# ocean1100/stereo_match

Measured on AMD Instinct MI355X. Metric: stereo pairs/sec + Mpix·disp/sec, KITTI 1242×375 D=128 SGM, 1/2/4/8 GPU, higher is better.
Workload: dtype u8

## Files before the change

### include/stereo_match_amd.h

```cpp
#ifndef STEREO_MATCH_AMD_H
#define STEREO_MATCH_AMD_H

#include <stddef.h>
#include <stdint.h>

#ifdef __cplusplus
extern "C" {
#endif

#define SM_ABI_VERSION 3

#define SM_OK 0
#define SM_E_ARG (-1)
#define SM_E_HIP (-2)
#define SM_E_UNSUPPORTED (-4)

#define SM_COST_SGBM 0
#define SM_COST_CENSUS 1
#define SM_COST_VOLUME 2

#define SM_MODE_SGBM 5
#define SM_MODE_HH 8

typedef struct sm_params {
// ... 158 lines not shown
    int min_disparity;
    int num_disparities;
    int block_size;
    int pre_filter_type;
    int pre_filter_size;
    int pre_filter_cap;
    int texture_threshold;
    int uniqueness_ratio;
    int speckle_window_size;
    int speckle_range;
    int disp12_max_diff;
} sm_bm_params;

int sm_bm_default_params(int num_disparities, int block_size, sm_bm_params* out);
int sm_bm_right_matcher_params(const sm_bm_params* left, sm_bm_params* right_out);
int sm_bm_compute(sm_ctx* ctx, const uint8_t* left, const uint8_t* right, int H, int W, int stride,
                  const sm_bm_params* p, int16_t* disp_out);
int sm_bm_compute_batch_device(sm_ctx* ctx, const uint8_t* d_left, const uint8_t* d_right, int npairs,
                               size_t pair_stride_bytes, int H, int W, int stride, const sm_bm_params* p,
                               int16_t* d_disp_out);

int sm_compute_batch(sm_ctx** ctxs, int ngpu, const uint8_t* const* left, const uint8_t* const* right, int npairs,
                     int H, int W, const sm_params* p, int16_t* out);

int sm_right_matcher_params(const sm_params* left, sm_params* right_out);

int sm_synchronize(sm_ctx* ctx);

int sm_get_counters(sm_ctx* ctx, long long* sweep_fallbacks);

#define SM_COUNTER_SWEEP_FALLBACKS 0
#define SM_COUNTER_EW_REPAIRS 1
#define SM_COUNTER_VOLUME_CLAMPED 2
#define SM_COUNTER_VOLUME_NAN 3
#define SM_COUNTER_LINE_GROUPS 4
#define SM_COUNTER_EW_OPEN 5
#define SM_COUNTER_BAND_REPAIRS 6
#define SM_COUNTER_BAND_OPEN 7
#define SM_COUNTER_BAND_GROUPS 8
#define SM_COUNTER_LINE_STRIPS 9
int sm_get_counter(sm_ctx* ctx, int which, long long* value);

int sm_set_cu_mask(sm_ctx* ctx, const uint32_t* mask, int nwords);

#define SM_STAGE_COST 0
#define SM_STAGE_PATHS 1
#define SM_STAGE_WTA 2
#define SM_STAGE_MEDIAN 3
#define SM_STAGE_TOTAL 4
#define SM_STAGE_WLS 5
#define SM_STAGE_SPECKLE 6
#define SM_STAGE_HORIZONTAL 7
#define SM_STAGE_SWEEP 8
#define SM_STAGE_SWEEP_WTA 9
#define SM_STAGE_H2D 10
#define SM_STAGE_D2H 11
#define SM_STAGE_FALLBACK 12
#define SM_STAGE_CALL 13
#define SM_NUM_STAGES 14
#define SM_TIMING_ONLY 0x40000000
int sm_set_timing(sm_ctx* ctx, int enable);
int sm_get_timing(sm_ctx* ctx, int stage, double* total_ms, long long* launches, long long* pairs);
int sm_reset_timing(sm_ctx* ctx);

long long sm_debug_fetch(sm_ctx* ctx, int what, void* host, size_t bytes);

int sm_set_debug_flags(sm_ctx* ctx, int flags);

#define SM_TUNE_EW_LANES 1
#define SM_TUNE_SWEEP_NCW 2
#define SM_TUNE_EW_WAVES 3
#define SM_TUNE_EW_PRIO 4
#define SM_TUNE_EW_WARMUP 5
#define SM_TUNE_SWEEP_LINES 6
#define SM_TUNE_EW_GUESS 7
#define SM_TUNE_BANDS 8
#define SM_TUNE_BAND_WARMUP 9
#define SM_TUNE_BAND_GUESS 10
#define SM_TUNE_COST_WGS 11
#define SM_TUNE_LR_STAGGER 12
#define SM_TUNE_SWEEP_XCD 13
#define SM_TUNE_PLY_STAGE 14
#define SM_TUNE_EW_START 15
int sm_set_tuning(sm_ctx* ctx, int key, int value);

const char* sm_last_error(sm_ctx* ctx);

const char* sm_version(void);
int sm_abi_version(void);

#ifdef __cplusplus
}
#endif

#endif
```

### stereo_match_amd/_lib.py

```python
from __future__ import annotations

import ctypes
import os
import re
import threading

import numpy as np

_HERE = os.path.dirname(os.path.abspath(__file__))
LIB_PATH = os.environ.get("STEREO_MATCH_AMD_LIB") or os.path.join(_HERE, "libstereo_match_amd.so")
HEADER_PATH = os.path.join(os.path.dirname(_HERE), "include", "stereo_match_amd.h")

SM_OK, SM_E_ARG, SM_E_HIP, SM_E_UNSUPPORTED = 0, -1, -2, -4
SM_COST_SGBM, SM_COST_CENSUS, SM_COST_VOLUME = 0, 1, 2
SM_MODE_SGBM, SM_MODE_HH = 5, 8
TIMING_ONLY = 0x40000000
STAGES = ("cost", "paths", "wta", "median", "total", "wls", "speckle", "horizontal", "sweep", "sweep_wta", "h2d",
          "d2h", "fallback", "call")


class SmParams(ctypes.Structure):
    _fields_ = [(n, ctypes.c_int) for n in (
        "min_disparity", "num_disparities", "block_size", "P1", "P2",
        "disp12_max_diff", "uniqueness_ratio", "pre_filter_cap",
# ... 632 lines not shown
        if src.size and (src.strides[1] != cn or (src.ndim == 3 and src.strides[2] != 1) or src.strides[0] < W * cn):
            src = np.ascontiguousarray(src)
        dH, dW = (H + 1) // 2, (W + 1) // 2
        out = np.empty((dH, dW) if src.ndim == 2 else (dH, dW, cn), np.uint8)
        self._check(self._lib.sm_pyr_down_u8(self.ctx, src.ctypes.data if src.size else None, H, W,
                                             src.strides[0] if src.size else W * cn, cn,
                                             out.ctypes.data if out.size else None))
        return out

    def pyr_down_batch_device(self, d_src: int, nimg: int, src_img_stride: int, H: int, W: int, src_stride: int,
                              channels: int, d_dst: int, dst_img_stride: int, dst_stride: int):
        self._check(self._lib.sm_pyr_down_u8_batch_device(
            self.ctx, ctypes.c_void_p(d_src), nimg, src_img_stride, H, W, src_stride, channels, ctypes.c_void_p(d_dst),
            dst_img_stride, dst_stride))

    def bm_compute(self, left: np.ndarray, right: np.ndarray, params: "SmBmParams") -> np.ndarray:
        left = np.ascontiguousarray(left)
        right = np.ascontiguousarray(right)
        H, W = left.shape
        out = np.empty((H, W), np.int16)
        self._check(self._lib.sm_bm_compute(self.ctx, left.ctypes.data, right.ctypes.data, H, W, W,
                                            ctypes.byref(params), out.ctypes.data))
        return out

    def bm_compute_batch_device(self, d_left: int, d_right: int, npairs: int, pair_stride: int, H: int, W: int,
                                stride: int, params: "SmBmParams", d_out: int):
        self._check(self._lib.sm_bm_compute_batch_device(
            self.ctx, ctypes.c_void_p(d_left), ctypes.c_void_p(d_right), npairs, pair_stride, H, W, stride,
            ctypes.byref(params), ctypes.c_void_p(d_out)))

    def synchronize(self):
        self._check(self._lib.sm_synchronize(self.ctx))

    COUNTERS = ("sweep_fallbacks", "ew_repairs", "volume_clamped", "volume_nan", "line_groups",
                "ew_open", "band_repairs", "band_open", "band_groups", "line_strips")

    def counters(self) -> dict:
        out = {}
        n = ctypes.c_longlong()
        for i, name in enumerate(self.COUNTERS):
            self._check(self._lib.sm_get_counter(self.ctx, i, ctypes.byref(n)))
            out[name] = n.value
        return out

    def set_cu_mask(self, cus):
        if cus is None:
            self._check(self._lib.sm_set_cu_mask(self.ctx, None, 0))
            return
        nwords = (max(cus) // 32 + 1) if cus else 1
        words = (ctypes.c_uint32 * nwords)()
        for c in cus:
            words[c // 32] |= 1 << (c % 32)
        self._check(self._lib.sm_set_cu_mask(self.ctx, words, nwords))

    def set_timing(self, on, stages=None):
        v = int(bool(on))
        if on and stages is not None:
            v = TIMING_ONLY
            for name in stages:
                v |= 1 << STAGES.index(name)
        self._check(self._lib.sm_set_timing(self.ctx, v))

    def reset_timing(self):
        self._check(self._lib.sm_reset_timing(self.ctx))

    def timing(self) -> dict:
        out = {}
        for i, name in enumerate(STAGES):
            ms = ctypes.c_double()
            n = ctypes.c_longlong()
            np_ = ctypes.c_longlong()
            self._check(self._lib.sm_get_timing(self.ctx, i, ctypes.byref(ms), ctypes.byref(n), ctypes.byref(np_)))
            out[name] = (ms.value, n.value, np_.value)
        return out

    def set_debug_flags(self, flags: int):
        self._check(self._lib.sm_set_debug_flags(self.ctx, int(flags)))

    TUNE_EW_LANES, TUNE_SWEEP_NCW, TUNE_EW_WAVES, TUNE_EW_PRIO, TUNE_EW_WARMUP, TUNE_SWEEP_LINES = 1, 2, 3, 4, 5, 6
    TUNE_EW_GUESS = 7
    TUNE_BANDS, TUNE_BAND_WARMUP, TUNE_BAND_GUESS, TUNE_COST_WGS, TUNE_LR_STAGGER, TUNE_SWEEP_XCD = 8, 9, 10, 11, 12, 13
    TUNE_PLY_STAGE = 14
    TUNE_EW_START = 15

    def set_tuning(self, key: int, value: int):
        self._check(self._lib.sm_set_tuning(self.ctx, int(key), int(value)))

    def debug_fetch(self, what: int) -> bytes:
        n = self._lib.sm_debug_fetch(self.ctx, what, None, 0)
        if n < 0:
            _raise(int(n), self.ctx)
        buf = (ctypes.c_char * max(int(n), 1))()
        r = self._lib.sm_debug_fetch(self.ctx, what, buf, int(n))
        if r < 0:
            _raise(int(r), self.ctx)
        return bytes(buf)[:int(n)]


def right_matcher_params(p: SmParams) -> SmParams:
    lib = load()
    out = SmParams()
    rc = lib.sm_right_matcher_params(ctypes.byref(p), ctypes.byref(out))
    if rc != SM_OK:
        _raise(rc, None)
    return out


def compute_batch(engines, lefts, rights, params: SmParams) -> np.ndarray:
    lib = load()
    n = len(lefts)
    if n != len(rights):
        raise ValueError("lefts and rights differ in length")
    if n == 0:
        return np.empty((0, 0, 0), np.int16)
    L = [np.ascontiguousarray(a, np.uint8) for a in lefts]
    R = [np.ascontiguousarray(b, np.uint8) for b in rights]
    H, W = L[0].shape
    if any(a.shape != (H, W) for a in L + R):
        raise ValueError("all images must have the same shape")
    out = np.empty((n, H, W), np.int16)
    ctxs = (ctypes.c_void_p * len(engines))(*[e.ctx for e in engines])
    lp = (ctypes.c_void_p * n)(*[a.ctypes.data for a in L])
    rp = (ctypes.c_void_p * n)(*[b.ctypes.data for b in R])
    rc = lib.sm_compute_batch(ctxs, len(engines), lp, rp, n, H, W, ctypes.byref(params), out.ctypes.data)
    if rc != SM_OK:
        _raise(rc, None)
    return out


_engines: dict = {}


def engine(device: int = 0) -> Engine:
    key = (threading.get_ident(), device)
    e = _engines.get(key)
    if e is None:
        e = _engines[key] = Engine(device)
    return e
```

### stereo_match_amd/csrc/sm_api.hip

```cpp
#include <hip/hip_runtime.h>

#include <algorithm>
#include <cmath>
#include <cstdarg>
#include <cstdio>
#include <cstring>
#include <string>
#include <thread>
#include <type_traits>
#include <vector>

#include "../../include/stereo_match_amd.h"
#include "sm_cost.hpp"
#include "sm_paths.hpp"
#include "sm_post.hpp"
#include "sm_wls.hpp"
#include "sm_speckle.hpp"
#include "sm_reproject.hpp"
#include "sm_rectify.hpp"
#include "sm_nlm.hpp"
#include "sm_filter.hpp"
#include "sm_cloud.hpp"
#include "sm_bm.hpp"
#include "sm_wide.hpp"
// ... 30 lines not shown
    hipEvent_t a, b;
};

struct BufSet {
    DevBuf census[2], cost, L, raw;
    DevBuf part, key2, pre;
    DevBuf st;
    DevBuf vst;
    hipEvent_t paths_done = nullptr, wta_done = nullptr;
    bool pending = false;
};

#ifndef EW_PATCH_ATOM
#define EW_PATCH_ATOM 1
#endif

constexpr int DBG_VL16 = 8, DBG_STORE_W = 16, DBG_ROW = 32, DBG_OVERLAP = 64, DBG_H64 = 512, DBG_NO_C8 = 1024;
constexpr int DBG_OLD_EW = 256, DBG_SWEEP_V2 = 128, DBG_SWEEP2_NW = 1 << 27;
constexpr int DBG_FGS_NO_SWEEP = 1 << 28, DBG_FGS_NO_MEM = 1 << 29;
constexpr int DBG_NO_MALL_GROUPS = 1 << 30;
constexpr int DBG_NARROW_SWEEPS = 1 << 19, DBG_WIDE_SWEEPS = 1 << 21;
constexpr int DBG_LEGACY = 4096, DBG_SWEEP1 = 8192, DBG_SWEEP8 = 16384, DBG_HYBRID = 32768;
constexpr int DBG_COST_TILE = 1 << 22;
constexpr int DBG_CONCURRENT_LR = 1 << 20;
constexpr int DBG_FORCE_FALLBACK = 1 << 23;
constexpr int ERR_GROUP0 = 0, ERR_STICKY = 32, ERR_FALLBACKS = 48;
constexpr int ERR_VOL_CLAMPED = 52, ERR_VOL_NAN = 54, ERR_EW_REPAIRS = 56, ERR_EW_OPEN = 58;
constexpr int ERR_BAND_REPAIRS = 60, ERR_BAND_OPEN = 62;
constexpr int DBG_NO_FALLBACK = (int)0x80000000u;
constexpr int kAblationFlags = 1 | 2 | 4 | DBG_STORE_W | DBG_ROW | DBG_SWEEP_V2 | DBG_SWEEP2_NW | DBG_HYBRID |
                               (7 << 24) | DBG_FGS_NO_SWEEP | DBG_FGS_NO_MEM | DBG_NO_FALLBACK;

}

struct sm_ctx {
    int device = 0;
    hipStream_t own_stream = nullptr;
    hipStream_t stream = nullptr;
    hipStream_t side = nullptr;
    DevBuf img[2], planes, out, dbg, volbuf, sp_parent, sp_count, rp_in, rp_out, rp_min, bm_pre[2], bm_cost;
    DevBuf rm_src, rm_mapx, rm_mapy, rm_dst, rm_gray;
    DevBuf nlm_tab;
    std::vector<int32_t> nlm_tab_host;
    uint32_t nlm_key_h = 0;
    int nlm_key_t = 0, nlm_key_s = 0, nlm_ntab = 0, nlm_shift = 0;
    DevBuf cl_tot, cl_off, ply_tot, ply_off, cl_verts, cl_colors, cl_out;
    DevBuf flt_a;
    DevBuf wls_num, wls_den, wls_inter, wls_w, wls_disp[2], wls_out;
    DevBuf wls_R, wls_IT;
    hipStream_t wls_stream = nullptr;
    hipStream_t lr_stream = nullptr;
    hipEvent_t ev_stagger = nullptr;
    hipEvent_t sweep_done_ev = nullptr;
    bool sweep_done_hit = false;
    int tune_lr_stagger = 0;
    hipEvent_t ev_wls_fork = nullptr, ev_wls_ready = nullptr;
    DevBuf hop, sweep_err;
    DevBuf volwin;

    void* pin = nullptr;
    size_t pin_n = 0;
    sm_ctx* twin = nullptr;
    hipEvent_t ev_lr_fork = nullptr, ev_lr_join = nullptr;
    std::vector<uint32_t> cu_mask;
    uint32_t hop_epoch = 0;
    hipEvent_t ev_fork = nullptr, ev_join = nullptr;
    hipEvent_t ev_fb_fork = nullptr, ev_fb_join = nullptr;
    hipEvent_t ev_ew_done = nullptr;
    const uint32_t* fb_guard = nullptr;
    hipStream_t wta_override = nullptr;
    const uint32_t* wta_skip = nullptr;
    int16_t* wta_dst = nullptr;
    BufSet set[2];
    int next_set = 0;
    int lastH = 0, lastW = 0, last_width1 = 0, lastD = 0, last_ndirs = 0, last_cost = 0, last_minD = 0;
    int last_minX1 = 0, last_index = 0, last_set = 0;
    size_t last_L_pair = 0;
    uint32_t timing = 0;
    int dbg_flags = 0;
    int tune_ew_lanes = 0, tune_sweep_ncw = 0, tune_ew_waves = 0, tune_ew_prio = 0;
    int tune_ew_warmup = 0, tune_sweep_lines = 0;
    int tune_ew_guess = 0;
    int tune_ew_start = 0;
    int tune_bands = 0, tune_band_warmup = 0, tune_band_guess = 0;
    int tune_cost_wgs = 0;
    int tune_ply_stage = 0;
    int tune_sweep_xcd = 0;
    long long line_groups = 0;
    long long band_groups = 0;
    long long line_strips = 0;
    std::vector<TimedEvent> pending;
    std::vector<hipEvent_t> free_events;
    double stage_ms[SM_NUM_STAGES] = {0};
    long long stage_launches[SM_NUM_STAGES] = {0};
    long long stage_pairs[SM_NUM_STAGES] = {0};
    std::string err;
};

namespace {

int fail(sm_ctx* ctx, int code, const char* fmt, ...)
{
    char buf[512];
    va_list ap;
    va_start(ap, fmt);
    vsnprintf(buf, sizeof buf, fmt, ap);
    va_end(ap);
    if (ctx) ctx->err = buf;
    g_thread_error = buf;
    return code;
}

#define HIP_TRY(ctx, expr)                                                                           \
    do {                                                                                              \
        hipError_t e_ = (expr);                                                                       \
        if (e_ != hipSuccess)                                                                         \
            return fail((ctx), SM_E_HIP, "%s failed: %s (%s:%d)", #expr, hipGetErrorString(e_),   \
                        __FILE__, __LINE__);                                                          \
    } while (0)

int ensure(sm_ctx* ctx, DevBuf& b, size_t bytes)
{
    if (b.n >= bytes && b.p) return SM_OK;
    if (b.p) {
        HIP_TRY(ctx, hipDeviceSynchronize());
        (void)hipFree(b.p);
        b.p = nullptr;
        b.n = 0;
    }
    size_t want = std::max<size_t>(bytes, 256);
    HIP_TRY(ctx, hipMalloc(&b.p, want));
    b.n = want;
    return SM_OK;
}

int normalize(sm_ctx* ctx, const sm_params* p, int H, int W, Norm& n, int cn = 1)
{
    if (!p) return fail(ctx, SM_E_ARG, "params is NULL");
    if (H <= 0 || W <= 0) return fail(ctx, SM_E_ARG, "empty image (%dx%d)", W, H);
    if (W > 32767) return fail(ctx, SM_E_UNSUPPORTED, "width %d > 32767", W);
    n.minD = p->min_disparity;
    n.D = n.Dv = p->num_disparities;
    if (p->cost_kind == SM_COST_VOLUME) {
        if (n.Dv <= 0) return fail(ctx, SM_E_ARG, "cost volume needs at least one disparity plane (got %d)", n.Dv);
        n.D = (n.Dv + 15) & ~15;
    } else if (n.D <= 0 || n.D % 16 != 0) {
        return fail(ctx, SM_E_ARG, "numDisparities must be a positive multiple of 16 (got %d)", n.D);
    }
    if (n.D > 256) return fail(ctx, SM_E_UNSUPPORTED, "numDisparities %d > 256 not built", n.Dv);
    n.maxD = n.minD + n.Dv;
    n.bs = p->block_size > 0 ? p->block_size : 5;
    n.ftzero = std::max(p->pre_filter_cap, 15) | 1;
    n.uniq = p->uniqueness_ratio >= 0 ? p->uniqueness_ratio : 10;
    n.disp12 = p->disp12_max_diff > 0 ? p->disp12_max_diff : 1;
    n.P1 = p->P1 > 0 ? p->P1 : 2;
    n.P2 = std::max(p->P2 > 0 ? p->P2 : 5, n.P1 + 1);
    n.speckle_ws = p->speckle_window_size;
    n.speckle_range = p->speckle_range;
    n.cost = p->cost_kind;
    n.mode = p->mode;
    if (n.cost != SM_COST_SGBM && n.cost != SM_COST_CENSUS && n.cost != SM_COST_VOLUME)
        return fail(ctx, SM_E_ARG, "cost_kind %d unknown", n.cost);
    if (n.mode != SM_MODE_SGBM && n.mode != SM_MODE_HH)
        return fail(ctx, SM_E_UNSUPPORTED, "mode %d not supported (5 = MODE_SGBM, 8 = MODE_HH)", n.mode);
    if (cn != 1 && cn != 3) return fail(ctx, SM_E_ARG, "images must have 1 or 3 channels (got %d)", cn);
    if (cn != 1 && n.cost != SM_COST_SGBM) return fail(ctx, SM_E_UNSUPPORTED, "colour input needs the SGBM cost");
// ... 340 lines not shown
    HIP_TRY(ctx, hipGetLastError());
    return SM_OK;
}

template <int DPLV, bool CENSUS>
int launch_paths_dpl(sm_ctx* ctx, const Norm& n, const Geo& g, BufSet& bs, int dirset)
{
    if constexpr ((16 * DPLV) % 64 == 0) {
        if (ctx->dbg_flags & DBG_H64) {
            if (DPLV == 8 && !(ctx->dbg_flags & DBG_VL16))
                return launch_paths_t<DPLV, CENSUS, 8>(ctx, n, g, bs, dirset);
            return launch_paths_t<DPLV, CENSUS, 16>(ctx, n, g, bs, dirset);
        }
    }
    if constexpr (DPLV == 8) {
        if (!(ctx->dbg_flags & DBG_VL16)) return launch_paths_t<DPLV, CENSUS, 8, true>(ctx, n, g, bs, dirset);
    }
    return launch_paths_t<DPLV, CENSUS, 16, true>(ctx, n, g, bs, dirset);
}

enum { DISPATCH_PATHS = 0, DISPATCH_WTA = 1, DISPATCH_HORIZONTAL = 2, DISPATCH_HYBRID = 3 };

int dispatch(sm_ctx* ctx, const Norm& n, const Geo& g, BufSet& bs, int what)
{
    const bool census = n.cost == SM_COST_CENSUS;
    const int h = what == DISPATCH_HORIZONTAL ? DIRS_EW : what == DISPATCH_HYBRID ? DIRS_EW_UP : DIRS_ALL;
    switch (n.dpl) {
#define CASE(k)                                                                                               \
    case k:                                                                                                   \
        if (what == DISPATCH_WTA)                                                                             \
            return census ? launch_wta_t<k, true>(ctx, n, g, bs) : launch_wta_t<k, false>(ctx, n, g, bs);     \
        return census ? launch_paths_dpl<k, true>(ctx, n, g, bs, h) : launch_paths_dpl<k, false>(ctx, n, g, bs, h);
        CASE(1) CASE(2) CASE(3) CASE(4) CASE(5) CASE(6) CASE(7) CASE(8)
        CASE(9) CASE(10) CASE(11) CASE(12) CASE(13) CASE(14) CASE(15) CASE(16)
#undef CASE
    default: return fail(ctx, SM_E_UNSUPPORTED, "numDisparities %d not built", n.D);
    }
}

int ensure_event(sm_ctx* ctx, hipEvent_t& e);
bool use_sweep(const sm_ctx* ctx, const Norm& n, int H);

int hybrid_slots(const Norm& n) { return n.ndirs == 8 ? 5 : 2; }

bool use_hybrid(const sm_ctx* ctx, const Norm& n, int H)
{
    if (!SM_ABLATIONS || (n.ndirs != 8 && n.ndirs != 5) || !(ctx->dbg_flags & DBG_HYBRID) ||
        (ctx->dbg_flags & (DBG_LEGACY | DBG_SWEEP8)))
        return false;
    sm_ctx tmp = *ctx;
    tmp.dbg_flags = (ctx->dbg_flags & ~DBG_HYBRID) | DBG_SWEEP8;
    return use_sweep(&tmp, n, H);
}

bool use_sweep(const sm_ctx* ctx, const Norm& n, int H)
{
    if (ctx->dbg_flags & (DBG_LEGACY | DBG_ROW)) return false;
    if (n.cost == SM_COST_CENSUS && !use_cost8(ctx, n)) return false;
    const int cmax = n.cost == SM_COST_CENSUS ? 64 : n.cost == SM_COST_VOLUME ? smk::VOL_CMAX : 0;
    if (cmax + n.P2 > 16383) return false;
    if (H > 65535 || n.width1 <= 0) return false;
    const size_t W = (size_t)(n.maxX1 - std::min(n.minD, 0));
    if (W * 6 + 16 > kRowLds) return false;
    return (uint64_t)H * n.width1 * n.D * 2 <= smk::kMaxRecords;
}

struct SweepJob {
    const uint8_t* cost;
    size_t cost_pair;
    const uint8_t* ew;
    size_t ew_pair, ew_slot;
    uint16_t* part;
    size_t part_pair;
    uint32_t* key2;
    uint32_t* pre;
    uint32_t* err;
    int G;
    uint8_t* st = nullptr;
    size_t st_pair = 0;
    int ewarm = 0;
    int ewguess = 0;
    int ewstart = 0;
    int part_il = 0;
    int nband = 1, band_h = 0, vwarm = 0, vguess = 0;
    uint8_t* vst = nullptr;
    size_t vst_pair = 0;
};

int stream_cus(hipStream_t st, int ncu)
{
    uint32_t mask[32] = {0};
    const uint32_t words = (uint32_t)std::min(32, (ncu + 31) / 32);
    if (hipExtStreamGetCUMask(st, words, mask) != hipSuccess) return ncu;
    int c = 0;
    for (uint32_t i = 0; i < words; i++) c += __builtin_popcount(mask[i]);
    return c > 0 ? std::min(c, ncu) : ncu;
}

int ensure_sweep_err(sm_ctx* ctx)
{
    if (ctx->sweep_err.p) return SM_OK;
    int rc = ensure(ctx, ctx->sweep_err, SWEEP_STATS ? (size_t(8) << 20) : 256);
    if (rc != SM_OK) return rc;
    HIP_TRY(ctx, hipMemsetAsync(ctx->sweep_err.p, 0, SWEEP_STATS ? (size_t(8) << 20) : 256, ctx->stream));
    return SM_OK;
}

int sweep_variant(const sm_ctx* ctx)
{
    if (SM_ABLATIONS && (ctx->dbg_flags & DBG_SWEEP_V2)) return 6;
    if (SM_ABLATIONS && (ctx->dbg_flags & DBG_SWEEP2_NW)) return 3;
    return (ctx->dbg_flags & DBG_NARROW_SWEEPS) ? 1 : 0;
}

struct SweepFit {
    smk::SweepInfo si{};
    int nwg = 0, cap = 0, ncu = 0;
};
bool sweep_fit_variant(sm_ctx* ctx, const Norm& n, int mode, int variant, SweepFit& f)
{
    if (smk::sweep_info(n.D, (int)elem_bytes(n), mode, variant, ctx->device, &f.si) != hipSuccess) return false;
    int ncu = 0;
    if (hipDeviceGetAttribute(&ncu, hipDeviceAttributeMultiprocessorCount, ctx->device) != hipSuccess) return false;
    f.ncu = stream_cus(ctx->stream, std::max(ncu, 1));
    const int per_cu = f.si.blocks_per_cu >= 3 ? f.si.blocks_per_cu - 1 : std::max(f.si.blocks_per_cu, 1);
    f.cap = per_cu * f.ncu;
    f.nwg = (n.width1 + f.si.cw - 1) / f.si.cw;
    return f.nwg <= f.cap;
}

int sweep_min_pairs(sm_ctx* ctx, const Norm& n)
{
    if (n.cost != SM_COST_CENSUS) return 3;
    SweepFit f;
    if (!sweep_fit_variant(ctx, n, 2, 0, f) || f.nwg <= 0) return 7;
    return std::max(2, std::min(7, (200 + f.nwg - 1) / f.nwg));
}

double sweep_model(const SweepFit& f, int G)
{
    const int per_launch = std::max(1, std::min(G, f.cap / std::max(f.nwg, 1)));
    const int launches = (G + per_launch - 1) / per_launch;
    const int per_cu = (per_launch * f.nwg + f.ncu - 1) / std::max(f.ncu, 1);
    return (double)launches * per_cu * (f.si.threads / 64 - 1) * std::max(f.si.dpl, 1);
}

bool sweep_capacity(sm_ctx* ctx, const Norm& n, int mode, int G, SweepFit& f)
{
    if (ctx->tune_sweep_ncw && sweep_variant(ctx) <= 1) {
        for (int v : {0, 1, 2}) {
            SweepFit t;
            if (sweep_fit_variant(ctx, n, mode, v, t) && t.si.ncw == ctx->tune_sweep_ncw) {
                f = t;
                return true;
            }
        }
        return false;
    }
    const int variant = sweep_variant(ctx);
    if (!sweep_fit_variant(ctx, n, mode, variant, f)) {
        if (!(variant == 0 && f.si.impl == 1 && sweep_fit_variant(ctx, n, mode, 1, f))) return false;
    } else if (variant == 0 && f.si.impl == 1 && G > 0 && !(ctx->dbg_flags & DBG_WIDE_SWEEPS)) {
        SweepFit nf;
        if (sweep_fit_variant(ctx, n, mode, 1, nf) && sweep_model(nf, G) < sweep_model(f, G)) f = nf;
    }
    if (variant == 0 && G > 0 && !(ctx->dbg_flags & DBG_WIDE_SWEEPS)) {
        SweepFit lf;
        if (sweep_fit_variant(ctx, n, mode, 2, lf) && sweep_model(lf, G) < sweep_model(f, G)) f = lf;
    }
    return true;
}

bool sweeps_fit(sm_ctx* ctx, const Norm& n, bool hybrid, bool lines = false)
{
    const int m8[2] = {0, 2}, m5[1] = {1}, mh[1] = {0}, l8[2] = {3, 4}, l5[1] = {3};
    const int* modes = hybrid ? mh : lines ? (n.ndirs == 8 ? l8 : l5) : n.ndirs == 8 ? m8 : m5;
    const int count = !hybrid && n.ndirs == 8 ? 2 : 1;
    for (int k = 0; k < count; k++) {
        SweepFit f;
        if (!sweep_capacity(ctx, n, modes[k], 0, f)) return false;
        if (lines && modes[k] == 3 && f.nwg > smk::patch_max_strips(n.D)) return false;
        if (lines && modes[k] == 3 && f.si.ncw < 11) return false;
    }
    return true;
}

int sweep_pass(sm_ctx* ctx, const Norm& n, const Geo& g, const SweepJob& j, int mode)
{
    SweepFit f;
    const bool banded = j.nband > 1;
    if (banded ? !(sweep_fit_variant(ctx, n, mode, 0, f) && f.si.impl == 1) : !sweep_capacity(ctx, n, mode, j.G, f)) {
        if (f.nwg > f.cap)
            return fail(ctx, SM_E_UNSUPPORTED, "sweep: %d strips exceed %d resident workgroups", f.nwg, f.cap);
        return fail(ctx, SM_E_UNSUPPORTED, "sweep: numDisparities %d not built", n.D);
    }
    const smk::SweepInfo& si = f.si;
    const int nwg = f.nwg, cap = f.cap;
    const int nb = banded ? j.nband : 1;
    const int nblk = banded ? (j.band_h + j.vwarm + si.hb - 1) / si.hb : (g.H + si.hb - 1) / si.hb;
    const int per_launch = (ctx->dbg_flags & DBG_SWEEP1) ? 1 : std::max(1, std::min(j.G, cap / (nwg * nb)));
    const size_t hop_pair = (size_t)nwg * nb * 2 * nblk * si.ngr;
    const size_t hop_bytes = hop_pair * 8 * per_launch;
    if (hop_pair * 8 > smk::kMaxRecords) return fail(ctx, SM_E_UNSUPPORTED, "sweep: boundary buffer too large");
    int rc;
    if (ctx->hop.n < hop_bytes || !ctx->hop.p) {
        if ((rc = ensure(ctx, ctx->hop, hop_bytes)) != SM_OK) return rc;
        HIP_TRY(ctx, hipMemsetAsync(ctx->hop.p, 0, ctx->hop.n, ctx->stream));
        ctx->hop_epoch = 0;
    }
    if ((rc = ensure_sweep_err(ctx)) != SM_OK) return rc;
    for (int p0 = 0; p0 < j.G; p0 += per_launch) {
        const int np = std::min(per_launch, j.G - p0);
        if (++ctx->hop_epoch > 0xFFFFu) {
            HIP_TRY(ctx, hipMemsetAsync(ctx->hop.p, 0, ctx->hop.n, ctx->stream));
            ctx->hop_epoch = 1;
        }
        smk::SweepArgs a{};
        a.cost = j.cost + (size_t)p0 * j.cost_pair;
        a.cost_pair = j.cost_pair;
        a.ew = j.ew ? j.ew + (size_t)p0 * j.ew_pair : nullptr;
        a.ew_pair = j.ew_pair;
        a.ew_slot = j.ew_slot;
        a.part = j.part ? (uint16_t*)((uint8_t*)j.part + (size_t)p0 * j.part_pair) : nullptr;
        a.part_pair = j.part_pair;
        a.hop = (unsigned long long*)ctx->hop.p;
        a.hop_pair = hop_pair;
        a.st = j.st ? j.st + (size_t)p0 * j.st_pair : nullptr;
        a.st_pair = j.st_pair;
        a.ewarm = j.ewarm;
        a.ewguess = j.ewguess;
        a.ewstart = j.ewstart;
        a.part_il = j.part_il;
        a.nband = nb;
        a.band_h = j.band_h;
        a.vwarm = j.vwarm;
        a.vguess = j.vguess;
        a.hop_nblk = nblk;
        a.vst = j.vst ? j.vst + (size_t)p0 * j.vst_pair : nullptr;
        a.vst_pair = j.vst_pair;
        if (ctx->tune_sweep_xcd > 0) {
            a.xcd_total = np * nwg * nb;
            a.xcd_per = (a.xcd_total + 7) / 8;
        }
        a.rec = j.key2 ? j.key2 + (size_t)p0 * g.H * g.W : nullptr;
        a.nb = j.pre ? j.pre + (size_t)p0 * g.H * g.W : nullptr;
        a.err = j.err;
        a.H = g.H;
        a.W = g.W;
        a.W1 = n.width1;
        a.D = n.D;
        a.Dv = n.Dv;
        a.minD = n.minD;
        a.minX1 = n.minX1;
        a.P1 = n.P1;
        a.P2 = n.P2;
        a.uniq = n.uniq;
        a.inv_ku = n.uniq < 100 ? 1.0f / (float)(100 - n.uniq) : 0.f;
        a.nwg = nwg;
        a.epoch = ctx->hop_epoch;
#if SWEEP_STATS
        a.stats = (unsigned long long*)((char*)ctx->sweep_err.p + 1024);
#endif
        a.dbg = (ctx->dbg_flags >> 24) & 7;
        HIP_TRY(ctx, smk::sweep_launch(n.D, (int)elem_bytes(n), mode, si.impl, a, np, ctx->stream));
    }
    return SM_OK;
}

struct StreamSwap {
    sm_ctx* c;
    hipStream_t old;
    StreamSwap(sm_ctx* c_, hipStream_t s) : c(c_), old(c_->stream) { c->stream = s; }
    ~StreamSwap() { c->stream = old; }
};

int ew_lanes(const sm_ctx* ctx, const Norm& n)
{
    if (ctx->tune_ew_lanes) return ctx->tune_ew_lanes;
    if (ctx->dbg_flags & DBG_OLD_EW) return -1;
    if (n.D % 64 == 0) return 32;
    if (n.D % 32 == 0) return 16;
    return elem_bytes(n) == 1 ? 0 : -1;
}

int launch_ew(sm_ctx* ctx, const Norm& n, const Geo& g, BufSet& bs)
{
    const size_t et = elem_bytes(n);
    const int vl = ew_lanes(ctx, n);
    if (vl < 0) return dispatch(ctx, n, g, bs, DISPATCH_HORIZONTAL);
    smk::EwArgs a{};
    a.cost = (const uint8_t*)bs.cost.p;
    a.cost_pair = g.vol * et;
    a.out = (uint8_t*)bs.L.p;
    a.out_pair = g.L_pair;
    a.out_slot = g.slot_bytes;
    a.H = g.H;
    a.W1 = n.width1;
    a.P1 = n.P1;
    a.P2 = n.P2;
    a.wpb = ctx->tune_ew_waves;
    a.prio = ctx->tune_ew_prio;
    StageTimer t(ctx, ctx->stream, SM_STAGE_HORIZONTAL, g.G);
    const hipError_t e = smk::ew_launch(n.D, (int)et, vl, a, g.G, ctx->stream);
    if (e == hipErrorInvalidValue) return fail(ctx, SM_E_UNSUPPORTED, "E/W lines: numDisparities %d not built", n.D);
    HIP_TRY(ctx, e);
    return SM_OK;
}

int run_sweep(sm_ctx* ctx, const Norm& n, const Geo& g, BufSet& bs, hipStream_t wta_stream, uint32_t* err)
{
    const int G = g.G;
    int rc;
    const size_t et = elem_bytes(n);
    SweepJob j{};
    j.cost = (const uint8_t*)bs.cost.p;
// ... 50 lines not shown
        if (ctx->dbg_flags & DBG_FORCE_FALLBACK) HIP_TRY(ctx, hipMemsetAsync(gflag, 1, 1, ws));
        HIP_TRY(ctx, smk::lr_rows_launch((const uint32_t*)bs.key2.p, (const uint32_t*)bs.pre.p, (int16_t*)bs.raw.p,
                                         ctx->wta_dst, g.G, g.H, g.W, n.Dv, n.minD, n.minX1, n.maxX1, n.disp12,
                                         gflag, ws));
        StreamSwap sw(ctx, ws);
        ctx->wta_override = ws;
        ctx->fb_guard = gflag;
        rc = dispatch(ctx, n, g, bs, DISPATCH_PATHS);
        if (rc == SM_OK) rc = dispatch(ctx, n, g, bs, DISPATCH_WTA);
        ctx->fb_guard = nullptr;
        ctx->wta_override = nullptr;
        return rc;
    }
    hipStream_t fs = ctx->side;
    if (fb) {
        if (ctx->dbg_flags & DBG_FORCE_FALLBACK) HIP_TRY(ctx, hipMemsetAsync(gflag, 1, 1, ws));
        if ((rc = ensure_event(ctx, ctx->ev_fb_fork)) != SM_OK) return rc;
        if ((rc = ensure_event(ctx, ctx->ev_fb_join)) != SM_OK) return rc;
        HIP_TRY(ctx, hipEventRecord(ctx->ev_fb_fork, ws));
        HIP_TRY(ctx, hipStreamWaitEvent(fs, ctx->ev_fb_fork, 0));
        StreamSwap sw(ctx, fs);
        ctx->wta_override = fs;
        ctx->fb_guard = gflag;
        rc = dispatch(ctx, n, g, bs, DISPATCH_PATHS);
        if (rc == SM_OK) rc = dispatch(ctx, n, g, bs, DISPATCH_WTA);
        ctx->fb_guard = nullptr;
        ctx->wta_override = nullptr;
        if (rc != SM_OK) return rc;
        HIP_TRY(ctx, hipEventRecord(ctx->ev_fb_join, fs));
    }
    HIP_TRY(ctx, smk::lr_rows_launch((const uint32_t*)bs.key2.p, (const uint32_t*)bs.pre.p, (int16_t*)bs.raw.p,
                                     ctx->wta_dst, g.G, g.H, g.W, n.Dv, n.minD, n.minX1, n.maxX1, n.disp12,
                                     fb ? gflag : nullptr, ws));
    if (fb) HIP_TRY(ctx, hipStreamWaitEvent(ws, ctx->ev_fb_join, 0));
    return SM_OK;
}

bool use_lines(sm_ctx* ctx, const Norm& n)
{
    if (ctx->tune_sweep_lines < 0 || ctx->tune_ew_lanes || (ctx->dbg_flags & DBG_OLD_EW)) return false;
    return sweeps_fit(ctx, n, false, true);
}

int ew_start(const sm_ctx* ctx, const Norm& n)
{
    if (ctx->tune_ew_start < 0) return 0;
    if (ctx->tune_ew_start > 0) return ctx->tune_ew_start == 1 ? smk::EWS_MAXN : ctx->tune_ew_start;
    return elem_bytes(n) == 1 ? smk::EWS_MAXN : 0;
}

int ew_warmup(const sm_ctx* ctx, const Norm& n, int ewstart)
{
    if (ctx->tune_ew_warmup > 0) return ctx->tune_ew_warmup;
    if (ewstart > 0 && elem_bytes(n) == 1) return 9;
    return 16;
}

long long path_max(const Norm& n)
{
    if (n.cost == SM_COST_CENSUS) return 62 + n.P2;
    if (n.cost == SM_COST_VOLUME) return smk::VOL_CMAX + n.P2;
    const long long side = 2 * (n.bs / 2) + 1;
    return side * side * (2 * n.ftzero + (255 >> 2)) + n.P2;
}

int line_bands(const sm_ctx* ctx, const Norm& n, int H, int G)
{
    if (n.ndirs != 5 || ctx->tune_bands == 1 || 5 * path_max(n) > 65535) return 1;
    SweepFit f;
    if (!sweep_fit_variant(const_cast<sm_ctx*>(ctx), n, 3, 0, f) || f.si.impl != 1 || f.nwg <= 0) return 1;
    int nb = ctx->tune_bands >= 2 ? ctx->tune_bands : std::min(f.cap / std::max(1, G * f.nwg), H / 24);
    nb = std::min(nb, H);
    if (nb < 2) return 1;
    const int bh = (H + nb - 1) / nb;
    return (H + bh - 1) / bh;
}

int band_warmup(const sm_ctx* ctx, const Norm& n)
{
    if (ctx->tune_band_warmup > 0) return ctx->tune_band_warmup;
    return elem_bytes(n) == 1 ? 16 : 24;
}

int run_lines(sm_ctx* ctx, const Norm& n, const Geo& g, BufSet& bs, hipStream_t ws, uint32_t* gflag)
{
    const int G = g.G;
    const size_t et = elem_bytes(n);
    int rc;
    SweepJob j{};
    j.cost = (const uint8_t*)bs.cost.p;
    j.cost_pair = g.vol * et;
    j.G = G;
    j.err = gflag;
    if ((rc = ensure(ctx, bs.part, (size_t)G * g.vol * 2)) != SM_OK) return rc;
    j.part = (uint16_t*)bs.part.p;
    j.part_pair = g.vol * 2;
    SweepFit f;
    j.nband = line_bands(ctx, n, g.H, G);
    if (j.nband > 1 ? !sweep_fit_variant(ctx, n, 3, 0, f) : !sweep_capacity(ctx, n, 3, G, f))
        return fail(ctx, SM_E_UNSUPPORTED, "sweep lines: no instance fits");
    j.st_pair = ((size_t)g.H * f.nwg * 4 * n.D * et + 255) & ~size_t(255);
    if ((rc = ensure(ctx, bs.st, j.st_pair * G)) != SM_OK) return rc;
    j.st = (uint8_t*)bs.st.p;
    j.ewstart = ew_start(ctx, n);
    j.ewarm = ew_warmup(ctx, n, j.ewstart);
    j.ewguess = ctx->tune_ew_guess;
    j.part_il = SWEEP_IL && n.ndirs == 8 && et == 1 && n.D != 256 && f.si.dpl % 2 == 0 &&
                f.si.dpl == (n.D % 32 == 0 ? n.D / 16 : n.D / 8) ? 1 : 0;
    if (j.nband > 1 && ctx->tune_ew_warmup <= 0 && et == 2) j.ewarm = 54;
    if (j.nband > 1) {
        j.band_h = (g.H + j.nband - 1) / j.nband;
        j.vwarm = band_warmup(ctx, n);
        j.vguess = ctx->tune_band_guess;
        j.vst_pair = ((size_t)j.nband * 6 * n.width1 * n.D * et + 255) & ~size_t(255);
        if ((rc = ensure(ctx, bs.vst, j.vst_pair * G)) != SM_OK) return rc;
        j.vst = (uint8_t*)bs.vst.p;
        ctx->band_groups++;
    }
    ctx->line_groups++;
    ctx->line_strips += (long long)f.nwg * G;
    const bool fb_side = n.ndirs == 5 && ws == ctx->stream && !(ctx->dbg_flags & DBG_NO_FALLBACK);
    {
        StageTimer t(ctx, ctx->stream, SM_STAGE_PATHS, G);
        {
            StageTimer ts(ctx, ctx->stream, SM_STAGE_SWEEP, G);
            if ((rc = sweep_pass(ctx, n, g, j, 3)) != SM_OK) return rc;
        }
        if (ctx->sweep_done_ev) {
            HIP_TRY(ctx, hipEventRecord(ctx->sweep_done_ev, ctx->stream));
            ctx->sweep_done_hit = true;
        }
        smk::EwPatchArgs pa{};
        pa.cost = j.cost;
        pa.cost_pair = j.cost_pair;
        pa.part = j.part;
        pa.part_pair = j.part_pair * 1;
        pa.st = j.st;
        pa.st_pair = j.st_pair;
        pa.H = g.H;
        pa.W1 = n.width1;
        pa.nwg = f.nwg;
        pa.cw = f.si.cw;
        pa.P1 = n.P1;
        pa.P2 = n.P2;
        pa.guard = gflag;
        pa.fixes = reinterpret_cast<unsigned long long*>((uint32_t*)ctx->sweep_err.p + ERR_EW_REPAIRS);
        pa.atom = EW_PATCH_ATOM && et == 2 && 5 * path_max(n) < 65536 ? 1 : 0;
        pa.part_il = j.part_il;
        auto ew_patch = [&](hipStream_t st) -> int {
            const hipError_t e = smk::ew_patch_launch(n.D, (int)et, pa, G, st);
            if (e == hipErrorInvalidValue) return fail(ctx, SM_E_UNSUPPORTED, "E/W patch: numDisparities %d not built", n.D);
            HIP_TRY(ctx, e);
            return SM_OK;
        };
        const bool ew_side = fb_side && pa.atom && j.nband > 1;
        if (fb_side) {
            if (ctx->dbg_flags & DBG_FORCE_FALLBACK) HIP_TRY(ctx, hipMemsetAsync(gflag, 1, 1, ctx->stream));
            if ((rc = ensure_event(ctx, ctx->ev_fb_fork)) != SM_OK) return rc;
            if ((rc = ensure_event(ctx, ctx->ev_fb_join)) != SM_OK) return rc;
            HIP_TRY(ctx, hipEventRecord(ctx->ev_fb_fork, ctx->stream));
            HIP_TRY(ctx, hipStreamWaitEvent(ctx->side, ctx->ev_fb_fork, 0));
            if (ew_side) {
                if ((rc = ensure_event(ctx, ctx->ev_ew_done)) != SM_OK) return rc;
                {
                    StageTimer th(ctx, ctx->side, SM_STAGE_HORIZONTAL, G);
                    if ((rc = ew_patch(ctx->side)) != SM_OK) return rc;
                }
                HIP_TRY(ctx, hipEventRecord(ctx->ev_ew_done, ctx->side));
            }
            StreamSwap sw(ctx, ctx->side);
            ctx->wta_override = ctx->side;
            ctx->fb_guard = gflag;
            rc = dispatch(ctx, n, g, bs, DISPATCH_PATHS);
            if (rc == SM_OK) rc = dispatch(ctx, n, g, bs, DISPATCH_WTA);
            ctx->fb_guard = nullptr;
            ctx->wta_override = nullptr;
            if (rc != SM_OK) return rc;
            HIP_TRY(ctx, hipEventRecord(ctx->ev_fb_join, ctx->side));
        }
        if (!ew_side) {
            StageTimer th(ctx, ctx->stream, SM_STAGE_HORIZONTAL, G);
            if ((rc = ew_patch(ctx->stream)) != SM_OK) return rc;
        }
        if (j.nband > 1) {
            smk::BandPatchArgs ba{};
            ba.cost = j.cost;
            ba.cost_pair = j.cost_pair;
            ba.part = j.part;
            ba.part_pair = j.part_pair;
            ba.vst = j.vst;
            ba.vst_pair = j.vst_pair;

            ba.H = g.H;
            ba.W1 = n.width1;
            ba.nband = j.nband;
            ba.band_h = j.band_h;
            ba.P1 = n.P1;
            ba.P2 = n.P2;
            ba.guard = gflag;
            ba.fixes = reinterpret_cast<unsigned long long*>((uint32_t*)ctx->sweep_err.p + ERR_BAND_REPAIRS);
            const hipError_t eb = smk::band_patch_launch(n.D, (int)et, ba, G, ctx->stream);
            if (eb == hipErrorInvalidValue) return fail(ctx, SM_E_UNSUPPORTED, "band patch: numDisparities %d not built", n.D);
            HIP_TRY(ctx, eb);
            if (ew_side) HIP_TRY(ctx, hipStreamWaitEvent(ctx->stream, ctx->ev_ew_done, 0));
        }
    }
    if (ws != ctx->stream) {
        HIP_TRY(ctx, hipEventRecord(bs.paths_done, ctx->stream));
        HIP_TRY(ctx, hipStreamWaitEvent(ws, bs.paths_done, 0));
    }
    if (n.ndirs == 8) {
        if ((rc = ensure(ctx, bs.key2, (size_t)G * g.H * g.W * 4)) != SM_OK) return rc;
        if ((rc = ensure(ctx, bs.pre, (size_t)G * g.H * g.W * 4)) != SM_OK) return rc;
        j.key2 = (uint32_t*)bs.key2.p;
        j.pre = (uint32_t*)bs.pre.p;
        {
            StreamSwap sw(ctx, ws);
            StageTimer t(ctx, ctx->stream, SM_STAGE_WTA, G);
            StageTimer ts(ctx, ctx->stream, SM_STAGE_SWEEP_WTA, G);
            if ((rc = sweep_pass(ctx, n, g, j, 4)) != SM_OK) return rc;
        }
        return sweep_finish(ctx, n, g, bs, ws, gflag);
    }
    StreamSwap sw(ctx, ws);
    ctx->wta_override = ws;
    {
        StageTimer ts(ctx, ws, SM_STAGE_SWEEP_WTA, G);
        ctx->wta_skip = fb_side ? gflag : nullptr;
        rc = dispatch(ctx, n, g, bs, DISPATCH_WTA);
        ctx->wta_skip = nullptr;
    }
    if (fb_side) {
        if (rc == SM_OK) HIP_TRY(ctx, hipStreamWaitEvent(ws, ctx->ev_fb_join, 0));
    } else if (rc == SM_OK && !(ctx->dbg_flags & DBG_NO_FALLBACK)) {
        if (ctx->dbg_flags & DBG_FORCE_FALLBACK) HIP_TRY(ctx, hipMemsetAsync(gflag, 1, 1, ws));
        ctx->fb_guard = gflag;
        rc = dispatch(ctx, n, g, bs, DISPATCH_PATHS);
        if (rc == SM_OK) rc = dispatch(ctx, n, g, bs, DISPATCH_WTA);
        ctx->fb_guard = nullptr;
    }
    ctx->wta_override = nullptr;
    return rc;
}

int run_hybrid(sm_ctx* ctx, const Norm& n, const Geo& g, BufSet& bs)
{
    const int G = g.G;
    int rc;
    SweepJob j{};
    j.cost = (const uint8_t*)bs.cost.p;
    j.cost_pair = g.vol * elem_bytes(n);
    j.G = G;
    if ((rc = ensure_sweep_err(ctx)) != SM_OK) return rc;
    j.err = (uint32_t*)ctx->sweep_err.p + ERR_STICKY;
    if ((rc = ensure(ctx, bs.part, (size_t)G * g.vol * 2)) != SM_OK) return rc;
    j.part = (uint16_t*)bs.part.p;
    j.part_pair = g.vol * 2;
    if ((rc = ensure_event(ctx, ctx->ev_fork)) != SM_OK) return rc;
    if ((rc = ensure_event(ctx, ctx->ev_join)) != SM_OK) return rc;
    StageTimer t(ctx, ctx->stream, SM_STAGE_PATHS, G);
    HIP_TRY(ctx, hipEventRecord(ctx->ev_fork, ctx->stream));
    HIP_TRY(ctx, hipStreamWaitEvent(ctx->side, ctx->ev_fork, 0));
    const hipStream_t main = ctx->stream;
    ctx->stream = ctx->side;
    {
        StageTimer ts(ctx, ctx->stream, SM_STAGE_SWEEP, G);
        rc = sweep_pass(ctx, n, g, j, 0);
    }
    ctx->stream = main;
    if (rc != SM_OK) return rc;
    HIP_TRY(ctx, hipEventRecord(ctx->ev_join, ctx->side));
    if ((rc = dispatch(ctx, n, g, bs, n.ndirs == 8 ? DISPATCH_HYBRID : DISPATCH_HORIZONTAL)) != SM_OK) return rc;
    HIP_TRY(ctx, hipStreamWaitEvent(ctx->stream, ctx->ev_join, 0));
    return SM_OK;
}

int check_sweep_errors(sm_ctx* ctx)
{
    if (ctx->twin) {
        int rc = check_sweep_errors(ctx->twin);
        if (rc != SM_OK) return fail(ctx, rc, "%s", ctx->twin->err.c_str());
    }
    if (!ctx->sweep_err.p) return SM_OK;
    uint32_t e = 0;
    uint32_t* w = (uint32_t*)ctx->sweep_err.p + ERR_STICKY;
    HIP_TRY(ctx, hipMemcpy(&e, w, 4, hipMemcpyDeviceToHost));
    if (e) {
        HIP_TRY(ctx, hipMemset(w, 0, 4));
        return fail(ctx, SM_E_HIP, "sweep: strip-boundary hand-off timed out (workgroups not co-resident?)");
    }
    return SM_OK;
}

int cost_nt(const Geo& g, size_t elem_bytes)
{
    return (size_t)g.G * g.vol * elem_bytes > ((size_t)224 << 20) ? 1 : 0;
}

#ifndef SGBM_COST2_WGS
#define SGBM_COST2_WGS 2048
#endif
template <int S, int CPT>
int launch_cost2_s(sm_ctx* ctx, const Norm& n, const Geo& g, const smk::SgbmCostArgs& sc)
// ... 2497 lines not shown
        hipError_t e = hipStreamCreateWithFlags(&b, hipStreamNonBlocking);
        if (e != hipSuccess) {
            (void)hipStreamDestroy(a);
            return fail(ctx, SM_E_HIP, "hipStreamCreateWithFlags: %s", hipGetErrorString(e));
        }
    }
    (void)hipStreamDestroy(ctx->own_stream);
    (void)hipStreamDestroy(ctx->side);
    if (ctx->wls_stream) {
        (void)hipStreamDestroy(ctx->wls_stream);
        ctx->wls_stream = nullptr;
    }
    if (ctx->lr_stream) {
        (void)hipStreamDestroy(ctx->lr_stream);
        ctx->lr_stream = nullptr;
    }
    ctx->own_stream = a;
    ctx->side = b;
    ctx->stream = a;
    ctx->cu_mask.assign(mask, mask + nwords);
    if (ctx->twin) {
        int rc = sm_set_cu_mask(ctx->twin, mask, nwords);
        if (rc != SM_OK) return fail(ctx, rc, "%s", ctx->twin->err.c_str());
    }
    return SM_OK;
}

int sm_set_timing(sm_ctx* ctx, int enable)
{
    if (!ctx) return fail(nullptr, SM_E_ARG, "ctx is NULL");
    if (ctx->twin) sm_set_timing(ctx->twin, enable);
    ctx->timing = enable == 0 ? 0u
                : (enable & SM_TIMING_ONLY) ? (uint32_t)enable & ((1u << SM_NUM_STAGES) - 1)
                                            : (1u << SM_NUM_STAGES) - 1;
    return SM_OK;
}

int sm_set_debug_flags(sm_ctx* ctx, int flags)
{
    if (!ctx) return fail(nullptr, SM_E_ARG, "ctx is NULL");
    if (!SM_ABLATIONS && (flags & kAblationFlags))
        return fail(ctx, SM_E_UNSUPPORTED, "debug flags 0x%x need the ablation build (make -C stereo_match_amd/csrc "
                    "ablation; STEREO_MATCH_AMD_LIB=.../libstereo_match_amd_ablate.so)",
                    (unsigned)(flags & kAblationFlags));
    if (ctx->twin) sm_set_debug_flags(ctx->twin, flags);
    ctx->dbg_flags = flags;
    return SM_OK;
}

int sm_set_tuning(sm_ctx* ctx, int key, int value)
{
    if (!ctx) return fail(nullptr, SM_E_ARG, "ctx is NULL");
    switch (key) {
    case SM_TUNE_EW_LANES:
        if (value != 0 && value != -1 && value != 8 && value != 16 && value != 32 && value != 64)
            return fail(ctx, SM_E_ARG, "E/W lanes %d: 0, -1, 8, 16, 32 or 64", value);
        ctx->tune_ew_lanes = value;
        break;
    case SM_TUNE_EW_WAVES:
        if (value < 0 || value > 4) return fail(ctx, SM_E_ARG, "E/W waves per workgroup %d: 0..4", value);
        ctx->tune_ew_waves = value;
        break;
    case SM_TUNE_EW_PRIO:
        if (value < 0 || value > 3) return fail(ctx, SM_E_ARG, "E/W issue priority %d: 0..3", value);
        ctx->tune_ew_prio = value;
        break;
    case SM_TUNE_SWEEP_NCW:
        if (value < 0) return fail(ctx, SM_E_ARG, "sweep compute waves %d < 0", value);
        ctx->tune_sweep_ncw = value;
        break;
    case SM_TUNE_EW_WARMUP:
        if (value < 0 || value > 4096) return fail(ctx, SM_E_ARG, "E/W segment warmup %d: 0..4096", value);
        ctx->tune_ew_warmup = value;
        break;
    case SM_TUNE_EW_GUESS:
        if (value < 0 || value > 1) return fail(ctx, SM_E_ARG, "E/W guess %d: 0 or 1", value);
        ctx->tune_ew_guess = value;
        break;
    case SM_TUNE_EW_START:
        if (value < -1 || value > smk::EWS_MAXN)
            return fail(ctx, SM_E_ARG, "E/W start state %d: -1, 0, 1 or 2..%d cost columns", value, smk::EWS_MAXN);
        ctx->tune_ew_start = value;
        break;
    case SM_TUNE_SWEEP_LINES:
        if (value < -1 || value > 1) return fail(ctx, SM_E_ARG, "sweep lines %d: -1, 0 or 1", value);
        ctx->tune_sweep_lines = value;
        break;
    case SM_TUNE_BANDS:
        if (value < 0 || value > 65535) return fail(ctx, SM_E_ARG, "row bands %d: 0..65535", value);
        ctx->tune_bands = value;
        break;
    case SM_TUNE_BAND_WARMUP:
        if (value < 0 || value > 4096) return fail(ctx, SM_E_ARG, "band warmup %d: 0..4096", value);
        ctx->tune_band_warmup = value;
        break;
    case SM_TUNE_BAND_GUESS:
        if (value < 0 || value > 1) return fail(ctx, SM_E_ARG, "band guess %d: 0 or 1", value);
        ctx->tune_band_guess = value;
        break;
    case SM_TUNE_COST_WGS:
        if (value < 0 || value > 65536) return fail(ctx, SM_E_ARG, "cost workgroups %d: 0..65536", value);
        ctx->tune_cost_wgs = value;
        break;
    case SM_TUNE_SWEEP_XCD:
        if (value < -1 || value > 1) return fail(ctx, SM_E_ARG, "sweep XCD placement %d: -1, 0 or 1", value);
        ctx->tune_sweep_xcd = value;
        break;
    case SM_TUNE_LR_STAGGER:
        if (value < -1 || value > 1) return fail(ctx, SM_E_ARG, "matcher stagger %d: -1, 0 or 1", value);
        ctx->tune_lr_stagger = value;
        break;
    case SM_TUNE_PLY_STAGE:
        if (value < -1 || value > 1) return fail(ctx, SM_E_ARG, "PLY staging %d: -1, 0 or 1", value);
        ctx->tune_ply_stage = value;
        break;
    default: return fail(ctx, SM_E_ARG, "unknown tuning key %d", key);
    }
    if (ctx->twin) sm_set_tuning(ctx->twin, key, value);
    return SM_OK;
}

int sm_reset_timing(sm_ctx* ctx)
{
    if (!ctx) return fail(nullptr, SM_E_ARG, "ctx is NULL");
    if (ctx->twin) sm_reset_timing(ctx->twin);
    harvest_timing(ctx);
    for (int i = 0; i < SM_NUM_STAGES; i++) {
        ctx->stage_ms[i] = 0;
        ctx->stage_launches[i] = 0;
        ctx->stage_pairs[i] = 0;
    }
    return SM_OK;
}

int sm_get_timing(sm_ctx* ctx, int stage, double* total_ms, long long* launches, long long* pairs)
{
    if (!ctx) return fail(nullptr, SM_E_ARG, "ctx is NULL");
    if (stage < 0 || stage >= SM_NUM_STAGES) return fail(ctx, SM_E_ARG, "stage %d out of range", stage);
    harvest_timing(ctx);
    double ms = ctx->stage_ms[stage];
    long long nl = ctx->stage_launches[stage], np = ctx->stage_pairs[stage];
    if (ctx->twin) {
        double tms = 0;
        long long tl = 0, tp = 0;
        sm_get_timing(ctx->twin, stage, &tms, &tl, &tp);
        ms += tms;
        nl += tl;
        np += tp;
    }
    if (total_ms) *total_ms = ms;
    if (launches) *launches = nl;
    if (pairs) *pairs = np;
    return SM_OK;
}

long long sm_debug_fetch(sm_ctx* ctx, int what, void* host, size_t bytes)
{
    if (!ctx) return fail(nullptr, SM_E_ARG, "ctx is NULL");
    const size_t et = ctx->last_cost == SM_COST_CENSUS ? 1 : 2;
    const size_t vol = (size_t)ctx->lastH * ctx->last_width1 * ctx->lastD;
    const size_t slot_bytes = (vol * et + 255) & ~size_t(255);
    const size_t img = (size_t)ctx->lastH * ctx->lastW;
    const int li = ctx->last_index;
    BufSet& bs = ctx->set[ctx->last_set];
    size_t need;
    switch (what) {
// ... 82 lines not shown
```

### stereo_match_amd/csrc/sm_ew.hpp

```cpp
#pragma once
#include "sm_pk.hpp"
#include "sm_sweep_host.hpp"

namespace smk {

#ifndef SWEEP_STREAM_AUX
#define SWEEP_STREAM_AUX 2
#endif
#ifndef EW_H16
#define EW_H16 1
#endif
#ifndef EW_STEPN
#define EW_STEPN 1
#endif

template <int VL, int NP, typename CT, typename LT, int PF>
__global__ void __launch_bounds__(256) k_ew(EwArgs a)
{
    constexpr int LPW = 64 / VL, DPL = 2 * NP, D = VL * DPL;
    constexpr int CB = DPL * (int)sizeof(CT);
    switch (a.prio) {
    case 1: __builtin_amdgcn_s_setprio(1); break;
    case 2: __builtin_amdgcn_s_setprio(2); break;
    case 3: __builtin_amdgcn_s_setprio(3); break;
    default: break;
    }
    const int lane = threadIdx.x & 63, wave = threadIdx.x >> 6;
    const int g = lane % VL, kl = lane / VL;
    const int dir = (int)blockIdx.x >= a.nrb ? 1 : 0;
    const int H = a.H, W1 = a.W1;
    const int y0 = (((int)blockIdx.x - dir * a.nrb) * a.wpb + wave) * LPW;
    if (y0 >= H) return;
    const bool line_ok = y0 + kl < H;
    const int y = min(y0 + kl, H - 1);
    const size_t pair = blockIdx.y;
    const uint64_t cells = (uint64_t)H * W1 * D;
    const rsrc_t rc = make_rsrc(a.cost + pair * a.cost_pair, cells * sizeof(CT));
    const rsrc_t ro = make_rsrc(a.out + pair * a.out_pair + (size_t)dir * a.out_slot, cells * sizeof(LT));
    const uint32_t estep = dir ? (uint32_t)(-D) : (uint32_t)D;
    uint32_t e = ((uint32_t)y * (uint32_t)W1 + (uint32_t)(dir ? W1 - 1 : 0)) * (uint32_t)D + (uint32_t)(g * DPL);
    const uint32_t P1p = (uint32_t)a.P1 * 0x10001u, P2p = (uint32_t)a.P2 * 0x10001u;
    constexpr bool H16 = sizeof(CT) == 1 && EW_H16;
    constexpr uint32_t EDGE = H16 ? 0x7BFF7BFFu : (kBig | (kBig << 16));
    const uint32_t eL = g == 0 ? EDGE : 0u, eR = g == VL - 1 ? EDGE : 0u;

    RawBytes<CB> ring[PF];
#pragma unroll
    for (int k = 0; k < PF; k++) {
        ring[k].load(rc, k < W1 ? (e + (uint32_t)k * estep) * (uint32_t)sizeof(CT) : kOOB);
        asm volatile("" ::: "memory");
    }
    uint32_t Lp[NP];
#pragma unroll
    for (int k = 0; k < NP; k++) Lp[k] = 0;
    uint32_t minLp = 0;
    for (int s0 = 0; s0 < W1; s0 += PF) {
#pragma unroll
        for (int k = 0; k < PF; k++) {
            const int s = s0 + k;
#pragma unroll
            for (int j = 0; j < RawBytes<CB>::WORDS; j++) asm volatile("" : "+v"(ring[k].w[j]) : "v"(minLp));
            uint32_t C[NP];
            unpack_ct_pk<CT, DPL>(ring[k], C);
#pragma unroll
            for (int i = 0; i < NP; i++) asm volatile("" : "+v"(C[i])::"memory");
            ring[k].load(rc, s + PF < W1 ? (e + (uint32_t)PF * estep) * (uint32_t)sizeof(CT) : kOOB);
            uint32_t Ln[NP], mn;
            if constexpr (EW_STEPN) {
                uint32_t Lp1[1][NP], m1[1] = {minLp}, C1[1][NP], Ln1[1][NP], mn1[1];
#pragma unroll
                for (int i = 0; i < NP; i++) {
                    Lp1[0][i] = Lp[i];
                    C1[0][i] = C[i];
                }
                sweep_step2n<VL, NP, H16, 1>(Lp1, m1, C1, P1p, P2p, eL, eR, Ln1, mn1);
#pragma unroll
                for (int i = 0; i < NP; i++) Ln[i] = Ln1[0][i];
                mn = mn1[0];
            } else {
                mn = sweep_step2<VL, NP, H16>(Lp, minLp, C, P1p, P2p, eL, eR, Ln);
            }
            store_pk<LT, NP, SWEEP_STREAM_AUX>(ro, (line_ok && s < W1) ? e * (uint32_t)sizeof(LT) : kOOB, Ln);
            e += estep;
#pragma unroll
            for (int i = 0; i < NP; i++) Lp[i] = Ln[i];
            minLp = mn;
        }
    }
}

#ifndef EW_PATCH_NO_CARRY
#define EW_PATCH_NO_CARRY 0
#endif
#ifndef EW_PATCH_B64
#define EW_PATCH_B64 1
#endif
#ifndef EW_PATCH_RC
#define EW_PATCH_RC 0
#endif
template <int VL, int NP, typename CT, bool ATOM = false>
__global__ void __launch_bounds__(256) k_ew_patch(EwPatchArgs a)
{
    constexpr int LPW = 64 / VL, DPL = 2 * NP, D = VL * DPL;
    constexpr int CB = DPL * (int)sizeof(CT);
    constexpr bool H16 = sizeof(CT) == 1 && EW_H16;
    constexpr bool SAT = sizeof(CT) == 2;
    constexpr uint32_t EDGE = H16 ? 0x7BFF7BFFu : (kBig | (kBig << 16));
    constexpr int KU = 8;
    constexpr int CHUNK = LPW * KU;
    constexpr int RC = EW_PATCH_RC ? EW_PATCH_RC : sizeof(CT) == 1 ? 8 : 16;
    if (a.guard && __hip_atomic_load(a.guard, __ATOMIC_RELAXED, __HIP_MEMORY_SCOPE_AGENT) != 0u) return;
    const int lane = threadIdx.x & 63, wave = threadIdx.x >> 6;
    const int g = lane % VL, kl = lane / VL;
    const int yw = (int)blockIdx.x * 4 + wave;
    const int y = ATOM ? yw >> 1 : yw;
    const int dir0 = ATOM ? (yw & 1) : 0, dir1 = ATOM ? dir0 + 1 : 2;
    const size_t pair = blockIdx.y;
    const int H = a.H, W1 = a.W1, nwg = a.nwg, CW = a.cw;
    if (y >= H) return;
    const uint64_t cells = (uint64_t)H * W1 * D;
    const rsrc_t rc = make_rsrc(a.cost + pair * a.cost_pair, cells * sizeof(CT));
    const rsrc_t rp = make_rsrc((const uint8_t*)a.part + pair * a.part_pair, cells * 2);
    uint32_t* const pw = reinterpret_cast<uint32_t*>((uint8_t*)a.part + pair * a.part_pair);
    auto atom_add = [&](uint32_t word, uint32_t first, uint32_t second) {
        const int lo = (int)(second & 0xFFFFu) - (int)(first & 0xFFFFu);
        const int hi = (int)(second >> 16) - (int)(first >> 16);
        const uint32_t add = (uint32_t)(hi * 65536 + lo);
        if (add) __hip_atomic_fetch_add(pw + word, add, __ATOMIC_RELAXED, __HIP_MEMORY_SCOPE_AGENT);
    };
    const rsrc_t rs = make_rsrc(a.st + pair * a.st_pair, a.st_pair);
    const uint32_t P1p = (uint32_t)a.P1 * 0x10001u, P2p = (uint32_t)a.P2 * 0x10001u;
    const uint32_t eL = g == 0 ? EDGE : 0u, eR = g == VL - 1 ? EDGE : 0u;
    const bool pil = !ATOM && a.part_il != 0;
    auto soff = [&](int k, int dir, int which) -> uint32_t {
        return (((((uint32_t)y * (uint32_t)nwg + (uint32_t)k) * 2u + (uint32_t)dir) * 2u + (uint32_t)which) *
                    (uint32_t)D + (uint32_t)(g * DPL)) * (uint32_t)sizeof(CT);
    };
    auto cell = [&](int c) -> uint32_t { return ((uint32_t)y * (uint32_t)W1 + (uint32_t)c) * (uint32_t)D + (uint32_t)(g * DPL); };
    auto line_all = [&](bool ok) -> bool { return group_min<VL>(ok ? 1u : 0u) != 0u; };
    auto same_state = [&](const uint32_t (&x)[NP], const uint32_t (&z)[NP]) -> bool {
        bool ok = true;
#pragma unroll
        for (int i = 0; i < NP; i++) ok &= x[i] == z[i];
        return line_all(ok);
    };
    auto state_min = [&](const uint32_t (&x)[NP]) -> uint32_t {
        uint32_t m = x[0];
#pragma unroll
        for (int i = 1; i < NP; i++) m = pk_min(m, x[i]);
        m = ::min(m & 0xFFFFu, m >> 16);
        return group_min<VL>(m) * 0x10001u;
    };
    auto load_state = [&](uint32_t off, uint32_t (&v)[NP]) {
        RawBytes<CB> b;
        b.load(rs, off);
        unpack_ct_pk<CT, DPL>(b, v);
    };
    auto walk = [&](int k, int dir, uint32_t aoff, uint32_t toff, uint32_t (&T)[NP], bool check) -> int {
        const int x0 = k * CW, ncol = ::min(CW, W1 - x0);
        RawBytes<CB> cc[RC];
        RawBytes<DPL * 2> pb[RC];
        auto issue1 = [&](int u, int o) {
            const int c = dir ? x0 + CW - 1 - o : x0 + o;
            cc[u].load(rc, o < ncol ? cell(c) * (uint32_t)sizeof(CT) : kOOB);
            if constexpr (!ATOM) pb[u].load(rp, o < ncol ? cell(c) * 2u : kOOB);
        };
        auto issue = [&](int o0) {
#pragma unroll
            for (int u = 0; u < RC; u++) issue1(u, o0 + u);
        };
        issue(0);
        uint32_t A[NP];
        load_state(aoff, A);
        if (toff != kOOB) load_state(toff, T);
        if (check && same_state(A, T)) return 2;
        uint32_t Lq[2][NP], mq[2];
#pragma unroll
        for (int q = 0; q < NP; q++) {
            Lq[0][q] = A[q];
            Lq[1][q] = T[q];
        }
        mq[0] = state_min(Lq[0]);
        mq[1] = state_min(Lq[1]);
        bool met = false;
        for (int o0 = 0; o0 < ncol && !met; o0 += RC) {
            if (o0 > 0) issue(o0);
#pragma unroll
            for (int u = 0; u < RC; u++) {
                const int o = o0 + u;
                if (o >= ncol || met) continue;
                const int c = dir ? x0 + CW - 1 - o : x0 + o;
                uint32_t C2[2][NP], Ln[2][NP], mn[2], pv_[NP];
                unpack_ct_pk<CT, DPL>(cc[u], C2[0]);
#pragma unroll
                for (int q = 0; q < NP; q++) pv_[q] = ATOM ? 0u : pb[u].w[q];
                if (pil) {
                    uint32_t t[NP];
                    pk_to_plain<NP, true>(pv_, t);
#pragma unroll
                    for (int q = 0; q < NP; q++) pv_[q] = t[q];
                }
#pragma unroll
                for (int q = 0; q < NP; q++) C2[1][q] = C2[0][q];
                sweep_step2n<VL, NP, H16, 2>(Lq, mq, C2, P1p, P2p, eL, eR, Ln, mn);
                if (same_state(Ln[0], Ln[1])) {
                    met = true;
                    continue;
                }
                if constexpr (ATOM) {
#pragma unroll
                    for (int q = 0; q < NP; q++) atom_add(cell(c) / 2u + (uint32_t)q, Ln[0][q], Ln[1][q]);
                }
                uint32_t P[NP];
#pragma unroll
                for (int q = 0; q < NP && !ATOM; q++) {
                    if constexpr (SAT) {
                        const uint32_t pv = pv_[q];
                        const uint32_t x = pk_adds(pk_sub(pv, Ln[0][q]), Ln[1][q]);
                        const uint32_t sat = pk_sub(pk_min(pk_add(pv, 0x00010001u), 0x00010001u), 0x00010001u);
                        P[q] = pkw(__builtin_elementwise_max(pkv(x), pkv(sat)));
                    } else {
                        P[q] = pk_add(pk_sub(pv_[q], Ln[0][q]), Ln[1][q]);
                    }
                }
                if (pil) {
                    uint32_t t[NP];
                    pk_from_plain<NP, true>(P, t);
#pragma unroll
                    for (int q = 0; q < NP; q++) P[q] = t[q];
                }
                if constexpr (!ATOM) bstore_n<uint32_t, NP>(rp, cell(c) * 2u, P);
#pragma unroll
                for (int q = 0; q < NP; q++) {
                    Lq[0][q] = Ln[0][q];
                    Lq[1][q] = Ln[1][q];
                }
                mq[0] = mn[0];
                mq[1] = mn[1];
            }
        }
        if (!met) {
#pragma unroll
            for (int q = 0; q < NP; q++) T[q] = pk_sub(Lq[1][q], mq[1]);
        }
        return met ? 1 : 0;
    };
    constexpr int DPLW = D % 128 == 0 ? D / 64 : 2, NPW = DPLW / 2;
    constexpr int CBW = DPLW * (int)sizeof(CT);
    auto soff64 = [&](int k, int dir, int which) -> uint32_t {
        return (((((uint32_t)y * (uint32_t)nwg + (uint32_t)k) * 2u + (uint32_t)dir) * 2u + (uint32_t)which) *
                    (uint32_t)D + (uint32_t)(lane * DPLW)) * (uint32_t)sizeof(CT);
    };
    auto cell64 = [&](int c) -> uint32_t {
        return ((uint32_t)y * (uint32_t)W1 + (uint32_t)c) * (uint32_t)D + (uint32_t)(lane * DPLW);
    };
    auto load_state64 = [&](uint32_t off, uint32_t (&v)[NPW]) {
        RawBytes<CBW> b;
        b.load(rs, off);
        unpack_ct_pk<CT, DPLW>(b, v);
    };
    auto same_state64 = [&](const uint32_t (&x)[NPW], const uint32_t (&z)[NPW]) -> bool {
        bool ok = true;
#pragma unroll
        for (int i = 0; i < NPW; i++) ok &= x[i] == z[i];
        return __all(ok);
    };
    auto state_min64 = [&](const uint32_t (&x)[NPW]) -> uint32_t {
        uint32_t m = x[0];
#pragma unroll
        for (int i = 1; i < NPW; i++) m = pk_min(m, x[i]);
        m = ::min(m & 0xFFFFu, m >> 16);
        return Line<64>::min(m) * 0x10001u;
    };
    auto walk64 = [&](int k, int dir, uint32_t aoff, uint32_t toff, uint32_t (&T)[NPW], bool check) -> int {
        const int x0 = k * CW, ncol = ::min(CW, W1 - x0);
        RawBytes<CBW> cc[RC];
        RawBytes<DPLW * 2> pb[RC];
        auto issue1 = [&](int u, int o) {
            const int c = dir ? x0 + CW - 1 - o : x0 + o;
            cc[u].load(rc, o < ncol ? cell64(c) * (uint32_t)sizeof(CT) : kOOB);
            if constexpr (!ATOM) pb[u].load(rp, o < ncol ? cell64(c) * 2u : kOOB);
        };
        auto issue = [&](int o0) {
#pragma unroll
            for (int u = 0; u < RC; u++) issue1(u, o0 + u);
        };
        issue(0);
        uint32_t A[NPW];
        load_state64(aoff, A);
        if (toff != kOOB) load_state64(toff, T);
        if (check && same_state64(A, T)) return 2;
        uint32_t Lq[2][NPW], mq[2];
#pragma unroll
        for (int q = 0; q < NPW; q++) {
            Lq[0][q] = A[q];
            Lq[1][q] = T[q];
        }
        mq[0] = state_min64(Lq[0]);
        mq[1] = state_min64(Lq[1]);
        bool met = false;
        for (int o0 = 0; o0 < ncol && !met; o0 += RC) {
            if (o0 > 0) issue(o0);
#pragma unroll
            for (int u = 0; u < RC; u++) {
                const int o = o0 + u;
                if (o >= ncol || met) continue;
                const int c = dir ? x0 + CW - 1 - o : x0 + o;
                uint32_t C2[2][NPW], Ln[2][NPW], mn[2], pv_[NPW];
                unpack_ct_pk<CT, DPLW>(cc[u], C2[0]);
#pragma unroll
                for (int q = 0; q < NPW; q++) pv_[q] = ATOM ? 0u : pb[u].w[q];
#pragma unroll
                for (int q = 0; q < NPW; q++) C2[1][q] = C2[0][q];
                sweep_step2n<64, NPW, H16, 2>(Lq, mq, C2, P1p, P2p, 0u, 0u, Ln, mn);
                if (same_state64(Ln[0], Ln[1])) {
                    met = true;
                    continue;
                }
                if constexpr (ATOM) {
#pragma unroll
                    for (int q = 0; q < NPW; q++) atom_add(cell64(c) / 2u + (uint32_t)q, Ln[0][q], Ln[1][q]);
                }
                uint32_t P[NPW];
#pragma unroll
                for (int q = 0; q < NPW && !ATOM; q++) {
                    if constexpr (SAT) {
                        const uint32_t pv = pv_[q];
                        const uint32_t x = pk_adds(pk_sub(pv, Ln[0][q]), Ln[1][q]);
                        const uint32_t sat = pk_sub(pk_min(pk_add(pv, 0x00010001u), 0x00010001u), 0x00010001u);
                        P[q] = pkw(__builtin_elementwise_max(pkv(x), pkv(sat)));
                    } else {
                        P[q] = pk_add(pk_sub(pv_[q], Ln[0][q]), Ln[1][q]);
                    }
                }
                if constexpr (!ATOM) bstore_n<uint32_t, NPW>(rp, cell64(c) * 2u, P);
#pragma unroll
                for (int q = 0; q < NPW; q++) {
                    Lq[0][q] = Ln[0][q];
                    Lq[1][q] = Ln[1][q];
                }
                mq[0] = mn[0];
                mq[1] = mn[1];
            }
        }
        if (!met) {
#pragma unroll
            for (int q = 0; q < NPW; q++) T[q] = pk_sub(Lq[1][q], mq[1]);
        }
        return met ? 1 : 0;
    };
    auto lines_or = [&](uint64_t v) -> uint64_t {
        uint64_t m = 0;
#pragma unroll
        for (int l = 0; l < LPW; l++) {
            const uint32_t lo = __builtin_amdgcn_readlane((uint32_t)v, l * VL);
            const uint32_t hi = __builtin_amdgcn_readlane((uint32_t)(v >> 32), l * VL);
            m |= ((uint64_t)hi << 32) | lo;
        }
        return m;
    };
    auto order_partial = [&]() {
        __builtin_amdgcn_fence(__ATOMIC_RELEASE, "workgroup");
        __builtin_amdgcn_fence(__ATOMIC_ACQUIRE, "workgroup");
    };
    __shared__ uint64_t openm[4][kPatchMaxChunks];
    uint32_t nfix = 0, nopen = 0;
    for (int dir = dir0; dir < dir1; dir++) {
        auto strip_of = [&](int i) { return dir ? nwg - 1 - i : i; };
        int first_open = nwg;
        for (int i0 = 1, ch = 0; i0 < nwg; i0 += CHUNK, ch++) {
            RawBytes<CB> sb[KU], eb[KU];
#pragma unroll
            for (int u = 0; u < KU; u++) {
                const int i = i0 + kl + LPW * u;
                sb[u].load(rs, i < nwg ? soff(strip_of(i), dir, 0) : kOOB);
                eb[u].load(rs, i < nwg ? soff(strip_of(i - 1), dir, 1) : kOOB);
            }
            uint64_t bad = 0;
#pragma unroll
            for (int u = 0; u < KU; u++) {
                bool ok = true;
#pragma unroll
                for (int q = 0; q < RawBytes<CB>::WORDS; q++) ok &= sb[u].w[q] == eb[u].w[q];
                ok = line_all(ok);
                if (!ok && i0 + kl + LPW * u < nwg) bad |= 1ull << (kl + LPW * u);
            }
            const uint64_t m = lines_or(bad);
            uint64_t open = 0;
            uint64_t rest = m;
            while (rest) {
                int mine = -1;
#pragma unroll
                for (int l = 0; l < LPW; l++) {
                    if (rest && l == kl) mine = __builtin_ctzll(rest);
                    if (rest) rest &= rest - 1;
                }
                if (mine >= 0) {
                    const int i = i0 + mine, k = strip_of(i);
                    uint32_t T[NP];
                    nfix++;
                    if (walk(k, dir, soff(k, dir, 0), soff(strip_of(i - 1), dir, 1), T, false) == 0) {
                        store_pk<CT, NP>(rs, soff(k, dir, 0), T);
                        open |= 1ull << mine;
                    }
                }
            }
            open = lines_or(open);
            nopen += (uint32_t)__builtin_popcountll(open);
            if (lane == 0) openm[wave][ch] = open;
            if (open && first_open == nwg) first_open = i0 + __builtin_ctzll(open);
        }
        if (first_open < nwg && !EW_PATCH_NO_CARRY && D % 128 == 0 && EW_PATCH_B64 && !pil) {
            order_partial();
            bool carry = false;
            uint32_t T[NPW];
#pragma unroll
            for (int q = 0; q < NPW; q++) T[q] = 0;
            for (int i = first_open; i < nwg; i++) {
                const int k = strip_of(i);
                if (carry) {
                    const int r = walk64(k, dir, soff64(strip_of(i - 1), dir, 1), kOOB, T, true);
                    nfix += r != 2 && kl == 0;
                    if (r != 0) carry = false;
                }
                const bool open_i = ((openm[wave][(i - 1) / CHUNK] >> ((i - 1) % CHUNK)) & 1ull) != 0;
                if (!carry && open_i) {
                    load_state64(soff64(k, dir, 0), T);
                    carry = true;
                }
            }
        } else if (first_open < nwg && !EW_PATCH_NO_CARRY) {
            order_partial();
            if (kl == 0) {
                bool carry = false;
                uint32_t T[NP];
#pragma unroll
                for (int q = 0; q < NP; q++) T[q] = 0;
                for (int i = first_open; i < nwg; i++) {
                    const int k = strip_of(i);
                    if (carry) {
                        const int r = walk(k, dir, soff(strip_of(i - 1), dir, 1), kOOB, T, true);
                        nfix += r != 2;
                        if (r != 0) carry = false;
                    }
                    const bool open_i = ((openm[wave][(i - 1) / CHUNK] >> ((i - 1) % CHUNK)) & 1ull) != 0;
                    if (!carry && open_i) {
                        load_state(soff(k, dir, 0), T);
                        carry = true;
                    }
                }
            }
        }
        if (!ATOM && dir == 0) order_partial();
    }
    if (a.fixes) {
        nfix = group_sum_u32_wave(g == 0 ? nfix : 0u);
        if (lane == 0 && nfix) atomicAdd(a.fixes, (unsigned long long)nfix);
        if (lane == 0 && nopen) atomicAdd(a.fixes + 1, (unsigned long long)nopen);
    }
}

template <int VL, int NP, typename CT>
__global__ void __launch_bounds__(256) k_band_patch(BandPatchArgs a)
{
    constexpr int LPW = 64 / VL, DPL = 2 * NP, D = VL * DPL, CB = DPL * (int)sizeof(CT);
    constexpr bool H16 = sizeof(CT) == 1 && EW_H16;
    constexpr uint32_t EDGE = H16 ? 0x7BFF7BFFu : (kBig | (kBig << 16));
    constexpr int RC = 8;
    if (a.guard && __hip_atomic_load(a.guard, __ATOMIC_RELAXED, __HIP_MEMORY_SCOPE_AGENT) != 0u) return;
    const int lane = threadIdx.x & 63, wave = threadIdx.x >> 6;
    const int g = lane % VL, kl = lane / VL;
    const int bi = (int)blockIdx.y + 1;
    const size_t pair = blockIdx.z;
    const int H = a.H, W1 = a.W1;
    const int y0 = bi * a.band_h;
    const int id = ((int)blockIdx.x * 4 + wave) * LPW + kl;
    const bool on = id < 3 * W1 && y0 < H;
    const int dir = on ? id / W1 : 0, x = on ? id % W1 : 0;
    const int dx = dir == 0 ? 0 : dir == 1 ? 1 : -1;
    const int nr = !on ? 0 : dx == 0 ? H - y0 : dx > 0 ? min(H - y0, W1 - 1 - x) : min(H - y0, x);
    const uint64_t cells = (uint64_t)H * W1 * D;
    const rsrc_t rc = make_rsrc(a.cost + pair * a.cost_pair, cells * sizeof(CT));
    const rsrc_t rv = make_rsrc(a.vst + pair * a.vst_pair, a.vst_pair);
    uint32_t* part = reinterpret_cast<uint32_t*>(reinterpret_cast<uint8_t*>(a.part) + pair * a.part_pair);
    const uint32_t P1p = (uint32_t)a.P1 * 0x10001u, P2p = (uint32_t)a.P2 * 0x10001u;
    const uint32_t eL = g == 0 ? EDGE : 0u, eR = g == VL - 1 ? EDGE : 0u;
    auto voff = [&](int band, int which, int col) -> uint32_t {
        return (((((uint32_t)band * 2u + (uint32_t)which) * 3u + (uint32_t)dir) * (uint32_t)W1 + (uint32_t)col) *
                    (uint32_t)D + (uint32_t)(g * DPL)) * (uint32_t)sizeof(CT);
    };
    auto cost_off = [&](int r) -> uint32_t {
        return r < nr ? (((uint32_t)(y0 + r) * (uint32_t)W1 + (uint32_t)(x + dx * (r + 1))) * (uint32_t)D +
                         (uint32_t)(g * DPL)) * (uint32_t)sizeof(CT)
                      : kOOB;
    };
    auto line_all = [&](bool ok) -> bool { return group_min<VL>(ok ? 1u : 0u) != 0u; };
    auto state_min = [&](const uint32_t (&v)[NP]) -> uint32_t {
        uint32_t m = v[0];
#pragma unroll
        for (int i = 1; i < NP; i++) m = pk_min(m, v[i]);
        m = ::min(m & 0xFFFFu, m >> 16);
        return group_min<VL>(m) * 0x10001u;
    };
    RawBytes<CB> sb, tb, cc[RC];
    sb.load(rv, on ? voff(bi, 0, x) : kOOB);
    tb.load(rv, on ? voff(bi - 1, 1, x) : kOOB);
#pragma unroll
    for (int u = 0; u < RC; u++) cc[u].load(rc, cost_off(u));
    uint32_t Lq[2][NP], mq[2];
    unpack_ct_pk<CT, DPL>(sb, Lq[0]);
    unpack_ct_pk<CT, DPL>(tb, Lq[1]);
    bool same = true;
#pragma unroll
    for (int i = 0; i < NP; i++) same &= Lq[0][i] == Lq[1][i];
    same = line_all(same);
    uint32_t nfix = 0, nlong = 0;
    if (on && !same && nr > 0) {
        nfix++;
        mq[0] = state_min(Lq[0]);
        mq[1] = state_min(Lq[1]);
        const int rb = min(H, y0 + a.band_h) - y0;
        bool met = false;
        int r0 = 0;
        for (; r0 < nr && !met; r0 += RC) {
            if (r0 > 0) {
#pragma unroll
                for (int u = 0; u < RC; u++) cc[u].load(rc, cost_off(r0 + u));
            }
#pragma unroll
            for (int u = 0; u < RC; u++) {
                const int r = r0 + u;
                if (r >= nr || met) continue;
                uint32_t C2[2][NP], Ln[2][NP], mn[2];
                unpack_ct_pk<CT, DPL>(cc[u], C2[0]);
#pragma unroll
                for (int q = 0; q < NP; q++) C2[1][q] = C2[0][q];
                sweep_step2n<VL, NP, H16, 2>(Lq, mq, C2, P1p, P2p, eL, eR, Ln, mn);
                bool eq = true;
#pragma unroll
                for (int q = 0; q < NP; q++) eq &= Ln[0][q] == Ln[1][q];
                if (line_all(eq)) {
                    met = true;
// ... 31 lines not shown
```

### stereo_match_amd/csrc/sm_sweep.hip

```cpp
#include <algorithm>

#include "sm_sweep.hpp"
#include "sm_sweep_host.hpp"
#ifndef SWEEP_WIDE
#define SWEEP_WIDE 0
#endif
#ifndef SM_ABLATIONS
#define SM_ABLATIONS 0
#endif
#if SM_ABLATIONS
#include "sm_sweep2.hpp"
#endif

namespace smk {

namespace {

template <class F>
hipError_t with_sweep(int D, int ct_bytes, F& f)
{
    return ct_bytes == 1 ? with_d<uint8_t, SWEEP_MODE>(D, f) : with_d<uint16_t, SWEEP_MODE>(D, f);
}

}

template <typename CT, int MODE, class F>
hipError_t with_d(int D, F& f)
{
    switch (D) {
#define SW8(d) \
    case d: return f.template run<8, d / 8, CT, MODE>();
#define SW16(d) \
    case d: return f.template run<16, d / 16, CT, MODE>();
        SW8(16) SW8(32) SW8(48) SW8(64) SW16(80) SW16(96) SW16(112)
#ifdef SWEEP_VL8_128
        SW8(128)
#else
        SW16(128)
#endif
        SW16(144) SW16(160) SW16(176) SW16(192) SW16(208) SW16(224) SW16(240)
#if SWEEP_WIDE == 1
    case 256:
        if constexpr (sizeof(CT) == 1) return f.template run<32, 8, CT, MODE>();
        else return f.template run<16, 16, CT, MODE>();
#else
        SW16(256)
#endif
#undef SW8
#undef SW16
    default: return hipErrorInvalidValue;
    }
}

namespace {

template <int D, typename CT>
constexpr int unit_ncw()
{
    if constexpr (SWEEP_WIDE == 2) return lat_built(D) ? kLatNcw : 0;
    return SWEEP_WIDE ? wide_ncw(D, (int)sizeof(CT)) : kNarrowNcw;
}

template <int VL, int DPL, typename CT, int MODE>
constexpr bool unit_built()
{
    constexpr int NCW = unit_ncw<VL * DPL, CT>();
    if constexpr (NCW == 0) return false;
    else if constexpr (MODE < 3) return true;
    else if constexpr (DPL % 2 != 0 || SWEEP_U32) return false;
    else if constexpr (MODE == 3) return LineGeo<VL, DPL, NCW, 3, (int)sizeof(CT)>::BUILT;
    else return true;
}

struct InfoF {
    int device;
    SweepInfo* out;
    template <int VL, int DPL, typename CT, int MODE>
    hipError_t run()
    {
        constexpr int NCW = unit_ncw<VL * DPL, CT>();
        if constexpr (!unit_built<VL, DPL, CT, MODE>()) {
            return hipErrorInvalidValue;
        } else {
            using SG = SweepGeo<VL, DPL, NCW>;
            constexpr int THREADS = sweep_threads<VL, DPL, NCW, MODE>();
            auto kern = k_sweep<VL, DPL, CT, MODE, NCW>;
            static int per_cu = -1;
            if (per_cu < 0) {
                int nb = 0;
                if (hipOccupancyMaxActiveBlocksPerMultiprocessor(&nb, kern, THREADS, 0) != hipSuccess) nb = 0;
                hipFuncAttributes fa{};
                if (SWEEP_WIDE && (hipFuncGetAttributes(&fa, (const void*)kern) != hipSuccess || fa.localSizeBytes > 0))
                    nb = 0;
                per_cu = SWEEP_WIDE ? nb : std::max(nb, 1);
            }
            if (per_cu < 1) return hipErrorInvalidValue;
            out->cw = SG::CW;
            out->hb = SG::HB;
            out->ngr = SG::SNG;
            out->threads = THREADS;
            out->blocks_per_cu = per_cu;
            out->impl = SWEEP_WIDE == 2 ? 2 : SWEEP_WIDE ? 1 : 0;
            out->dpl = DPL;
            out->ncw = NCW;
            return hipSuccess;
        }
    }
};

struct LaunchF {
    const SweepArgs* a;
    dim3 grid;
    hipStream_t stream;
    template <int VL, int DPL, typename CT, int MODE>
    hipError_t run()
    {
        constexpr int NCW = unit_ncw<VL * DPL, CT>();
        if constexpr (!unit_built<VL, DPL, CT, MODE>()) {
            return hipErrorInvalidValue;
        } else {
            hipLaunchKernelGGL((k_sweep<VL, DPL, CT, MODE, NCW>), grid, dim3(sweep_threads<VL, DPL, NCW, MODE>()), 0,
                               stream, *a);
            return hipGetLastError();
        }
    }
};

#if !SWEEP_WIDE && SM_ABLATIONS && SWEEP_MODE <= 2

constexpr int sw2_pf(int mode) { return mode == 2 ? 2 : 4; }

template <int NW, int CPW, int NP, int MODE>
hipError_t sweep2_run(bool info, int device, SweepInfo* out, const SweepArgs* a, int npairs, hipStream_t stream)
{
    using SG = Sweep2Geo<NW, CPW, NP>;
    auto kern = k_sweep2<NW, CPW, NP, uint8_t, MODE, sw2_pf(MODE)>;
    if (info) {
        static int per_cu = -1;
        if (per_cu < 0) {
            int nb = 0;
            if (hipOccupancyMaxActiveBlocksPerMultiprocessor(&nb, kern, SG::THREADS, 0) != hipSuccess) nb = 1;
            per_cu = nb;
        }
        out->cw = SG::CW;
        out->hb = SG::HB;
        out->ngr = SG::NGR;
        out->threads = SG::THREADS;
        out->blocks_per_cu = per_cu;
        out->impl = NW;
        out->dpl = 128 / 64;
        out->ncw = NW;
        return hipSuccess;
    }
    hipLaunchKernelGGL(kern, dim3(a->nwg, npairs), dim3(SG::THREADS), 0, stream, *a);
    return hipGetLastError();
}

template <int NW, int CPW>
hipError_t sweep2_d(int D, bool info, int device, SweepInfo* out, const SweepArgs* a, int npairs, hipStream_t stream)
{
    constexpr int PARTS = 64 / CPW;
    if (D != 128) return hipErrorInvalidValue;
    return sweep2_run<NW, CPW, 128 / (2 * PARTS), SWEEP_MODE>(info, device, out, a, npairs, stream);
}

hipError_t sweep2(int D, int ct_bytes, int variant, bool info, int device, SweepInfo* out, const SweepArgs* a,
                  int npairs, hipStream_t stream)
{
    if (ct_bytes != 1) return hipErrorInvalidValue;
    switch (variant) {
    case 3: return sweep2_d<3, 16>(D, info, device, out, a, npairs, stream);
    case 6: return sweep2_d<6, 8>(D, info, device, out, a, npairs, stream);
    default: return hipErrorInvalidValue;
    }
}

#endif

}

#define SW_CAT2(a, b) a##b
#define SW_CAT(a, b) SW_CAT2(a, b)

#if SWEEP_WIDE == 2
hipError_t SW_CAT(sweep_info_lat_m, SWEEP_MODE)(int D, int ct_bytes, int device, SweepInfo* out)
{
    InfoF f{device, out};
    return with_sweep(D, ct_bytes, f);
}

hipError_t SW_CAT(sweep_launch_lat_m, SWEEP_MODE)(int D, int ct_bytes, const SweepArgs& a, int npairs,
                                                  hipStream_t stream)
{
    LaunchF f{&a, a.xcd_per > 0 ? dim3(8 * a.xcd_per, 1) : dim3(a.nwg * (a.nband > 1 ? a.nband : 1), npairs), stream};
    return with_sweep(D, ct_bytes, f);
}
#elif SWEEP_WIDE
hipError_t SW_CAT(sweep_info_wide_m, SWEEP_MODE)(int D, int ct_bytes, int device, SweepInfo* out)
{
    InfoF f{device, out};
    return with_sweep(D, ct_bytes, f);
}

hipError_t SW_CAT(sweep_launch_wide_m, SWEEP_MODE)(int D, int ct_bytes, const SweepArgs& a, int npairs,
                                                   hipStream_t stream)
{
    LaunchF f{&a, a.xcd_per > 0 ? dim3(8 * a.xcd_per, 1) : dim3(a.nwg * (a.nband > 1 ? a.nband : 1), npairs), stream};
    return with_sweep(D, ct_bytes, f);
}
#else
hipError_t SW_CAT(sweep_info_m, SWEEP_MODE)(int D, int ct_bytes, int variant, int device, SweepInfo* out)
{
#if SM_ABLATIONS && SWEEP_MODE <= 2
    if (variant && sweep2(D, ct_bytes, variant, true, device, out, nullptr, 0, nullptr) == hipSuccess)
        return hipSuccess;
#else
    (void)variant;
#endif
    InfoF f{device, out};
    return with_sweep(D, ct_bytes, f);
}

hipError_t SW_CAT(sweep_launch_m, SWEEP_MODE)(int D, int ct_bytes, int variant, const SweepArgs& a, int npairs,
                                              hipStream_t stream)
{
#if SM_ABLATIONS && SWEEP_MODE <= 2
    if (variant) {
        const hipError_t e = sweep2(D, ct_bytes, variant, false, 0, nullptr, &a, npairs, stream);
        if (e != hipErrorInvalidValue) return e;
    }
#else
    (void)variant;
#endif
    LaunchF f{&a, a.xcd_per > 0 ? dim3(8 * a.xcd_per, 1) : dim3(a.nwg * (a.nband > 1 ? a.nband : 1), npairs), stream};
    return with_sweep(D, ct_bytes, f);
}
#endif

#if SWEEP_MODE == 0 && !SWEEP_WIDE
hipError_t lr_rows_launch(const uint32_t* rec, const uint32_t* nb, int16_t* out, int16_t* wta, int G, int H, int W,
                          int D, int minD, int minX1, int maxX1, int disp12, const uint32_t* guard, hipStream_t stream)
{
    hipLaunchKernelGGL(k_lr_rows, dim3(H, G), dim3(256), (size_t)W * 6 + 16, stream, rec, nb, out, wta, H, W, D, minD,
                       minX1, maxX1, disp12, guard);
    return hipGetLastError();
}
#endif

}
```

### stereo_match_amd/csrc/sm_sweep.hpp

```cpp
#pragma once
#include "sm_common.hpp"
#include "sm_sweep_host.hpp"
#include "sm_pk.hpp"

#include <type_traits>

namespace smk {

typedef __attribute__((address_space(1))) unsigned long long gu64;

constexpr uint32_t SW_SPIN_LIMIT = 1u << 19;

#if SWEEP_STATS
#define SW_T0(v) const uint64_t v = __builtin_readcyclecounter()
#define SW_ACC(acc, v) acc += __builtin_readcyclecounter() - v
#else
#define SW_T0(v) (void)0
#define SW_ACC(acc, v) (void)0
#endif

#ifndef SWEEP_STREAM_AUX
#define SWEEP_STREAM_AUX 2
#endif

#ifndef SWEEP_COST_AUX
#define SWEEP_COST_AUX 0
#endif

#ifndef SWEEP_ROW_SYNC
#define SWEEP_ROW_SYNC 1
#endif
#ifndef SWEEP_ROW_SLEEP
#define SWEEP_ROW_SLEEP 1
#endif

#ifndef SWEEP_U32
#define SWEEP_U32 0
#endif
#ifndef SWEEP_H16
#define SWEEP_H16 1
#endif
#ifndef SWEEP_DS
#define SWEEP_DS 1
#endif
#ifndef SWEEP_DS_LINES
#define SWEEP_DS_LINES 1
#endif
#ifndef SWEEP_DS_LANE0
#define SWEEP_DS_LANE0 0
#endif
#define SWEEP_DS_RN 16
static_assert(62 * SWEEP_DS_RN + 62 + 193 + 192 < 2048, "DS renormalisation interval too long for the f16 form");
#ifndef SWEEP_STEPN
#define SWEEP_STEPN 1
#endif
#ifndef SWEEP_LDS_FIRST
#define SWEEP_LDS_FIRST 1
#endif
template <typename CT, int DPL>
constexpr bool sweep_il()
{
    return SWEEP_IL && sizeof(CT) == 1 && DPL % 2 == 0 && !SWEEP_U32;
}

constexpr int kNarrowNcw = 7;
#ifndef SWEEP_LAT_NCW
#define SWEEP_LAT_NCW 5
#endif
constexpr int kLatNcw = SWEEP_LAT_NCW;
constexpr bool lat_built(int D) { return D % 32 == 0 && D >= 64 && D <= 224; }
#ifndef SWEEP_HM
#define SWEEP_HM 2
#endif
template <int VL, int DPL, int NCW_ = kNarrowNcw>
struct SweepGeo {
    static constexpr int LPW = 64 / VL;
    static constexpr int HM = (DPL % 2 == 0 && !SWEEP_U32 && NCW_ >= 2 + 2 * SWEEP_HM) ? SWEEP_HM : 1;
    static constexpr int NCW = NCW_;
    static constexpr int THREADS = (NCW + 1) * 64;
    static constexpr int HW = HM * LPW;
    static constexpr int HB = HW;
    static constexpr int NCOL = (NCW - 2) * LPW + 2 * HW;
    static constexpr int COLS = NCOL + 2;
    static constexpr int CW = (NCW - 2) * LPW;
    static constexpr int D = VL * DPL;
    static constexpr int NG = (DPL + 1) / 2;
    static constexpr int NDAT = NG * HW * VL;
    static constexpr int SNG = NDAT + HW;
    static constexpr int PF = ((DPL >= 10 && NCW_ >= 11) || VL == 32) ? 2 : 4;
    static_assert(NCW - 2 >= 2 * HM, "the snapshot's own waves of the two sides are distinct");
    static_assert(HB % PF == 0, "the input ring is indexed by the row within a block");
};

constexpr int wide_ncw(int D, int ct_bytes)
{
    if (ct_bytes == 1 && D == 256) return 15;
    if (ct_bytes == 1) return (D <= 96 || D == 128 || D == 160 || D == 192) ? 11 : 0;
    if (D == 16 || D == 32 || D == 96) return 13;
    return (D == 48 || D == 80 || D == 128 || D == 160) ? 11 : 0;
}

#ifndef SWEEP_NLW
#define SWEEP_NLW 4
#endif
#ifndef SWEEP_HALO_POLL
#define SWEEP_HALO_POLL 1
#endif
#ifndef SWEEP_LINE_PRIO
#define SWEEP_LINE_PRIO 2
#endif
#ifndef SWEEP_LPF8
#define SWEEP_LPF8 12
#endif
#ifndef SWEEP_LPF16
#define SWEEP_LPF16 12
#endif
constexpr int largest_divisor_upto(int n, int cap)
{
    for (int p = cap < n ? cap : n; p > 1; p--)
        if (n % p == 0) return p;
    return 1;
}
#ifndef SWEEP_LEAD_BLOCKS
#define SWEEP_LEAD_BLOCKS 1
#endif
#ifndef SWEEP_LINE_NOBAR
#define SWEEP_LINE_NOBAR 1
#endif
#ifndef SWEEP_NOBAR_MODES
#define SWEEP_NOBAR_MODES 21
#endif
constexpr int kMaxLds = 163840;
#ifndef SWEEP_ROWSYNC_M1
#define SWEEP_ROWSYNC_M1 0
#endif
template <int DPL, int MODE>
constexpr bool sweep_nobar()
{
    return SWEEP_ROW_SYNC && (MODE != 1 || SWEEP_ROWSYNC_M1) && DPL % 2 == 0 && !SWEEP_U32 &&
           (MODE == 3 ? SWEEP_LINE_NOBAR != 0 : ((SWEEP_NOBAR_MODES >> MODE) & 1) != 0);
}
template <int DPL, int MODE>
constexpr bool sweep_halo_poll() { return sweep_nobar<DPL, MODE>() && SWEEP_HALO_POLL; }
template <int VL, int DPL, int NCW_, int MODE, int CTB = 1>
struct LineGeo {
    using G = SweepGeo<VL, DPL, NCW_>;
    static constexpr bool ON = MODE == 3;
    static constexpr bool DSO = CTB == 1 && SWEEP_DS && SWEEP_DS_LINES && SWEEP_H16 && VL != 8;
    static constexpr bool HPOLL = sweep_halo_poll<DPL, MODE>();
    static constexpr int POLLER = HPOLL ? 0 : 1;
    static constexpr int NLW = !ON ? 0 : (SWEEP_NLW < 16 - POLLER - NCW_ ? SWEEP_NLW : 16 - POLLER - NCW_);
    static constexpr int RPW = G::LPW / 2;
    static constexpr int BASE = 8 * G::COLS * G::D + 16 * G::COLS + 4 * NCW_ + 4 * 16 + 512 + 4 * G::D;
    static constexpr int ROWB = G::CW * G::D * 2 + (DSO ? G::CW * 8 : 0);
    static constexpr int FIT = (kMaxLds - BASE) / ROWB;
    static constexpr int LEAD0 = SWEEP_LEAD_BLOCKS * G::HB;
    static constexpr int LEAD = LEAD0 + RPW <= FIT ? LEAD0 : (FIT > RPW ? (FIT - RPW) / RPW * RPW : 0);
    static constexpr int LR = SWEEP_LINE_NOBAR ? FIT : LEAD + 2 * RPW <= FIT ? LEAD + 2 * RPW : LEAD + RPW;
    static constexpr bool BUILT = ON && NLW >= 3 && DPL % 2 == 0 && !SWEEP_U32 &&
                                  (SWEEP_LINE_NOBAR ? RPW <= FIT : LEAD + RPW <= FIT) &&
                                  G::CW % 2 == 0 && G::HB % RPW == 0 && RPW >= 1;
    template <typename CT>
    static constexpr int lpf()
    {
        return largest_divisor_upto(G::CW / 2, VL == 8 ? 9 : sizeof(CT) == 1 ? SWEEP_LPF8 : SWEEP_LPF16);
    }
};
template <int VL, int DPL, int NCW_, int MODE>
constexpr int sweep_threads()
{
    using LG = LineGeo<VL, DPL, NCW_, MODE>;
    return SweepGeo<VL, DPL, NCW_>::THREADS + 64 * (LG::NLW - (LG::HPOLL ? 1 : 0));
}

template <int NP>
__device__ __forceinline__ void lds_get_pk(const uint16_t* p, uint32_t (&v)[NP])
{
    if constexpr (NP % 4 == 0) {
#pragma unroll
        for (int k = 0; k < NP / 4; k++) {
            const uint4 q = reinterpret_cast<const uint4*>(p)[k];
            v[4 * k] = q.x; v[4 * k + 1] = q.y; v[4 * k + 2] = q.z; v[4 * k + 3] = q.w;
        }
    } else if constexpr (NP % 2 == 0) {
#pragma unroll
        for (int k = 0; k < NP / 2; k++) {
            const uint2 q = reinterpret_cast<const uint2*>(p)[k];
            v[2 * k] = q.x; v[2 * k + 1] = q.y;
        }
    } else {
#pragma unroll
        for (int k = 0; k < NP; k++) v[k] = reinterpret_cast<const uint32_t*>(p)[k];
    }
}

template <int NP>
__device__ __forceinline__ void lds_put_pk(uint16_t* p, const uint32_t (&v)[NP])
{
    if constexpr (NP % 4 == 0) {
#pragma unroll
        for (int k = 0; k < NP / 4; k++)
            reinterpret_cast<uint4*>(p)[k] = make_uint4(v[4 * k], v[4 * k + 1], v[4 * k + 2], v[4 * k + 3]);
    } else if constexpr (NP % 2 == 0) {
#pragma unroll
        for (int k = 0; k < NP / 2; k++) reinterpret_cast<uint2*>(p)[k] = make_uint2(v[2 * k], v[2 * k + 1]);
    } else {
#pragma unroll
        for (int k = 0; k < NP; k++) reinterpret_cast<uint32_t*>(p)[k] = v[k];
    }
}

template <int DPL>
__device__ __forceinline__ void lds_put(uint16_t* p, const uint32_t (&v)[DPL])
{
    if constexpr (DPL % 2 == 0) {
        uint32_t w[DPL / 2];
#pragma unroll
        for (int k = 0; k < DPL / 2; k++) w[k] = __builtin_amdgcn_perm(v[2 * k + 1], v[2 * k], 0x05040100u);
        if constexpr (DPL % 8 == 0) {
#pragma unroll
            for (int k = 0; k < DPL / 8; k++)
                reinterpret_cast<uint4*>(p)[k] = make_uint4(w[4 * k], w[4 * k + 1], w[4 * k + 2], w[4 * k + 3]);
        } else if constexpr (DPL % 4 == 0) {
#pragma unroll
            for (int k = 0; k < DPL / 4; k++) reinterpret_cast<uint2*>(p)[k] = make_uint2(w[2 * k], w[2 * k + 1]);
        } else {
#pragma unroll
            for (int k = 0; k < DPL / 2; k++) reinterpret_cast<uint32_t*>(p)[k] = w[k];
        }
    } else {
#pragma unroll
        for (int i = 0; i < DPL; i++) p[i] = (uint16_t)v[i];
    }
}

template <int DPL>
__device__ __forceinline__ void lds_get(const uint16_t* p, uint32_t (&v)[DPL])
{
    if constexpr (DPL % 8 == 0) {
#pragma unroll
        for (int k = 0; k < DPL / 8; k++) {
            const uint4 q = reinterpret_cast<const uint4*>(p)[k];
            const uint32_t w[4] = {q.x, q.y, q.z, q.w};
#pragma unroll
            for (int j = 0; j < 4; j++) {
                v[8 * k + 2 * j] = w[j] & 0xFFFFu;
                v[8 * k + 2 * j + 1] = w[j] >> 16;
            }
        }
    } else if constexpr (DPL % 4 == 0) {
#pragma unroll
        for (int k = 0; k < DPL / 4; k++) {
            const uint2 q = reinterpret_cast<const uint2*>(p)[k];
            v[4 * k] = q.x & 0xFFFFu;
            v[4 * k + 1] = q.x >> 16;
            v[4 * k + 2] = q.y & 0xFFFFu;
            v[4 * k + 3] = q.y >> 16;
        }
    } else if constexpr (DPL % 2 == 0) {
#pragma unroll
        for (int k = 0; k < DPL / 2; k++) {
            const uint32_t q = reinterpret_cast<const uint32_t*>(p)[k];
            v[2 * k] = q & 0xFFFFu;
            v[2 * k + 1] = q >> 16;
        }
    } else {
#pragma unroll
        for (int i = 0; i < DPL; i++) v[i] = p[i];
    }
}

template <typename CT, int DPL>
__device__ __forceinline__ void unpack_ct(const RawBytes<DPL * (int)sizeof(CT)>& r, uint32_t (&C)[DPL])
{
#pragma unroll
    for (int i = 0; i < DPL; i++) C[i] = r.template get<CT>(i);
}

__device__ __forceinline__ void lds_barrier()
{
    __builtin_amdgcn_fence(__ATOMIC_RELEASE, "workgroup", "local");
    __builtin_amdgcn_s_barrier();
    __builtin_amdgcn_fence(__ATOMIC_ACQUIRE, "workgroup", "local");
}

#ifndef SWEEP_EARLY_XCHG
#define SWEEP_EARLY_XCHG 1
#endif

template <int N>
__device__ __forceinline__ void poll_set(const gu64* const (&src)[N], const bool (&need)[N], uint32_t tag,
                                         uint32_t (&v)[N], bool& dead, uint32_t* err)
{
    for (uint32_t spins = 0;; spins++) {
        unsigned long long x[N];
#pragma unroll
        for (int k = 0; k < N; k++) x[k] = __hip_atomic_load(src[k], __ATOMIC_RELAXED, __HIP_MEMORY_SCOPE_AGENT);
        bool ok = true;
#pragma unroll
        for (int k = 0; k < N; k++) {
            v[k] = (uint32_t)x[k];
            ok &= !need[k] || (uint32_t)(x[k] >> 32) == tag;
        }
        if (__all(ok) || dead) return;
        if (spins >= SW_SPIN_LIMIT) {
            if ((threadIdx.x & 63) == 0) atomicOr(err, 1u);
            dead = true;
            return;
        }
        __builtin_amdgcn_s_sleep(2);
    }
}

template <int N>
__device__ __forceinline__ void poll_granules(const gu64* src, bool need, uint32_t tag, uint32_t (&v)[N], bool& dead,
                                              uint32_t* err)
{
    const gu64* p[N];
    bool nd[N];
#pragma unroll
    for (int k = 0; k < N; k++) {
        p[k] = src + k;
        nd[k] = need;
    }
    poll_set<N>(p, nd, tag, v, dead, err);
}

template <int VL, int DPL, typename CT, int MODE, int NCW_ = kNarrowNcw>
__global__ void __launch_bounds__((sweep_threads<VL, DPL, NCW_, MODE>())) k_sweep(SweepArgs a)
{
    using G = SweepGeo<VL, DPL, NCW_>;
    using LG = LineGeo<VL, DPL, NCW_, MODE, (int)sizeof(CT)>;
    constexpr bool UP = MODE == 2 || MODE == 4;
    constexpr bool WTA = MODE == 1 || MODE == 2 || MODE == 4;
    constexpr bool EWIN = MODE == 1 || MODE == 2;
    constexpr bool PARTR = MODE == 2 || MODE == 4;
    constexpr bool LINES = MODE == 3;
    constexpr bool HPOLL = LG::HPOLL;
    static_assert(!LINES || LG::BUILT, "MODE 3 instance not built for this geometry");
    static_assert(MODE < 3 || (DPL % 2 == 0 && !SWEEP_U32), "MODES 3 / 4 run the packed row loops only");
    constexpr int NTH = sweep_threads<VL, DPL, NCW_, MODE>();
#ifndef SWEEP_PRIO
#define SWEEP_PRIO 2
#endif
#ifndef SWEEP_DYNPRIO
#define SWEEP_DYNPRIO 1
#endif
    constexpr int PRIO_HI = 3, PRIO_LO = MODE == 0 ? 2 : 1;
    if constexpr (MODE == 0 && SWEEP_PRIO > 0) __builtin_amdgcn_s_setprio(SWEEP_PRIO);
    constexpr bool ROWSYNC = SWEEP_ROW_SYNC && (MODE != 1 || SWEEP_ROWSYNC_M1);
    constexpr bool NOBAR = sweep_nobar<DPL, MODE>();
    static_assert(!LINES || ROWSYNC, "the line waves mirror the row-synchronised barrier pattern");
    constexpr int LPW = G::LPW, NCW = G::NCW, HB = G::HB, NCOL = G::NCOL, COLS = G::COLS, CW = G::CW, D = G::D;
    constexpr int NG = G::NG, SNG = G::SNG, PF = G::PF, HM = G::HM, HW = G::HW;
    constexpr int CB = DPL * (int)sizeof(CT);
    constexpr bool IL = sweep_il<CT, DPL>();
    constexpr int NPW = DPL / 2 > 0 ? DPL / 2 : 1;
    __shared__ __attribute__((aligned(16))) uint16_t lv[2][2][COLS][D];
    __shared__ uint32_t lmin[2][2][COLS];
    __shared__ __attribute__((aligned(16))) uint16_t srow[WTA ? NCW - 2 : 1][WTA ? LPW : 1][WTA ? D : 2];
    __shared__ uint32_t rowcnt[NCW];
    constexpr int RING_D = LINES ? D : 2;
    __shared__ __attribute__((aligned(16))) uint16_t ring_pad[(LINES ? LG::LR : 1) * (LINES ? CW : 1) * RING_D + 2 * RING_D];
    auto& ring = *reinterpret_cast<uint16_t(*)[LINES ? LG::LR : 1][LINES ? CW : 1][RING_D]>(ring_pad + RING_D);
    __shared__ __attribute__((aligned(8))) uint32_t roff[LINES && LG::DSO ? LG::LR : 1][LINES && LG::DSO ? CW : 1][2];
    __shared__ uint32_t linecnt[LINES ? LG::NLW : 1], conscnt[NCW];
    __shared__ uint32_t pollcnt;

    int bx = blockIdx.x, by = blockIdx.y;
    if (a.xcd_per > 0) {
        const int item = (int)(blockIdx.x & 7u) * a.xcd_per + (int)(blockIdx.x >> 3);
        if (item >= a.xcd_total) return;
        const int per_pair = a.nwg * (a.nband > 1 ? a.nband : 1);
        by = item / per_pair;
        bx = item - by * per_pair;
    }
    const int nband = LINES && a.nband > 1 ? a.nband : 1;
    const int band = nband > 1 ? bx / a.nwg : 0;
    const int wg = bx - band * a.nwg, pair = by;
    const int H = a.H, W1 = a.W1;
    const int y0b = nband > 1 ? band * a.band_h : 0;
    const int y1b = nband > 1 ? min(H, y0b + a.band_h) : H;
    const int ys = band > 0 ? max(0, y0b - a.vwarm) : 0;
    const int nrow = y1b - ys, wrows = y0b - ys;
    const int nblk = (nrow + HB - 1) / HB;
    const int nblk_rec = nband > 1 ? a.hop_nblk : nblk;
    const bool vguess = a.vguess && band > 0;
    auto in_domain_slot = [&](int q) { const int x = wg * CW + (q - 1) - HW; return x >= 0 && x < W1; };

    for (int i = threadIdx.x; i < 2 * 2 * COLS * D / 2; i += NTH) {
        uint32_t v = 0;
        if (vguess) {
            const int q = (i / (D / 2)) % COLS, wi = i % (D / 2);
            const int d0 = IL ? wi / NPW * DPL + pk_disp<NPW, IL>(wi % NPW, 0) : 2 * wi;
            const int d1 = IL ? wi / NPW * DPL + pk_disp<NPW, IL>(wi % NPW, 1) : 2 * wi + 1;
            if (in_domain_slot(q)) v = (uint32_t)(d0 % 5 + 3 * (q & 1)) | ((uint32_t)(d1 % 5 + 3 * (q & 1)) << 16);
        }
        reinterpret_cast<uint32_t*>(&lv[0][0][0][0])[i] = v;
    }
    for (int i = threadIdx.x; i < 2 * 2 * COLS; i += NTH) {
        const int q = i % COLS;
        (&lmin[0][0][0])[i] = vguess && in_domain_slot(q) ? (uint32_t)(3 * (q & 1)) * 0x10001u : 0u;
    }
    for (int i = threadIdx.x; i < NCW; i += NTH) rowcnt[i] = conscnt[i] = 0;
    if (threadIdx.x == 0) pollcnt = 0;

    if constexpr (LINES)
        for (int i = threadIdx.x; i < LG::NLW; i += NTH) linecnt[i] = 0;
    __syncthreads();

    const int lane = threadIdx.x & 63, wave = threadIdx.x >> 6;
    const bool has_left = wg > 0, has_right = wg + 1 < a.nwg;
    const uint32_t tag0 = a.epoch << 16;
    unsigned long long* hopp = a.hop + (size_t)pair * a.hop_pair;
    auto gbase = [&](int strip, int dir, int b) -> size_t {
        return ((size_t)((band * a.nwg + strip) * 2 + dir) * nblk_rec + b) * SNG;
    };

    if (!HPOLL && wave == NCW) {
        constexpr int NDAT = G::NDAT;
        constexpr int GPL = (2 * SNG + 63) / 64;
        int gdir[GPL], grec[GPL];
        bool gneed[GPL];
#pragma unroll
        for (int k = 0; k < GPL; k++) {
            const int r2 = k * 64 + lane;
            gdir[k] = r2 >= SNG ? 1 : 0;
            grec[k] = r2 - gdir[k] * SNG;
            gneed[k] = r2 < 2 * SNG && (gdir[k] == 0 ? has_left : has_right);
        }
        bool dead = (a.dbg & 1) != 0;
        [[maybe_unused]] uint64_t st_poll = 0, st_bar = 0;
        SW_T0(st_life);
        const bool xchg = (has_left || has_right) && !(a.dbg & 2);
        for (int b = 0; b < nblk; b++) {
            uint32_t v[GPL];
            auto poll = [&]() {
                if (b + 1 < nblk && xchg) {
                    const gu64* src[GPL];
#pragma unroll
                    for (int k = 0; k < GPL; k++)
                        src[k] = (const gu64*)(hopp + gbase(gneed[k] ? wg + (gdir[k] ? 1 : -1) : wg, gdir[k], b) + grec[k]);
                    SW_T0(tp);
                    poll_set<GPL>(src, gneed, tag0 | (uint32_t)(b + 1), v, dead, a.err);
                    SW_ACC(st_poll, tp);
#if SWEEP_STATS
                    if (a.stats && (lane == 0 || lane == 32)) {
                        const int dir = lane == 0 ? 0 : 1;
                        if (dir == 0 ? has_left : has_right)
                            a.stats[1024 + 3 * 65536 + (size_t)MODE * 65536 +
                                    ((size_t)(pair * a.nwg + wg + (dir ? 1 : -1)) * 2 + dir) * nblk + b] =
                                __builtin_amdgcn_s_memrealtime();
                    }
#endif
                }
            };
            if (NOBAR) {
                poll();
                SW_T0(tb);
                const uint32_t need = (uint32_t)((b + 1) * HB);
                for (uint32_t spins = 0; !(a.dbg & 4); spins++) {
                    const uint32_t n0 = __builtin_amdgcn_readfirstlane(
                        __hip_atomic_load(&rowcnt[0], __ATOMIC_RELAXED, __HIP_MEMORY_SCOPE_WORKGROUP));
                    const uint32_t n1 = __builtin_amdgcn_readfirstlane(
                        __hip_atomic_load(&rowcnt[NCW - 1], __ATOMIC_RELAXED, __HIP_MEMORY_SCOPE_WORKGROUP));
                    if (min(n0, n1) >= need) {
                        __builtin_amdgcn_fence(__ATOMIC_ACQUIRE, "workgroup", "local");
                        break;
                    }
                    if (spins >= SW_SPIN_LIMIT) {
                        if (lane == 0) atomicOr(a.err, 1u);
                        break;
                    }
                    __builtin_amdgcn_s_sleep(1);
                }
                SW_ACC(st_bar, tb);
            } else if (ROWSYNC) {
                if (SWEEP_EARLY_XCHG == 2) poll();
                SW_T0(tb);
                if (!(a.dbg & 4)) lds_barrier();
                SW_ACC(st_bar, tb);
            } else {
#pragma unroll 1
                for (int j = 0; j < HB; j++) {
                    if (SWEEP_EARLY_XCHG == 2 && j == HB - 1) poll();
                    if (!(a.dbg & 4)) lds_barrier();
                }
            }
// ... 173 lines not shown
                    uint32_t m = Lp[0];
#pragma unroll
                    for (int i = 1; i < NP; i++) m = pk_min(m, Lp[i]);
                    m = min(m & 0xFFFFu, m >> 16);
                    mm = group_min<VL>(m) * 0x10001u;
                }
                auto chunk = [&](int j0, auto ring_c) {
                    constexpr int RING = decltype(ring_c)::value;
#pragma unroll
                    for (int k = 0; k < LPF; k++) {
                        const int j = j0 + k;
#pragma unroll
                        for (int q = 0; q < RawBytes<CB>::WORDS; q++) asm volatile("" : "+v"(cr[k].w[q]) : "v"(mm));
                        uint32_t C[1][NP];
                        unpack_vol_pk<CT, DPL, IL>(cr[k], C[0]);
#pragma unroll
                        for (int i = 0; i < NP; i++) asm volatile("" : "+v"(C[0][i])::"memory");
                        cr[k].load(rc, coff_at(j + LPF));
                        uint32_t Lq[1][NP], mq[1] = {mm}, Ln[1][NP], mn[1];
#pragma unroll
                        for (int i = 0; i < NP; i++) Lq[0][i] = Lp[i];
                        sweep_step2n<VL, NP, H16, 1, DSL, IL>(Lq, mq, C, P1p, P2p, eL, eR, Ln, mn);
#pragma unroll
                        for (int i = 0; i < NP; i++) Lp[i] = Ln[0][i];
                        if constexpr (DSL && RING != 0) {
#if SWEEP_DS_LANE0
                            if (g == 0) rop[(j - w) * ostep] = mq[0];
#else
                            rop[(j - w) * ostep] = mq[0];
#endif
                        }
                        mm = mn[0];
                        if constexpr (RING != 0) {
                            uint16_t* p = rp + (j - w) * rstep;
                            if constexpr (RING == 2) {
                                uint32_t v[NP];
#pragma unroll
                                for (int i = 0; i < NP; i++) v[i] = pk_add(old[i], Lp[i]);
                                lds_put_pk<NP>(p, v);
                                lds_get_pk<NP>(p + rstep, old);
                            } else {
                                lds_put_pk<NP>(p, Lp);
                            }
                        }
                        if constexpr (DSL) {
                            if (k == LPF - 1) {
#pragma unroll
                                for (int i = 0; i < NP; i++) Lp[i] = pk_sub(Lp[i], mm);
                                mm = 0;
                            }
                        }
                    }
                };
                const int half = CW / 2 / LPF;
                auto min0 = [&](uint32_t (&v)[NP]) {
#pragma unroll
                    for (int i = 0; i < NP; i++) v[i] = DSL ? Lp[i] : pk_sub(Lp[i], mm);
                };
                uint32_t sv[NP];
                for (int c = 0; c < wch; c++) chunk(c * LPF, std::integral_constant<int, 0>{});
                min0(sv);
                store_vol_pk<CT, NP, IL>(rs, so, sv);
                for (int c = 0; c < half; c++) chunk(w + c * LPF, std::integral_constant<int, 1>{});
                lds_get_pk<NP>(rp + (CW / 2) * rstep, old);
                for (int c = 0; c < half; c++) chunk(w + (half + c) * LPF, std::integral_constant<int, 2>{});
                min0(sv);
                store_vol_pk<CT, NP, IL>(rs, yl ? so + (uint32_t)(D * sizeof(CT)) : kOOB, sv);
                __builtin_amdgcn_fence(__ATOMIC_RELEASE, "workgroup", "local");
                __hip_atomic_store(&linecnt[li], (uint32_t)(t + 1), __ATOMIC_RELAXED, __HIP_MEMORY_SCOPE_WORKGROUP);
            }
            barriers_to(0x7FFFFFFF);
#if SWEEP_STATS
            if (a.stats && lane == 0) {
                atomicAdd(a.stats + 41, (unsigned long long)lst_cons);
                atomicAdd(a.stats + 42, (unsigned long long)lst_bar);
                atomicAdd(a.stats + 43, (unsigned long long)(__builtin_readcyclecounter() - lst_life));
                atomicAdd(a.stats + 44, 1ull);
            }
#endif
            return;
        }
    }

    const int kl = lane / VL, g = lane % VL;
    const int c = wave == 0 ? kl : wave == NCW - 1 ? NCOL - HW + kl : HW + (wave - 1) * LPW + kl;
    const int x1 = wg * CW + c - HW;
    const bool active = x1 >= 0 && x1 < W1;
    const bool halo_l = wave == 0, halo_r = wave == NCW - 1, own = !halo_l && !halo_r;
    const int wx0 = wg * CW + wave * LPW - LPW;
    const bool wave_ragged = wx0 < 0 || wx0 + LPW > W1;
    const uint32_t P1 = (uint32_t)a.P1, P2 = (uint32_t)a.P2;
    const int wl = wave > 0 ? wave - 1 : wave, wr = wave < NCW - 1 ? wave + 1 : wave;
    bool sync_dead = (a.dbg & 4) != 0;
    auto publish_row = [&](int s) {
        __hip_atomic_store(&rowcnt[wave], (uint32_t)(s + 1), __ATOMIC_RELEASE, __HIP_MEMORY_SCOPE_WORKGROUP);
    };
    [[maybe_unused]] uint64_t st_wait = 0, st_bbar = 0;
    SW_T0(st_clife);
    auto wait_row_spin = [&](int s) {
        for (uint32_t spins = 0;; spins++) {
            const uint32_t nl = __builtin_amdgcn_readfirstlane(
                __hip_atomic_load(&rowcnt[wl], __ATOMIC_RELAXED, __HIP_MEMORY_SCOPE_WORKGROUP));
            const uint32_t nr = __builtin_amdgcn_readfirstlane(
                __hip_atomic_load(&rowcnt[wr], __ATOMIC_RELAXED, __HIP_MEMORY_SCOPE_WORKGROUP));
            if (min(nl, nr) >= (uint32_t)s) {
                __builtin_amdgcn_fence(__ATOMIC_ACQUIRE, "workgroup", "local");
                return;
            }
            if (spins >= SW_SPIN_LIMIT) {
                if (lane == 0) atomicOr(a.err, 1u);
                sync_dead = true;
                return;
            }
            if (SWEEP_ROW_SLEEP) __builtin_amdgcn_s_sleep(SWEEP_ROW_SLEEP);
        }
    };
    auto wait_row = [&](int s) {
        if (sync_dead) return;
        SW_T0(tw);
        wait_row_spin(s);
        SW_ACC(st_wait, tw);
    };
    [[maybe_unused]] uint64_t st_wl = 0;
    auto wait_lines_spin = [&](int s) {
        if constexpr (LINES) {
            const int li = (s / LG::RPW) % LG::NLW;
            const uint32_t need = (uint32_t)(s / (LG::RPW * LG::NLW) + 1);
            for (uint32_t spins = 0;; spins++) {
                const uint32_t nd = __builtin_amdgcn_readfirstlane(
                    __hip_atomic_load(&linecnt[li], __ATOMIC_RELAXED, __HIP_MEMORY_SCOPE_WORKGROUP));
                if (nd >= need) {
                    __builtin_amdgcn_fence(__ATOMIC_ACQUIRE, "workgroup", "local");
                    return;
                }
                if (spins >= SW_SPIN_LIMIT) {
                    if (lane == 0) atomicOr(a.err, 1u);
                    return;
                }
                __builtin_amdgcn_s_sleep(1);
            }
        } else {
            (void)s;
        }
    };
    auto wait_lines = [&](int s) {
        SW_T0(twl);
        wait_lines_spin(s);
        SW_ACC(st_wl, twl);
    };
    auto wait_poll = [&](int b) {
        if constexpr (NOBAR) {
            for (uint32_t spins = 0; !sync_dead; spins++) {
                const uint32_t n = __builtin_amdgcn_readfirstlane(
                    __hip_atomic_load(&pollcnt, __ATOMIC_RELAXED, __HIP_MEMORY_SCOPE_WORKGROUP));
                if (n >= (uint32_t)b) {
                    __builtin_amdgcn_fence(__ATOMIC_ACQUIRE, "workgroup", "local");
                    return;
                }
                if (spins >= SW_SPIN_LIMIT) {
                    if (lane == 0) atomicOr(a.err, 1u);
                    sync_dead = true;
                    return;
                }
                __builtin_amdgcn_s_sleep(1);
            }
        } else {
            (void)b;
        }
    };
    auto end_row = [&](int j, int s) {
        if (!ROWSYNC || j == HB - 1) {
            if (!(a.dbg & 4)) lds_barrier();
        } else {
            publish_row(s);
        }
    };

    const uint64_t cells = (uint64_t)H * W1 * D;
    const rsrc_t rc = make_rsrc(a.cost + (size_t)pair * a.cost_pair, cells * sizeof(CT));
    rsrc_t re = make_rsrc(nullptr, 0), rw = re, rp = re, rrec = re, rnb = re;
    if constexpr (EWIN) {
        re = make_rsrc(a.ew + (size_t)pair * a.ew_pair, cells * sizeof(CT));
        rw = make_rsrc(a.ew + (size_t)pair * a.ew_pair + a.ew_slot, cells * sizeof(CT));
    }
    if constexpr (WTA) {
        rrec = make_rsrc(a.rec + (size_t)pair * H * a.W, (uint64_t)H * a.W * 4);
        rnb = make_rsrc(a.nb + (size_t)pair * H * a.W, (uint64_t)H * a.W * 4);
    }
    const int ku = 100 - a.uniq;
    if constexpr (MODE != 1) rp = make_rsrc((const uint8_t*)a.part + (size_t)pair * a.part_pair, cells * 2);
    const rsrc_t rhop = make_rsrc(hopp, (uint64_t)a.hop_pair * 8);
    constexpr uint32_t NONE = 0xFFFFFFFFu;
    auto cell = [&](int y) -> uint32_t {
        return active ? ((uint32_t)y * (uint32_t)W1 + (uint32_t)x1) * (uint32_t)D + (uint32_t)(g * DPL) : NONE;
    };
    auto boff = [&](uint32_t e, int bytes) -> uint32_t { return e == NONE ? kOOB : e * (uint32_t)bytes; };

    uint32_t LV[DPL];
#pragma unroll
    for (int i = 0; i < DPL; i++) LV[i] = 0;
    uint32_t mV = 0;

    RawBytes<CB> rc_[PF], re_[PF], rw_[PF];
    RawBytes<DPL * 2> rp_[PF];
    auto issue = [&](int k, int s) {
        const uint32_t en = s < H ? cell(UP ? H - 1 - s : s) : NONE;
        const uint32_t eo = own ? en : NONE;
        rc_[k].template load<WTA ? SWEEP_COST_AUX : 0>(rc, boff(en, sizeof(CT)));
        if constexpr (EWIN) {
            re_[k].template load<SWEEP_STREAM_AUX>(re, boff(eo, sizeof(CT)));
            rw_[k].template load<SWEEP_STREAM_AUX>(rw, boff(eo, sizeof(CT)));
        }
        if constexpr (PARTR) rp_[k].template load<SWEEP_STREAM_AUX>(rp, boff(eo, 2));
    };
    if constexpr (DPL % 2 == 0 && !SWEEP_U32) {
        constexpr int NP = DPL / 2;
        const uint32_t P1p = P1 * 0x10001u, P2p = P2 * 0x10001u;
        constexpr uint32_t EDGE2 = (sizeof(CT) == 1 && SWEEP_H16) ? 0x7BFF7BFFu : (kBig | (kBig << 16));
        const uint32_t eL = g == 0 ? EDGE2 : 0u, eR = g == VL - 1 ? EDGE2 : 0u;
        constexpr bool SAT = sizeof(CT) == 2;
        constexpr bool H16 = !SAT && SWEEP_H16;
        constexpr bool DS = H16 && SWEEP_DS;
        const bool pil = IL && (MODE == 3 || MODE == 4) && a.part_il != 0;
        static_assert(!DS || SWEEP_STEPN, "deferred subtraction runs the stage-wise steps");
        auto run = [&](auto role_c) {
            constexpr int ROLE = decltype(role_c)::value;
            constexpr bool HAS_A = ROLE != 2, HAS_B = ROLE != 0, OWN = ROLE == 1;
            constexpr int NS = OWN ? 1 : HM;
            auto cell_h = [&](int h, int y) -> uint32_t {
                const int xh = x1 + h * LPW;
                return xh >= 0 && xh < W1 ? ((uint32_t)y * (uint32_t)W1 + (uint32_t)xh) * (uint32_t)D + (uint32_t)(g * DPL)
                                          : NONE;
            };
            RawBytes<CB> rcs[PF][NS];
            auto issue_r = [&](int k, int s) {
                const int yy = UP ? H - 1 - s : ys + s;
#pragma unroll
                for (int h = 0; h < NS; h++)
                    rcs[k][h].template load<WTA ? SWEEP_COST_AUX : 0>(rc, boff(s < nrow ? cell_h(h, yy) : NONE, sizeof(CT)));
                if constexpr (OWN && EWIN) {
                    const uint32_t en = s < nrow ? cell(yy) : NONE;
                    re_[k].template load<SWEEP_STREAM_AUX>(re, boff(en, sizeof(CT)));
                    rw_[k].template load<SWEEP_STREAM_AUX>(rw, boff(en, sizeof(CT)));
                }
                if constexpr (OWN && PARTR) rp_[k].template load<SWEEP_STREAM_AUX>(rp, boff(s < nrow ? cell(yy) : NONE, 2));
            };
#pragma unroll
            for (int k = 0; k < PF; k++) issue_r(k, k);
            uint32_t LVp[NP];
#pragma unroll
            for (int i = 0; i < NP; i++) LVp[i] = 0;
            uint32_t mVl = 0;
            if (vguess && OWN && active) {
                const uint32_t o = (uint32_t)(3 * ((c + 1) & 1));
#pragma unroll
                for (int i = 0; i < NP; i++) {
                    const int d0 = g * DPL + pk_disp<NP, IL>(i, 0), d1 = g * DPL + pk_disp<NP, IL>(i, 1);
                    LVp[i] = ((uint32_t)(d0 % 5) + o) | (((uint32_t)(d1 % 5) + o) << 16);
                }
                mVl = o * 0x10001u;
            }
            auto vstore = [&](int which, const uint32_t (&sV)[NP], uint32_t mV_, const uint32_t (&sA)[NP], uint32_t mA_,
                              const uint32_t (&sB)[NP], uint32_t mB_) {
                if constexpr (LINES && OWN) {
                    const rsrc_t rv = make_rsrc(a.vst + (size_t)pair * a.vst_pair, a.vst_pair);
                    auto off = [&](int dir) -> uint32_t {
                        return active ? (((((uint32_t)band * 2u + (uint32_t)which) * 3u + (uint32_t)dir) * (uint32_t)W1 +
                                          (uint32_t)x1) * (uint32_t)D + (uint32_t)(g * DPL)) * (uint32_t)sizeof(CT)
                                      : kOOB;
                    };
                    uint32_t v[NP];
#pragma unroll
                    for (int i = 0; i < NP; i++) v[i] = pk_sub(sV[i], mV_);
                    store_vol_pk<CT, NP, IL>(rv, off(0), v);
#pragma unroll
                    for (int i = 0; i < NP; i++) v[i] = pk_sub(sA[i], mA_);
                    store_vol_pk<CT, NP, IL>(rv, off(1), v);
#pragma unroll
                    for (int i = 0; i < NP; i++) v[i] = pk_sub(sB[i], mB_);
                    store_vol_pk<CT, NP, IL>(rv, off(2), v);
                }
            };
            uint32_t dpk[NP];
#pragma unroll
            for (int i = 0; i < NP; i++)
                dpk[i] = (uint32_t)(g * DPL + pk_disp<NP, IL>(i, 0) + 1) * 0x10001u +
                         ((uint32_t)(pk_disp<NP, IL>(i, 1) - pk_disp<NP, IL>(i, 0)) << 16);
            if constexpr (SWEEP_DYNPRIO && !OWN) __builtin_amdgcn_s_setprio(PRIO_HI);
            for (int b = 0; b < nblk; b++) {
#pragma unroll
                for (int j = 0; j < HB; j++) {
                    const int k = j % PF;
                    const int s = b * HB + j;
                    if constexpr (SWEEP_DYNPRIO && OWN) __builtin_amdgcn_s_setprio(PRIO_HI);
                    const bool live = s < nrow;
                    const int y = UP ? H - 1 - s : ys + s;
                    const int rb = (s + 1) & 1, wb = s & 1;
                    const uint32_t e = live ? cell(y) : NONE;
                    uint32_t C[NS][NP], Ein[NP], Win[NP], Pin[NP];
#pragma unroll
                    for (int h = 0; h < NS; h++) unpack_vol_pk<CT, DPL, IL>(rcs[k][h], C[h]);
                    if constexpr (OWN && EWIN) {
                        unpack_vol_pk<CT, DPL, IL>(re_[k], Ein);
                        unpack_vol_pk<CT, DPL, IL>(rw_[k], Win);
                    }
                    if constexpr (OWN && PARTR) {
                        if (pil) {
#pragma unroll
                            for (int i = 0; i < NP; i++) Pin[i] = rp_[k].w[i];
                        } else {
                            unpack_vol_pk<uint16_t, DPL, IL>(rp_[k], Pin);
                            if constexpr (IL) asm volatile("");
                        }
                    }
#pragma unroll
                    for (int i = 0; i < NP; i++) {
#pragma unroll
                        for (int h = 0; h < NS; h++) asm volatile("" : "+v"(C[h][i])::"memory");
                        if constexpr (OWN && EWIN) asm volatile("" : "+v"(Ein[i]), "+v"(Win[i])::"memory");
                        if constexpr (OWN && PARTR) asm volatile("" : "+v"(Pin[i])::"memory");
                    }
                    issue_r(k, s + PF);
                    if (ROWSYNC && (j > 0 || NOBAR)) wait_row(s);
                    uint32_t LA[NS][NP], LB[NS][NP], mA[NS], mB[NS];
#pragma unroll
                    for (int h = 0; h < NS; h++) {
                        const int ch = c + h * LPW;
                        if constexpr (HAS_A) {
                            lds_get_pk<NP>(&lv[rb][0][ch][g * DPL], LA[h]);
                            mA[h] = lmin[rb][0][ch];
                        }
                        if constexpr (HAS_B) {
                            lds_get_pk<NP>(&lv[rb][1][ch + 2][g * DPL], LB[h]);
                            mB[h] = lmin[rb][1][ch + 2];
                        }
                    }
                    if constexpr (SWEEP_LDS_FIRST && MODE == 1) __builtin_amdgcn_sched_barrier(0);
                    uint32_t nV[NP], nA[NS][NP], nB[NS][NP], mnV = 0, mnA[NS], mnB[NS];
                    auto step = [&](const uint32_t(&Lp)[NP], uint32_t m, const uint32_t(&Ch)[NP], uint32_t(&Ln)[NP]) {
                        return sweep_step2<VL, NP, H16, DS, IL>(Lp, m, Ch, P1p, P2p, eL, eR, Ln);
                    };
                    if constexpr (OWN) {
                        if constexpr (SWEEP_STEPN) {
                            uint32_t Lp1[1][NP], m1[1] = {mVl}, C1[1][NP], Ln1[1][NP], mn1[1];
#pragma unroll
                            for (int i = 0; i < NP; i++) {
                                Lp1[0][i] = LVp[i];
                                C1[0][i] = C[0][i];
                            }
                            sweep_step2n<VL, NP, H16, 1, DS, IL>(Lp1, m1, C1, P1p, P2p, eL, eR, Ln1, mn1);
#pragma unroll
                            for (int i = 0; i < NP; i++) nV[i] = Ln1[0][i];
                            mnV = mn1[0];
                        } else {
                            mnV = step(LVp, mVl, C[0], nV);
                        }
                    }
                    if constexpr (SWEEP_STEPN && OWN && NS == 1) {
                        uint32_t Lp2[2][NP], m2[2], C2[2][NP], Ln2[2][NP], mn2[2];
#pragma unroll
                        for (int i = 0; i < NP; i++) {
                            Lp2[0][i] = LA[0][i];
                            Lp2[1][i] = LB[0][i];
                            C2[0][i] = C2[1][i] = C[0][i];
                        }
                        m2[0] = mA[0];
                        m2[1] = mB[0];
                        sweep_step2n<VL, NP, H16, 2, DS, IL>(Lp2, m2, C2, P1p, P2p, eL, eR, Ln2, mn2);
#pragma unroll
                        for (int i = 0; i < NP; i++) {
                            nA[0][i] = Ln2[0][i];
                            nB[0][i] = Ln2[1][i];
                        }
                        mnA[0] = mn2[0];
                        mnB[0] = mn2[1];
                    } else if constexpr (SWEEP_STEPN && !OWN && NS > 1) {
                        uint32_t Lpn[NS][NP], mn_in[NS], Lnn[NS][NP], mnn[NS];
#pragma unroll
                        for (int h = 0; h < NS; h++) {
                            if constexpr (HAS_A) {
#pragma unroll
                                for (int i = 0; i < NP; i++) Lpn[h][i] = LA[h][i];
                                mn_in[h] = mA[h];
                            } else {
#pragma unroll
                                for (int i = 0; i < NP; i++) Lpn[h][i] = LB[h][i];
                                mn_in[h] = mB[h];
                            }
                        }
                        sweep_step2n<VL, NP, H16, NS, DS, IL>(Lpn, mn_in, C, P1p, P2p, eL, eR, Lnn, mnn);
#pragma unroll
                        for (int h = 0; h < NS; h++) {
#pragma unroll
                            for (int i = 0; i < NP; i++) {
                                if constexpr (HAS_A) nA[h][i] = Lnn[h][i];
                                else nB[h][i] = Lnn[h][i];
                            }
                            if constexpr (HAS_A) mnA[h] = mnn[h];
                            else mnB[h] = mnn[h];
                        }
                    } else {
#pragma unroll
                        for (int h = 0; h < NS; h++) {
                            if constexpr (HAS_A) mnA[h] = step(LA[h], mA[h], C[h], nA[h]);
// ... 189 lines not shown
                                if constexpr (EWIN) {
#pragma unroll
                                    for (int i = 0; i < NP; i++) ew[i] = pk_add(Ein[i], Win[i]);
                                    if constexpr (PARTR) {
#pragma unroll
                                        for (int i = 0; i < NP; i++) ew[i] = pk_add(ew[i], Pin[i]);
                                    }
                                } else {
#pragma unroll
                                    for (int i = 0; i < NP; i++) ew[i] = Pin[i];
                                }
#pragma unroll
                                for (int i = 0; i < NP; i++) Sp[i] = pk_add(nV[i], nA[0][i]);
#pragma unroll
                                for (int i = 0; i < NP; i++) ew[i] = pk_add(nB[0][i], ew[i]);
#pragma unroll
                                for (int i = 0; i < NP; i++) Sp[i] = pk_add(Sp[i], ew[i]);
                                if constexpr (DS) {
#pragma unroll
                                    for (int i = 0; i < NP; i++) Sp[i] = pk_sub(Sp[i], offs);
                                }
                            }
                            uint32_t key = 0xFFFFFFFFu;
#pragma unroll
                            for (int i = 0; i < NP; i++)
                                key = min(key, min((Sp[i] << 16) | wta_rank(g * DPL + pk_disp<NP, IL>(i, 0), MODE == 1),
                                                   (Sp[i] & 0xFFFF0000u) | wta_rank(g * DPL + pk_disp<NP, IL>(i, 1), MODE == 1)));
                            asm volatile("" ::: "memory");
                            lds_put_pk<NP>(&srow[(wave - 1) % (NCW - 2)][kl][g * DPL], Sp);
                            asm volatile("" ::: "memory");
                            key = group_min<VL>(key);
                            const uint32_t minS = key >> 16;
                            const int best = wta_unrank(key & 0xFFFF, MODE == 1);
                            auto srow_at = [&](int d) -> int {
                                if constexpr (!IL) return d;
                                else if constexpr ((DPL & (DPL - 1)) == 0 && NP > 1) {
                                    uint32_t hb, ro, r;
                                    asm("v_bfe_u32 %0, %1, %2, 1" : "=v"(hb) : "v"(d), "n"(__builtin_ctz(NP)));
                                    asm("v_lshl_or_b32 %0, %1, 1, %2" : "=v"(ro) : "v"(d), "v"(hb));
                                    asm("v_bfi_b32 %0, %1, %2, %3" : "=v"(r) : "n"(DPL - 1), "v"(ro), "v"(d));
                                    return (int)r;
                                } else return d / DPL * DPL + pk_slot<NP, IL>(d % DPL);
                            };
                            const int bm = srow_at(max(best - 1, 0)), bq = srow_at(min(best + 1, D - 1));
                            const uint32_t Sm = srow[(wave - 1) % (NCW - 2)][kl][bm];
                            const uint32_t Sq = srow[(wave - 1) % (NCW - 2)][kl][bq];
                            const uint32_t bm1p = (uint32_t)best * 0x10001u;
                            uint32_t tw[NP];
#pragma unroll
                            for (int i = 0; i < NP; i++) tw[i] = pk_sub(dpk[i], bm1p);
#pragma unroll
                            for (int i = 0; i < NP; i++) tw[i] = pkw(__builtin_elementwise_sub_sat(pkv(0x00030003u), pkv(tw[i])));
#pragma unroll
                            for (int i = 0; i < NP; i++) tw[i] = pk_window_push(tw[i], Sp[i]);
                            uint32_t m2p = tw[0];
#pragma unroll
                            for (int i = 1; i < NP; i++) m2p = pk_min(m2p, tw[i]);
                            const uint32_t m2 = group_min<VL>(min(m2p & 0xFFFFu, m2p >> 16));
                            const bool ok = !(__mul24((int)m2, ku) < __mul24((int)minS, 100) && (!pad || m2 <= 32767u)) &&
                                            minS < 32767u;
                            const uint32_t recw = ok ? ((minS << 16) | (uint32_t)best) : 0xFFFFFFFFu;
                            const uint32_t nbw = Sm | (Sq << 16);
                            const bool wpx = g == 0 && active && live;
                            const uint32_t px = (uint32_t)y * (uint32_t)a.W + (uint32_t)(x1 + a.minX1);
                            __builtin_amdgcn_raw_buffer_store_b32(recw, rrec, wpx ? px * 4 : kOOB, 0, 0);
                            __builtin_amdgcn_raw_buffer_store_b32(nbw, rnb, wpx ? px * 4 : kOOB, 0, 0);
                        }
                    }
                }
                if (b + 1 < nblk && !HPOLL) {
                    SW_T0(tb);
                    if constexpr (NOBAR) wait_poll(b + 1);
                    else lds_barrier();
                    SW_ACC(st_bbar, tb);
                }
            }
#if SWEEP_STATS
            if (a.stats && lane == 0) {
                atomicAdd(a.stats + 8 * MODE + 2, (unsigned long long)st_wait);
                atomicAdd(a.stats + 8 * MODE + 3, (unsigned long long)st_bbar);
                atomicAdd(a.stats + 8 * MODE + 4, (unsigned long long)(__builtin_readcyclecounter() - st_clife));
                atomicAdd(a.stats + 8 * MODE + 5, 1ull);
                if (LINES) atomicAdd(a.stats + 40, (unsigned long long)st_wl);
            }
#endif
        };
        if (halo_l) run(std::integral_constant<int, 0>{});
        else if (halo_r) run(std::integral_constant<int, 2>{});
        else run(std::integral_constant<int, 1>{});
        return;
    }

#pragma unroll
    for (int k = 0; k < PF; k++) issue(k, k);
    for (int b = 0; b < nblk; b++) {
#pragma unroll
        for (int j = 0; j < HB; j++) {
            const int k = j % PF;
            const int s = b * HB + j;
            const bool live = s < H;
            const int y = UP ? H - 1 - s : s;
            const int rb = (s + 1) & 1, wb = s & 1;
            const uint32_t e = live ? cell(y) : NONE;
            uint32_t C[DPL];
            unpack_ct<CT, DPL>(rc_[k], C);
            uint32_t Ein[DPL], Win[DPL], Pin[DPL];
#pragma unroll
            for (int i = 0; i < DPL; i++) Ein[i] = Win[i] = Pin[i] = 0;
            if constexpr (EWIN) {
                unpack_ct<CT, DPL>(re_[k], Ein);
                unpack_ct<CT, DPL>(rw_[k], Win);
            }
            if constexpr (PARTR) unpack_ct<uint16_t, DPL>(rp_[k], Pin);
#pragma unroll
            for (int i = 0; i < DPL; i++) {
                asm volatile("" : "+v"(C[i])::"memory");
                if constexpr (EWIN) asm volatile("" : "+v"(Ein[i]), "+v"(Win[i])::"memory");
                if constexpr (PARTR) asm volatile("" : "+v"(Pin[i])::"memory");
            }
            issue(k, s + PF);

            if (ROWSYNC && j > 0) wait_row(s);
            uint32_t nA[DPL], nB[DPL];
            uint32_t mnA = 0, mnB = 0;
            if (!halo_r) {
                uint32_t LA[DPL];
                lds_get<DPL>(&lv[rb][0][c][g * DPL], LA);
                mnA = sweep_step<VL, DPL>(LA, lmin[rb][0][c], C, P1, P2, nA);
                if (wave_ragged) {
#pragma unroll
                    for (int i = 0; i < DPL; i++) nA[i] = active ? nA[i] : 0u;
                    mnA = active ? mnA : 0u;
                }
                lds_put<DPL>(&lv[wb][0][c + 1][g * DPL], nA);
                if (g == 0) lmin[wb][0][c + 1] = mnA;
            }
            if (!halo_l) {
                uint32_t LB[DPL];
                lds_get<DPL>(&lv[rb][1][c + 2][g * DPL], LB);
                mnB = sweep_step<VL, DPL>(LB, lmin[rb][1][c + 2], C, P1, P2, nB);
                if (wave_ragged) {
#pragma unroll
                    for (int i = 0; i < DPL; i++) nB[i] = active ? nB[i] : 0u;
                    mnB = active ? mnB : 0u;
                }
                lds_put<DPL>(&lv[wb][1][c + 1][g * DPL], nB);
                if (g == 0) lmin[wb][1][c + 1] = mnB;
            }
            if (j == HB - 1 && b + 1 < nblk) {
                const bool pa = wave == NCW - 2 && has_right, pb = wave == 1 && has_left;
                if (pa || pb) {
                    const uint32_t tag = tag0 | (uint32_t)(b + 1);
                    const size_t rec = gbase(wg, pa ? 0 : 1, b);
#pragma unroll
                    for (int q = 0; q < NG; q++) {
                        const uint32_t lo = pa ? nA[2 * q] : nB[2 * q];
                        const uint32_t hi = 2 * q + 1 < DPL ? (pa ? nA[2 * q + 1] : nB[2 * q + 1]) : 0u;
                        __builtin_amdgcn_raw_buffer_store_b64(u32x2{lo | (hi << 16), tag}, rhop,
                                                              (uint32_t)((rec + (size_t)(q * HW + kl) * VL + g) * 8), 0, 16);
                    }
                    if (g == 0)
                        __builtin_amdgcn_raw_buffer_store_b64(u32x2{pa ? mnA : mnB, tag}, rhop,
                                                              (uint32_t)((rec + G::NDAT + kl) * 8), 0, 16);
                }
            }

// ... 129 lines not shown
```

### stereo_match_amd/csrc/sm_sweep_host.hpp

```cpp
#pragma once
#include <hip/hip_runtime.h>
#include <stdint.h>

namespace smk {

#ifndef SWEEP_STATS
#define SWEEP_STATS 0
#endif

#ifndef SWEEP_IL
#define SWEEP_IL 1
#endif

constexpr int EWS_MAXN = 4;
constexpr int EWS_KSHIFT = 3;

struct SweepArgs {
    const uint8_t* cost;
    size_t cost_pair;
    const uint8_t* ew;
    size_t ew_pair, ew_slot;
    uint16_t* part;
    size_t part_pair;
    unsigned long long* hop;
    size_t hop_pair;
    uint32_t* rec;
    uint32_t* nb;
    uint32_t* err;
    int H, W, W1, D, minD, minX1, P1, P2, uniq;
    int Dv;
    float inv_ku;
    int nwg;
    uint32_t epoch;
    int dbg;
    unsigned long long* stats;
    uint8_t* st;
    size_t st_pair;
    int ewarm;
    int ewguess;
    int ewstart;
    int nband, band_h, vwarm;
    int vguess;
    int hop_nblk;
    uint8_t* vst;
    size_t vst_pair;
    int xcd_per, xcd_total;
    int part_il;
};


struct SweepInfo {
    int cw;
    int hb;
    int ngr;
    int threads;
    int blocks_per_cu;
    int impl;
    int dpl;
    int ncw;
};

template <typename CT, int MODE, class F>
hipError_t with_d(int D, F& f);

hipError_t sweep_info_m0(int D, int ct_bytes, int variant, int device, SweepInfo* out);
hipError_t sweep_info_m1(int D, int ct_bytes, int variant, int device, SweepInfo* out);
hipError_t sweep_info_m2(int D, int ct_bytes, int variant, int device, SweepInfo* out);
hipError_t sweep_info_m3(int D, int ct_bytes, int variant, int device, SweepInfo* out);
hipError_t sweep_info_m4(int D, int ct_bytes, int variant, int device, SweepInfo* out);
hipError_t sweep_info_wide_m0(int D, int ct_bytes, int device, SweepInfo* out);
hipError_t sweep_info_wide_m1(int D, int ct_bytes, int device, SweepInfo* out);
hipError_t sweep_info_wide_m2(int D, int ct_bytes, int device, SweepInfo* out);
hipError_t sweep_info_wide_m3(int D, int ct_bytes, int device, SweepInfo* out);
hipError_t sweep_info_wide_m4(int D, int ct_bytes, int device, SweepInfo* out);
hipError_t sweep_info_lat_m0(int D, int ct_bytes, int device, SweepInfo* out);
hipError_t sweep_info_lat_m1(int D, int ct_bytes, int device, SweepInfo* out);
hipError_t sweep_info_lat_m2(int D, int ct_bytes, int device, SweepInfo* out);
hipError_t sweep_info_lat_m3(int D, int ct_bytes, int device, SweepInfo* out);
hipError_t sweep_info_lat_m4(int D, int ct_bytes, int device, SweepInfo* out);
hipError_t sweep_launch_lat_m0(int D, int ct_bytes, const SweepArgs& a, int npairs, hipStream_t stream);
hipError_t sweep_launch_lat_m1(int D, int ct_bytes, const SweepArgs& a, int npairs, hipStream_t stream);
hipError_t sweep_launch_lat_m2(int D, int ct_bytes, const SweepArgs& a, int npairs, hipStream_t stream);
hipError_t sweep_launch_lat_m3(int D, int ct_bytes, const SweepArgs& a, int npairs, hipStream_t stream);
hipError_t sweep_launch_lat_m4(int D, int ct_bytes, const SweepArgs& a, int npairs, hipStream_t stream);
hipError_t sweep_launch_m0(int D, int ct_bytes, int variant, const SweepArgs& a, int npairs, hipStream_t stream);
hipError_t sweep_launch_m1(int D, int ct_bytes, int variant, const SweepArgs& a, int npairs, hipStream_t stream);
hipError_t sweep_launch_m2(int D, int ct_bytes, int variant, const SweepArgs& a, int npairs, hipStream_t stream);
hipError_t sweep_launch_m3(int D, int ct_bytes, int variant, const SweepArgs& a, int npairs, hipStream_t stream);
hipError_t sweep_launch_m4(int D, int ct_bytes, int variant, const SweepArgs& a, int npairs, hipStream_t stream);
hipError_t sweep_launch_wide_m0(int D, int ct_bytes, const SweepArgs& a, int npairs, hipStream_t stream);
hipError_t sweep_launch_wide_m1(int D, int ct_bytes, const SweepArgs& a, int npairs, hipStream_t stream);
hipError_t sweep_launch_wide_m2(int D, int ct_bytes, const SweepArgs& a, int npairs, hipStream_t stream);
hipError_t sweep_launch_wide_m3(int D, int ct_bytes, const SweepArgs& a, int npairs, hipStream_t stream);
hipError_t sweep_launch_wide_m4(int D, int ct_bytes, const SweepArgs& a, int npairs, hipStream_t stream);

inline hipError_t sweep_info(int D, int ct_bytes, int mode, int variant, int device, SweepInfo* out)
{
    typedef hipError_t (*InfoW)(int, int, int, SweepInfo*);
    typedef hipError_t (*InfoV)(int, int, int, int, SweepInfo*);
    static const InfoW lat[5] = {sweep_info_lat_m0, sweep_info_lat_m1, sweep_info_lat_m2, sweep_info_lat_m3,
                                 sweep_info_lat_m4};
    static const InfoW wide[5] = {sweep_info_wide_m0, sweep_info_wide_m1, sweep_info_wide_m2, sweep_info_wide_m3,
                                  sweep_info_wide_m4};
    static const InfoV narrow[5] = {sweep_info_m0, sweep_info_m1, sweep_info_m2, sweep_info_m3, sweep_info_m4};
    if (mode < 0 || mode > 4) return hipErrorInvalidValue;
    if (variant == 2) return lat[mode](D, ct_bytes, device, out);
    if (variant == 0) {
        const hipError_t e = wide[mode](D, ct_bytes, device, out);
        if (e == hipSuccess) return e;
    }
    return narrow[mode](D, ct_bytes, variant == 1 ? 0 : variant, device, out);
}
inline hipError_t sweep_launch(int D, int ct_bytes, int mode, int impl, const SweepArgs& a, int npairs,
                               hipStream_t stream)
{
    typedef hipError_t (*LaunchW)(int, int, const SweepArgs&, int, hipStream_t);
    typedef hipError_t (*LaunchV)(int, int, int, const SweepArgs&, int, hipStream_t);
    static const LaunchW lat[5] = {sweep_launch_lat_m0, sweep_launch_lat_m1, sweep_launch_lat_m2, sweep_launch_lat_m3,
                                   sweep_launch_lat_m4};
    static const LaunchW wide[5] = {sweep_launch_wide_m0, sweep_launch_wide_m1, sweep_launch_wide_m2,
                                    sweep_launch_wide_m3, sweep_launch_wide_m4};
    static const LaunchV narrow[5] = {sweep_launch_m0, sweep_launch_m1, sweep_launch_m2, sweep_launch_m3,
                                      sweep_launch_m4};
    if (mode < 0 || mode > 4) return hipErrorInvalidValue;
    if (impl == 2) return lat[mode](D, ct_bytes, a, npairs, stream);
    if (impl == 1) return wide[mode](D, ct_bytes, a, npairs, stream);
    return narrow[mode](D, ct_bytes, impl, a, npairs, stream);
}
hipError_t lr_rows_launch(const uint32_t* rec, const uint32_t* nb, int16_t* out, int16_t* wta, int G, int H, int W,
                          int D, int minD, int minX1, int maxX1, int disp12, const uint32_t* guard, hipStream_t stream);

struct EwArgs {
    const uint8_t* cost;
    size_t cost_pair;
    uint8_t* out;
    size_t out_pair, out_slot;
    int H, W1, P1, P2;
    int nrb;
    int wpb;
    int prio;
};
hipError_t ew_launch(int D, int ct_bytes, int vl, EwArgs a, int npairs, hipStream_t stream);

struct EwPatchArgs {
    const uint8_t* cost;
    size_t cost_pair;
    uint16_t* part;
    size_t part_pair;
    uint8_t* st;
    size_t st_pair;
    int H, W1, nwg, cw, P1, P2;
    const uint32_t* guard;
    unsigned long long* fixes;
    int atom;
    int part_il;
};
struct BandPatchArgs {
    const uint8_t* cost;
    size_t cost_pair;
    uint16_t* part;
    size_t part_pair;
    const uint8_t* vst;
    size_t vst_pair;
    int H, W1, nband, band_h, P1, P2;
    int nbx;
    const uint32_t* guard;
    unsigned long long* fixes;
};
hipError_t band_patch_launch(int D, int ct_bytes, const BandPatchArgs& a, int npairs, hipStream_t stream);

constexpr int kPatchMaxChunks = 8;
constexpr int patch_max_strips(int D) { return 1 + kPatchMaxChunks * (D % 32 == 0 ? 4 : 8) * 8; }
hipError_t ew_patch_launch(int D, int ct_bytes, const EwPatchArgs& a, int npairs, hipStream_t stream);

}
```

Baseline: 6994.

## Fuse E/W patch pass into final sweep kernel with per-row readiness flags

Moves the horizontal E/W patch work into extra patch waves inside the mode-4 sweep kernel, a new mode 5. Patch waves process rows bottom-up and publish per-row flags, and the sweep's row loads wait on a workgroup-local patched_upto counter. This removes a separate patch kernel launch and its serialization before the sweep, so the two can overlap. In exchange it adds waves per workgroup, which may reduce occupancy, and adds spin-wait synchronization. A tuning knob allows forcing or disabling the fused path.

```diff
diff --git a/include/stereo_match_amd.h b/include/stereo_match_amd.h
--- a/include/stereo_match_amd.h
+++ b/include/stereo_match_amd.h
@@ -264,6 +264,7 @@
 #define SM_TUNE_SWEEP_XCD 13
 #define SM_TUNE_PLY_STAGE 14
 #define SM_TUNE_EW_START 15
+#define SM_TUNE_EW_PATCH 16
 int sm_set_tuning(sm_ctx* ctx, int key, int value);
 
 const char* sm_last_error(sm_ctx* ctx);
diff --git a/stereo_match_amd/_lib.py b/stereo_match_amd/_lib.py
--- a/stereo_match_amd/_lib.py
+++ b/stereo_match_amd/_lib.py
@@ -738,6 +738,7 @@
     TUNE_BANDS, TUNE_BAND_WARMUP, TUNE_BAND_GUESS, TUNE_COST_WGS, TUNE_LR_STAGGER, TUNE_SWEEP_XCD = 8, 9, 10, 11, 12, 13
     TUNE_PLY_STAGE = 14
     TUNE_EW_START = 15
+    TUNE_EW_PATCH = 16
 
     def set_tuning(self, key: int, value: int):
         self._check(self._lib.sm_set_tuning(self.ctx, int(key), int(value)))
diff --git a/stereo_match_amd/csrc/sm_api.hip b/stereo_match_amd/csrc/sm_api.hip
--- a/stereo_match_amd/csrc/sm_api.hip
+++ b/stereo_match_amd/csrc/sm_api.hip
@@ -136,6 +136,7 @@
     int tune_ew_warmup = 0, tune_sweep_lines = 0;
     int tune_ew_guess = 0;
     int tune_ew_start = 0;
+    int tune_ew_patch = 0;
     int tune_bands = 0, tune_band_warmup = 0, tune_band_guess = 0;
     int tune_cost_wgs = 0;
     int tune_ply_stage = 0;
@@ -642,6 +643,8 @@
     int ewguess = 0;
     int ewstart = 0;
     int part_il = 0;
+    unsigned long long* fixes = nullptr;
+    int pnwg = 0, pcw = 0;
     int nband = 1, band_h = 0, vwarm = 0, vguess = 0;
     uint8_t* vst = nullptr;
     size_t vst_pair = 0;
@@ -759,7 +762,8 @@
     const int nb = banded ? j.nband : 1;
     const int nblk = banded ? (j.band_h + j.vwarm + si.hb - 1) / si.hb : (g.H + si.hb - 1) / si.hb;
     const int per_launch = (ctx->dbg_flags & DBG_SWEEP1) ? 1 : std::max(1, std::min(j.G, cap / (nwg * nb)));
-    const size_t hop_pair = (size_t)nwg * nb * 2 * nblk * si.ngr;
+    const size_t hop_snap = (size_t)nwg * nb * 2 * nblk * si.ngr;
+    const size_t hop_pair = hop_snap + (mode == 5 ? (size_t)g.H : 0);
     const size_t hop_bytes = hop_pair * 8 * per_launch;
     if (hop_pair * 8 > smk::kMaxRecords) return fail(ctx, SM_E_UNSUPPORTED, "sweep: boundary buffer too large");
     int rc;
@@ -791,6 +795,10 @@
         a.ewguess = j.ewguess;
         a.ewstart = j.ewstart;
         a.part_il = j.part_il;
+        a.fixes = mode == 5 ? j.fixes : nullptr;
+        a.flag_off = mode == 5 ? hop_snap : 0;
+        a.pnwg = j.pnwg;
+        a.pcw = j.pcw;
         a.nband = nb;
         a.band_h = j.band_h;
         a.vwarm = j.vwarm;
@@ -1007,6 +1015,8 @@
     return elem_bytes(n) == 1 ? 16 : 24;
 }
 
+constexpr bool kEwPatchInSweep = true;
+
 int run_lines(sm_ctx* ctx, const Norm& n, const Geo& g, BufSet& bs, hipStream_t ws, uint32_t* gflag)
 {
     const int G = g.G;
@@ -1045,6 +1055,16 @@
     ctx->line_groups++;
     ctx->line_strips += (long long)f.nwg * G;
     const bool fb_side = n.ndirs == 5 && ws == ctx->stream && !(ctx->dbg_flags & DBG_NO_FALLBACK);
+    bool patch_in_sweep = false;
+    if (n.ndirs == 8 && et == 1 && j.part_il && j.nband <= 1 && !(ctx->dbg_flags & DBG_SWEEP1) &&
+        (ctx->tune_ew_patch > 0 || (ctx->tune_ew_patch == 0 && kEwPatchInSweep))) {
+        SweepFit f5, f4;
+        patch_in_sweep = sweep_capacity(ctx, n, 5, G, f5) && f5.si.impl == 1 && f5.cap / std::max(f5.nwg, 1) >= G;
+        if (patch_in_sweep && ctx->tune_ew_patch == 0)
+            patch_in_sweep = sweep_capacity(ctx, n, 4, G, f4) && f4.si.impl == 1 && f4.si.ncw == f5.si.ncw;
+        j.pnwg = f.nwg;
+        j.pcw = f.si.cw;
+    }
     {
         StageTimer t(ctx, ctx->stream, SM_STAGE_PATHS, G);
         {
@@ -1103,10 +1123,11 @@
             if (rc != SM_OK) return rc;
             HIP_TRY(ctx, hipEventRecord(ctx->ev_fb_join, ctx->side));
         }
-        if (!ew_side) {
+        if (!ew_side && !patch_in_sweep) {
             StageTimer th(ctx, ctx->stream, SM_STAGE_HORIZONTAL, G);
             if ((rc = ew_patch(ctx->stream)) != SM_OK) return rc;
         }
+        j.fixes = pa.fixes;
         if (j.nband > 1) {
             smk::BandPatchArgs ba{};
             ba.cost = j.cost;
@@ -1143,7 +1164,7 @@
             StreamSwap sw(ctx, ws);
             StageTimer t(ctx, ctx->stream, SM_STAGE_WTA, G);
             StageTimer ts(ctx, ctx->stream, SM_STAGE_SWEEP_WTA, G);
-            if ((rc = sweep_pass(ctx, n, g, j, 4)) != SM_OK) return rc;
+            if ((rc = sweep_pass(ctx, n, g, j, patch_in_sweep ? 5 : 4)) != SM_OK) return rc;
         }
         return sweep_finish(ctx, n, g, bs, ws, gflag);
     }
@@ -3807,6 +3828,10 @@
             return fail(ctx, SM_E_ARG, "E/W start state %d: -1, 0, 1 or 2..%d cost columns", value, smk::EWS_MAXN);
         ctx->tune_ew_start = value;
         break;
+    case SM_TUNE_EW_PATCH:
+        if (value < -1 || value > 1) return fail(ctx, SM_E_ARG, "E/W patch placement %d: -1, 0 or 1", value);
+        ctx->tune_ew_patch = value;
+        break;
     case SM_TUNE_SWEEP_LINES:
         if (value < -1 || value > 1) return fail(ctx, SM_E_ARG, "sweep lines %d: -1, 0 or 1", value);
         ctx->tune_sweep_lines = value;
diff --git a/stereo_match_amd/csrc/sm_ew.hpp b/stereo_match_amd/csrc/sm_ew.hpp
--- a/stereo_match_amd/csrc/sm_ew.hpp
+++ b/stereo_match_amd/csrc/sm_ew.hpp
@@ -98,8 +98,8 @@
 #ifndef EW_PATCH_RC
 #define EW_PATCH_RC 0
 #endif
-template <int VL, int NP, typename CT, bool ATOM = false>
-__global__ void __launch_bounds__(256) k_ew_patch(EwPatchArgs a)
+template <int VL, int NP, typename CT, bool ATOM = false, bool PUB = false, int RC_ = 0>
+__device__ __forceinline__ void ew_patch_row(const EwPatchArgs& a, size_t pair, int y, int dir0, int dir1, uint64_t* openm)
 {
     constexpr int LPW = 64 / VL, DPL = 2 * NP, D = VL * DPL;
     constexpr int CB = DPL * (int)sizeof(CT);
@@ -108,16 +108,12 @@
     constexpr uint32_t EDGE = H16 ? 0x7BFF7BFFu : (kBig | (kBig << 16));
     constexpr int KU = 8;
     constexpr int CHUNK = LPW * KU;
-    constexpr int RC = EW_PATCH_RC ? EW_PATCH_RC : sizeof(CT) == 1 ? 8 : 16;
-    if (a.guard && __hip_atomic_load(a.guard, __ATOMIC_RELAXED, __HIP_MEMORY_SCOPE_AGENT) != 0u) return;
-    const int lane = threadIdx.x & 63, wave = threadIdx.x >> 6;
+    constexpr int RC = RC_ ? RC_ : EW_PATCH_RC ? EW_PATCH_RC : sizeof(CT) == 1 ? 8 : 16;
+    constexpr int PAUX = PUB ? 16 : 0;
+    static_assert(!(PUB && ATOM), "the published pass reads and writes the partial itself");
+    const int lane = threadIdx.x & 63;
     const int g = lane % VL, kl = lane / VL;
-    const int yw = (int)blockIdx.x * 4 + wave;
-    const int y = ATOM ? yw >> 1 : yw;
-    const int dir0 = ATOM ? (yw & 1) : 0, dir1 = ATOM ? dir0 + 1 : 2;
-    const size_t pair = blockIdx.y;
     const int H = a.H, W1 = a.W1, nwg = a.nwg, CW = a.cw;
-    if (y >= H) return;
     const uint64_t cells = (uint64_t)H * W1 * D;
     const rsrc_t rc = make_rsrc(a.cost + pair * a.cost_pair, cells * sizeof(CT));
     const rsrc_t rp = make_rsrc((const uint8_t*)a.part + pair * a.part_pair, cells * 2);
@@ -163,7 +159,7 @@
         auto issue1 = [&](int u, int o) {
             const int c = dir ? x0 + CW - 1 - o : x0 + o;
             cc[u].load(rc, o < ncol ? cell(c) * (uint32_t)sizeof(CT) : kOOB);
-            if constexpr (!ATOM) pb[u].load(rp, o < ncol ? cell(c) * 2u : kOOB);
+            if constexpr (!ATOM) pb[u].template load<PAUX>(rp, o < ncol ? cell(c) * 2u : kOOB);
         };
         auto issue = [&](int o0) {
 #pragma unroll
@@ -229,7 +225,7 @@
 #pragma unroll
                     for (int q = 0; q < NP; q++) P[q] = t[q];
                 }
-                if constexpr (!ATOM) bstore_n<uint32_t, NP>(rp, cell(c) * 2u, P);
+                if constexpr (!ATOM) bstore_n<uint32_t, NP, PAUX>(rp, cell(c) * 2u, P);
 #pragma unroll
                 for (int q = 0; q < NP; q++) {
                     Lq[0][q] = Ln[0][q];
@@ -279,7 +275,7 @@
         auto issue1 = [&](int u, int o) {
             const int c = dir ? x0 + CW - 1 - o : x0 + o;
             cc[u].load(rc, o < ncol ? cell64(c) * (uint32_t)sizeof(CT) : kOOB);
-            if constexpr (!ATOM) pb[u].load(rp, o < ncol ? cell64(c) * 2u : kOOB);
+            if constexpr (!ATOM) pb[u].template load<PAUX>(rp, o < ncol ? cell64(c) * 2u : kOOB);
         };
         auto issue = [&](int o0) {
 #pragma unroll
@@ -333,7 +329,7 @@
                         P[q] = pk_add(pk_sub(pv_[q], Ln[0][q]), Ln[1][q]);
                     }
                 }
-                if constexpr (!ATOM) bstore_n<uint32_t, NPW>(rp, cell64(c) * 2u, P);
+                if constexpr (!ATOM) bstore_n<uint32_t, NPW, PAUX>(rp, cell64(c) * 2u, P);
 #pragma unroll
                 for (int q = 0; q < NPW; q++) {
                     Lq[0][q] = Ln[0][q];
@@ -363,7 +359,6 @@
         __builtin_amdgcn_fence(__ATOMIC_RELEASE, "workgroup");
         __builtin_amdgcn_fence(__ATOMIC_ACQUIRE, "workgroup");
     };
-    __shared__ uint64_t openm[4][kPatchMaxChunks];
     uint32_t nfix = 0, nopen = 0;
     for (int dir = dir0; dir < dir1; dir++) {
         auto strip_of = [&](int i) { return dir ? nwg - 1 - i : i; };
@@ -407,7 +402,7 @@
             }
             open = lines_or(open);
             nopen += (uint32_t)__builtin_popcountll(open);
-            if (lane == 0) openm[wave][ch] = open;
+            if (lane == 0) openm[ch] = open;
             if (open && first_open == nwg) first_open = i0 + __builtin_ctzll(open);
         }
         if (first_open < nwg && !EW_PATCH_NO_CARRY && D % 128 == 0 && EW_PATCH_B64 && !pil) {
@@ -423,7 +418,7 @@
                     nfix += r != 2 && kl == 0;
                     if (r != 0) carry = false;
                 }
-                const bool open_i = ((openm[wave][(i - 1) / CHUNK] >> ((i - 1) % CHUNK)) & 1ull) != 0;
+                const bool open_i = ((openm[(i - 1) / CHUNK] >> ((i - 1) % CHUNK)) & 1ull) != 0;
                 if (!carry && open_i) {
                     load_state64(soff64(k, dir, 0), T);
                     carry = true;
@@ -443,7 +438,7 @@
                         nfix += r != 2;
                         if (r != 0) carry = false;
                     }
-                    const bool open_i = ((openm[wave][(i - 1) / CHUNK] >> ((i - 1) % CHUNK)) & 1ull) != 0;
+                    const bool open_i = ((openm[(i - 1) / CHUNK] >> ((i - 1) % CHUNK)) & 1ull) != 0;
                     if (!carry && open_i) {
                         load_state(soff(k, dir, 0), T);
                         carry = true;
@@ -458,6 +453,19 @@
         if (lane == 0 && nfix) atomicAdd(a.fixes, (unsigned long long)nfix);
         if (lane == 0 && nopen) atomicAdd(a.fixes + 1, (unsigned long long)nopen);
     }
+}
+
+template <int VL, int NP, typename CT, bool ATOM = false>
+__global__ void __launch_bounds__(256) k_ew_patch(EwPatchArgs a)
+{
+    if (a.guard && __hip_atomic_load(a.guard, __ATOMIC_RELAXED, __HIP_MEMORY_SCOPE_AGENT) != 0u) return;
+    const int wave = threadIdx.x >> 6;
+    const int yw = (int)blockIdx.x * 4 + wave;
+    const int y = ATOM ? yw >> 1 : yw;
+    const int dir0 = ATOM ? (yw & 1) : 0, dir1 = ATOM ? dir0 + 1 : 2;
+    if (y >= a.H) return;
+    __shared__ uint64_t openm[4][kPatchMaxChunks];
+    ew_patch_row<VL, NP, CT, ATOM>(a, blockIdx.y, y, dir0, dir1, openm[wave]);
 }
 
 template <int VL, int NP, typename CT>
diff --git a/stereo_match_amd/csrc/sm_sweep.hip b/stereo_match_amd/csrc/sm_sweep.hip
--- a/stereo_match_amd/csrc/sm_sweep.hip
+++ b/stereo_match_amd/csrc/sm_sweep.hip
@@ -72,6 +72,13 @@
     else return true;
 }
 
+template <int VL, int DPL, typename CT, int MODE>
+constexpr int unit_npw()
+{
+    return SWEEP_WIDE == 1 && MODE == 4 && sizeof(CT) == 1 && VL == 16 && VL * DPL == 128 ? SWEEP_NPW : 0;
+}
+
+template <bool PATCH = false>
 struct InfoF {
     int device;
     SweepInfo* out;
@@ -79,12 +86,13 @@
     hipError_t run()
     {
         constexpr int NCW = unit_ncw<VL * DPL, CT>();
-        if constexpr (!unit_built<VL, DPL, CT, MODE>()) {
+        constexpr int NPW = PATCH ? unit_npw<VL, DPL, CT, MODE>() : 0;
+        if constexpr (!unit_built<VL, DPL, CT, MODE>() || (PATCH && NPW == 0)) {
             return hipErrorInvalidValue;
         } else {
             using SG = SweepGeo<VL, DPL, NCW>;
-            constexpr int THREADS = sweep_threads<VL, DPL, NCW, MODE>();
-            auto kern = k_sweep<VL, DPL, CT, MODE, NCW>;
+            constexpr int THREADS = sweep_threads<VL, DPL, NCW, MODE, NPW>();
+            auto kern = k_sweep<VL, DPL, CT, MODE, NCW, NPW>;
             static int per_cu = -1;
             if (per_cu < 0) {
                 int nb = 0;
@@ -108,6 +116,7 @@
     }
 };
 
+template <bool PATCH = false>
 struct LaunchF {
     const SweepArgs* a;
     dim3 grid;
@@ -116,11 +125,12 @@
     hipError_t run()
     {
         constexpr int NCW = unit_ncw<VL * DPL, CT>();
-        if constexpr (!unit_built<VL, DPL, CT, MODE>()) {
+        constexpr int NPW = PATCH ? unit_npw<VL, DPL, CT, MODE>() : 0;
+        if constexpr (!unit_built<VL, DPL, CT, MODE>() || (PATCH && NPW == 0)) {
             return hipErrorInvalidValue;
         } else {
-            hipLaunchKernelGGL((k_sweep<VL, DPL, CT, MODE, NCW>), grid, dim3(sweep_threads<VL, DPL, NCW, MODE>()), 0,
-                               stream, *a);
+            hipLaunchKernelGGL((k_sweep<VL, DPL, CT, MODE, NCW, NPW>), grid,
+                               dim3(sweep_threads<VL, DPL, NCW, MODE, NPW>()), 0, stream, *a);
             return hipGetLastError();
         }
     }
@@ -185,29 +195,44 @@
 #if SWEEP_WIDE == 2
 hipError_t SW_CAT(sweep_info_lat_m, SWEEP_MODE)(int D, int ct_bytes, int device, SweepInfo* out)
 {
-    InfoF f{device, out};
+    InfoF<> f{device, out};
     return with_sweep(D, ct_bytes, f);
 }
 
 hipError_t SW_CAT(sweep_launch_lat_m, SWEEP_MODE)(int D, int ct_bytes, const SweepArgs& a, int npairs,
                                                   hipStream_t stream)
 {
-    LaunchF f{&a, a.xcd_per > 0 ? dim3(8 * a.xcd_per, 1) : dim3(a.nwg * (a.nband > 1 ? a.nband : 1), npairs), stream};
+    LaunchF<> f{&a, a.xcd_per > 0 ? dim3(8 * a.xcd_per, 1) : dim3(a.nwg * (a.nband > 1 ? a.nband : 1), npairs), stream};
     return with_sweep(D, ct_bytes, f);
 }
 #elif SWEEP_WIDE
 hipError_t SW_CAT(sweep_info_wide_m, SWEEP_MODE)(int D, int ct_bytes, int device, SweepInfo* out)
 {
-    InfoF f{device, out};
+    InfoF<> f{device, out};
     return with_sweep(D, ct_bytes, f);
 }
 
 hipError_t SW_CAT(sweep_launch_wide_m, SWEEP_MODE)(int D, int ct_bytes, const SweepArgs& a, int npairs,
                                                    hipStream_t stream)
 {
-    LaunchF f{&a, a.xcd_per > 0 ? dim3(8 * a.xcd_per, 1) : dim3(a.nwg * (a.nband > 1 ? a.nband : 1), npairs), stream};
-    return with_sweep(D, ct_bytes, f);
-}
+    LaunchF<> f{&a, a.xcd_per > 0 ? dim3(8 * a.xcd_per, 1) : dim3(a.nwg * (a.nband > 1 ? a.nband : 1), npairs), stream};
+    return with_sweep(D, ct_bytes, f);
+}
+#if SWEEP_WIDE == 1 && SWEEP_MODE == 4
+hipError_t sweep_info_wide_m4p(int D, int ct_bytes, int device, SweepInfo* out)
+{
+    InfoF<true> f{device, out};
+    return with_sweep(D, ct_bytes, f);
+}
+
+hipError_t sweep_launch_wide_m4p(int D, int ct_bytes, const SweepArgs& a, int npairs, hipStream_t stream)
+{
+    if (!a.fixes || !a.st || a.flag_off == 0 || a.nband > 1 || a.pcw < 1 || a.pnwg < 1 || a.pnwg > patch_max_strips(D))
+        return hipErrorInvalidValue;
+    LaunchF<true> f{&a, a.xcd_per > 0 ? dim3(8 * a.xcd_per, 1) : dim3(a.nwg, npairs), stream};
+    return with_sweep(D, ct_bytes, f);
+}
+#endif
 #else
 hipError_t SW_CAT(sweep_info_m, SWEEP_MODE)(int D, int ct_bytes, int variant, int device, SweepInfo* out)
 {
@@ -217,7 +242,7 @@
 #else
     (void)variant;
 #endif
-    InfoF f{device, out};
+    InfoF<> f{device, out};
     return with_sweep(D, ct_bytes, f);
 }
 
@@ -232,7 +257,7 @@
 #else
     (void)variant;
 #endif
-    LaunchF f{&a, a.xcd_per > 0 ? dim3(8 * a.xcd_per, 1) : dim3(a.nwg * (a.nband > 1 ? a.nband : 1), npairs), stream};
+    LaunchF<> f{&a, a.xcd_per > 0 ? dim3(8 * a.xcd_per, 1) : dim3(a.nwg * (a.nband > 1 ? a.nband : 1), npairs), stream};
     return with_sweep(D, ct_bytes, f);
 }
 #endif
diff --git a/stereo_match_amd/csrc/sm_sweep.hpp b/stereo_match_amd/csrc/sm_sweep.hpp
--- a/stereo_match_amd/csrc/sm_sweep.hpp
+++ b/stereo_match_amd/csrc/sm_sweep.hpp
@@ -2,6 +2,7 @@
 #include "sm_common.hpp"
 #include "sm_sweep_host.hpp"
 #include "sm_pk.hpp"
+#include "sm_ew.hpp"
 
 #include <type_traits>
 
@@ -166,12 +167,20 @@
         return largest_divisor_upto(G::CW / 2, VL == 8 ? 9 : sizeof(CT) == 1 ? SWEEP_LPF8 : SWEEP_LPF16);
     }
 };
-template <int VL, int DPL, int NCW_, int MODE>
+template <int VL, int DPL, int NCW_, int MODE, int NPW = 0>
 constexpr int sweep_threads()
 {
     using LG = LineGeo<VL, DPL, NCW_, MODE>;
-    return SweepGeo<VL, DPL, NCW_>::THREADS + 64 * (LG::NLW - (LG::HPOLL ? 1 : 0));
+    return SweepGeo<VL, DPL, NCW_>::THREADS + 64 * (LG::NLW - (LG::HPOLL ? 1 : 0) + NPW);
 }
+
+#ifndef SWEEP_PATCH_PRIO
+#define SWEEP_PATCH_PRIO 0
+#endif
+#ifndef SWEEP_PATCH_RC
+#define SWEEP_PATCH_RC 0
+#endif
+constexpr int kPatchFirstRows = 16;
 
 template <int NP>
 __device__ __forceinline__ void lds_get_pk(const uint16_t* p, uint32_t (&v)[NP])
@@ -326,8 +335,8 @@
     poll_set<N>(p, nd, tag, v, dead, err);
 }
 
-template <int VL, int DPL, typename CT, int MODE, int NCW_ = kNarrowNcw>
-__global__ void __launch_bounds__((sweep_threads<VL, DPL, NCW_, MODE>())) k_sweep(SweepArgs a)
+template <int VL, int DPL, typename CT, int MODE, int NCW_ = kNarrowNcw, int NPW = 0>
+__global__ void __launch_bounds__((sweep_threads<VL, DPL, NCW_, MODE, NPW>())) k_sweep(SweepArgs a)
 {
     using G = SweepGeo<VL, DPL, NCW_>;
     using LG = LineGeo<VL, DPL, NCW_, MODE, (int)sizeof(CT)>;
@@ -339,7 +348,9 @@
     constexpr bool HPOLL = LG::HPOLL;
     static_assert(!LINES || LG::BUILT, "MODE 3 instance not built for this geometry");
     static_assert(MODE < 3 || (DPL % 2 == 0 && !SWEEP_U32), "MODES 3 / 4 run the packed row loops only");
-    constexpr int NTH = sweep_threads<VL, DPL, NCW_, MODE>();
+    constexpr int NTH = sweep_threads<VL, DPL, NCW_, MODE, NPW>();
+    static_assert(NPW == 0 || (MODE == 4 && HPOLL && sizeof(CT) == 1 && DPL % 2 == 0 && VL * DPL % 32 == 0 && VL == 16),
+                  "patch waves: the 8-path u8 up sweep on the patch pass's 16-lane lines, no poller wave");
 #ifndef SWEEP_PRIO
 #define SWEEP_PRIO 2
 #endif
@@ -355,7 +366,7 @@
     constexpr int NG = G::NG, SNG = G::SNG, PF = G::PF, HM = G::HM, HW = G::HW;
     constexpr int CB = DPL * (int)sizeof(CT);
     constexpr bool IL = sweep_il<CT, DPL>();
-    constexpr int NPW = DPL / 2 > 0 ? DPL / 2 : 1;
+    constexpr int NPL = DPL / 2 > 0 ? DPL / 2 : 1;
     __shared__ __attribute__((aligned(16))) uint16_t lv[2][2][COLS][D];
     __shared__ uint32_t lmin[2][2][COLS];
     __shared__ __attribute__((aligned(16))) uint16_t srow[WTA ? NCW - 2 : 1][WTA ? LPW : 1][WTA ? D : 2];
@@ -366,6 +377,8 @@
     __shared__ __attribute__((aligned(8))) uint32_t roff[LINES && LG::DSO ? LG::LR : 1][LINES && LG::DSO ? CW : 1][2];
     __shared__ uint32_t linecnt[LINES ? LG::NLW : 1], conscnt[NCW];
     __shared__ uint32_t pollcnt;
+    __shared__ uint64_t popen[NPW > 0 ? NPW : 1][NPW > 0 ? kPatchMaxChunks : 1];
+    __shared__ uint32_t patched_upto;
 
     int bx = blockIdx.x, by = blockIdx.y;
     if (a.xcd_per > 0) {
@@ -392,8 +405,8 @@
         uint32_t v = 0;
         if (vguess) {
             const int q = (i / (D / 2)) % COLS, wi = i % (D / 2);
-            const int d0 = IL ? wi / NPW * DPL + pk_disp<NPW, IL>(wi % NPW, 0) : 2 * wi;
-            const int d1 = IL ? wi / NPW * DPL + pk_disp<NPW, IL>(wi % NPW, 1) : 2 * wi + 1;
+            const int d0 = IL ? wi / NPL * DPL + pk_disp<NPL, IL>(wi % NPL, 0) : 2 * wi;
+            const int d1 = IL ? wi / NPL * DPL + pk_disp<NPL, IL>(wi % NPL, 1) : 2 * wi + 1;
             if (in_domain_slot(q)) v = (uint32_t)(d0 % 5 + 3 * (q & 1)) | ((uint32_t)(d1 % 5 + 3 * (q & 1)) << 16);
         }
         reinterpret_cast<uint32_t*>(&lv[0][0][0][0])[i] = v;
@@ -403,7 +416,7 @@
         (&lmin[0][0][0])[i] = vguess && in_domain_slot(q) ? (uint32_t)(3 * (q & 1)) * 0x10001u : 0u;
     }
     for (int i = threadIdx.x; i < NCW; i += NTH) rowcnt[i] = conscnt[i] = 0;
-    if (threadIdx.x == 0) pollcnt = 0;
+    if (threadIdx.x == 0) pollcnt = patched_upto = 0;
 
     if constexpr (LINES)
         for (int i = threadIdx.x; i < LG::NLW; i += NTH) linecnt[i] = 0;
@@ -743,6 +756,82 @@
         }
     }
 
+    if constexpr (NPW > 0) {
+        if (wave >= NCW) {
+            const int pw = __builtin_amdgcn_readfirstlane(wave) - NCW;
+            const bool poller = pw == NPW - 1;
+            __builtin_amdgcn_s_setprio(SWEEP_PATCH_PRIO);
+            SW_T0(pst_life);
+            EwPatchArgs pa{};
+            pa.cost = a.cost;
+            pa.cost_pair = a.cost_pair;
+            pa.part = a.part;
+            pa.part_pair = a.part_pair;
+            pa.st = a.st;
+            pa.st_pair = a.st_pair;
+            pa.H = H;
+            pa.W1 = W1;
+            pa.nwg = a.pnwg;
+            pa.cw = a.pcw;
+            pa.P1 = a.P1;
+            pa.P2 = a.P2;
+            pa.fixes = a.fixes;
+            pa.part_il = a.part_il;
+            const int nid = a.nwg * NPW, id = pw * a.nwg + wg;
+            gu64* const flags = (gu64*)(hopp + a.flag_off);
+            const uint32_t ftag = tag0 | 0xFFFFu;
+            const bool gaveup = __hip_atomic_load(a.err, __ATOMIC_RELAXED, __HIP_MEMORY_SCOPE_AGENT) != 0u;
+            uint32_t upto = 0;
+            bool pdead = (a.dbg & 1) != 0;
+            auto set_upto = [&](uint32_t v) {
+                __hip_atomic_store(&patched_upto, v, __ATOMIC_RELAXED, __HIP_MEMORY_SCOPE_WORKGROUP);
+            };
+            auto advance = [&](uint32_t target, bool block) {
+                if (!poller) return;
+                for (uint32_t spins = 0; upto < target && !pdead;) {
+                    const uint32_t idx = upto + (uint32_t)lane;
+                    const unsigned long long x =
+                        __hip_atomic_load(flags + min(idx, (uint32_t)(H - 1)), __ATOMIC_RELAXED, __HIP_MEMORY_SCOPE_AGENT);
+                    const bool ok = idx >= (uint32_t)H || (uint32_t)(x >> 32) == ftag;
+                    const unsigned long long nb = ~__ballot(ok);
+                    const uint32_t nset = nb ? (uint32_t)__builtin_ctzll(nb) : 64u;
+                    if (nset) {
+                        upto = min(upto + nset, (uint32_t)H);
+                        set_upto(upto);
+                        spins = 0;
+                        if (nset == 64u) continue;
+                    }
+                    if (!block) return;
+                    if (nset == 0u) {
+                        if (++spins >= SW_SPIN_LIMIT) {
+                            if (lane == 0) atomicOr(a.err, 1u);
+                            pdead = true;
+                            break;
+                        }
+                        __builtin_amdgcn_s_sleep(2);
+                    }
+                }
+                if (pdead) set_upto((uint32_t)H);
+            };
+            advance((uint32_t)min(H, min(kPatchFirstRows, (NPW - 1) * a.nwg)), true);
+            for (int i = id; i < H; i += nid) {
+                if (!gaveup)
+                    ew_patch_row<VL, DPL / 2, CT, false, true, SWEEP_PATCH_RC>(pa, (size_t)pair, H - 1 - i, 0, 2, popen[pw]);
+                asm volatile("s_waitcnt vmcnt(0)" ::: "memory");
+                if (lane == 0)
+                    __hip_atomic_store(flags + i, (unsigned long long)ftag << 32, __ATOMIC_RELAXED, __HIP_MEMORY_SCOPE_AGENT);
+                advance((uint32_t)H, false);
+            }
+            advance((uint32_t)H, true);
+#if SWEEP_STATS
+            if (a.stats && lane == 0) {
+                atomicAdd(a.stats + 47, (unsigned long long)(__builtin_readcyclecounter() - pst_life));
+            }
+#endif
+            return;
+        }
+    }
+
     const int kl = lane / VL, g = lane % VL;
     const int c = wave == 0 ? kl : wave == NCW - 1 ? NCOL - HW + kl : HW + (wave - 1) * LPW + kl;
     const int x1 = wg * CW + c - HW;
@@ -757,6 +846,7 @@
         __hip_atomic_store(&rowcnt[wave], (uint32_t)(s + 1), __ATOMIC_RELEASE, __HIP_MEMORY_SCOPE_WORKGROUP);
     };
     [[maybe_unused]] uint64_t st_wait = 0, st_bbar = 0;
+    [[maybe_unused]] uint64_t st_pw0 = 0, st_pw1 = 0;
     SW_T0(st_clife);
     auto wait_row_spin = [&](int s) {
         for (uint32_t spins = 0;; spins++) {
@@ -904,8 +994,34 @@
                     re_[k].template load<SWEEP_STREAM_AUX>(re, boff(en, sizeof(CT)));
                     rw_[k].template load<SWEEP_STREAM_AUX>(rw, boff(en, sizeof(CT)));
                 }
-                if constexpr (OWN && PARTR) rp_[k].template load<SWEEP_STREAM_AUX>(rp, boff(s < nrow ? cell(yy) : NONE, 2));
+                if constexpr (OWN && PARTR)
+                    rp_[k].template load<(NPW > 0 ? 16 : SWEEP_STREAM_AUX)>(rp, boff(s < nrow ? cell(yy) : NONE, 2));
             };
+            [[maybe_unused]] uint32_t pseen = 0;
+            auto wait_patched = [&](int s) {
+                if constexpr (OWN && NPW > 0) {
+                    const uint32_t need = (uint32_t)s + 1u;
+                    if (pseen >= need) return;
+                    SW_T0(tp);
+                    for (uint32_t spins = 0;; spins++) {
+                        pseen = __builtin_amdgcn_readfirstlane(
+                            __hip_atomic_load(&patched_upto, __ATOMIC_RELAXED, __HIP_MEMORY_SCOPE_WORKGROUP));
+                        if (pseen >= need) break;
+                        if (spins >= SW_SPIN_LIMIT) {
+                            if (lane == 0) atomicOr(a.err, 1u);
+                            pseen = 0xFFFFFFFFu;
+                            break;
+                        }
+                        __builtin_amdgcn_s_sleep(1);
+                    }
+                    if (s < 40) SW_ACC(st_pw0, tp);
+                    else SW_ACC(st_pw1, tp);
+                    asm volatile("" ::: "memory");
+                } else {
+                    (void)s;
+                }
+            };
+            if (nrow > 0) wait_patched(min(PF, nrow) - 1);
 #pragma unroll
             for (int k = 0; k < PF; k++) issue_r(k, k);
             uint32_t LVp[NP];
@@ -981,6 +1097,7 @@
                         if constexpr (OWN && EWIN) asm volatile("" : "+v"(Ein[i]), "+v"(Win[i])::"memory");
                         if constexpr (OWN && PARTR) asm volatile("" : "+v"(Pin[i])::"memory");
                     }
+                    if (s + PF < nrow) wait_patched(s + PF);
                     issue_r(k, s + PF);
                     if (ROWSYNC && (j > 0 || NOBAR)) wait_row(s);
                     uint32_t LA[NS][NP], LB[NS][NP], mA[NS], mB[NS];
@@ -1336,6 +1453,10 @@
                 atomicAdd(a.stats + 8 * MODE + 4, (unsigned long long)(__builtin_readcyclecounter() - st_clife));
                 atomicAdd(a.stats + 8 * MODE + 5, 1ull);
                 if (LINES) atomicAdd(a.stats + 40, (unsigned long long)st_wl);
+                if (NPW > 0 && OWN) {
+                    atomicAdd(a.stats + 45, (unsigned long long)st_pw0);
+                    atomicAdd(a.stats + 46, (unsigned long long)st_pw1);
+                }
             }
 #endif
         };
diff --git a/stereo_match_amd/csrc/sm_sweep_host.hpp b/stereo_match_amd/csrc/sm_sweep_host.hpp
--- a/stereo_match_amd/csrc/sm_sweep_host.hpp
+++ b/stereo_match_amd/csrc/sm_sweep_host.hpp
@@ -46,8 +46,14 @@
     size_t vst_pair;
     int xcd_per, xcd_total;
     int part_il;
+    unsigned long long* fixes;
+    size_t flag_off;
+    int pnwg, pcw;
 };
 
+#ifndef SWEEP_NPW
+#define SWEEP_NPW 4
+#endif
 
 struct SweepInfo {
     int cw;
@@ -73,6 +79,7 @@
 hipError_t sweep_info_wide_m2(int D, int ct_bytes, int device, SweepInfo* out);
 hipError_t sweep_info_wide_m3(int D, int ct_bytes, int device, SweepInfo* out);
 hipError_t sweep_info_wide_m4(int D, int ct_bytes, int device, SweepInfo* out);
+hipError_t sweep_info_wide_m4p(int D, int ct_bytes, int device, SweepInfo* out);
 hipError_t sweep_info_lat_m0(int D, int ct_bytes, int device, SweepInfo* out);
 hipError_t sweep_info_lat_m1(int D, int ct_bytes, int device, SweepInfo* out);
 hipError_t sweep_info_lat_m2(int D, int ct_bytes, int device, SweepInfo* out);
@@ -93,6 +100,7 @@
 hipError_t sweep_launch_wide_m2(int D, int ct_bytes, const SweepArgs& a, int npairs, hipStream_t stream);
 hipError_t sweep_launch_wide_m3(int D, int ct_bytes, const SweepArgs& a, int npairs, hipStream_t stream);
 hipError_t sweep_launch_wide_m4(int D, int ct_bytes, const SweepArgs& a, int npairs, hipStream_t stream);
+hipError_t sweep_launch_wide_m4p(int D, int ct_bytes, const SweepArgs& a, int npairs, hipStream_t stream);
 
 inline hipError_t sweep_info(int D, int ct_bytes, int mode, int variant, int device, SweepInfo* out)
 {
@@ -103,6 +111,7 @@
     static const InfoW wide[5] = {sweep_info_wide_m0, sweep_info_wide_m1, sweep_info_wide_m2, sweep_info_wide_m3,
                                   sweep_info_wide_m4};
     static const InfoV narrow[5] = {sweep_info_m0, sweep_info_m1, sweep_info_m2, sweep_info_m3, sweep_info_m4};
+    if (mode == 5) return variant == 0 ? sweep_info_wide_m4p(D, ct_bytes, device, out) : hipErrorInvalidValue;
     if (mode < 0 || mode > 4) return hipErrorInvalidValue;
     if (variant == 2) return lat[mode](D, ct_bytes, device, out);
     if (variant == 0) {
@@ -122,6 +131,7 @@
                                     sweep_launch_wide_m3, sweep_launch_wide_m4};
     static const LaunchV narrow[5] = {sweep_launch_m0, sweep_launch_m1, sweep_launch_m2, sweep_launch_m3,
                                       sweep_launch_m4};
+    if (mode == 5) return impl == 1 ? sweep_launch_wide_m4p(D, ct_bytes, a, npairs, stream) : hipErrorInvalidValue;
     if (mode < 0 || mode > 4) return hipErrorInvalidValue;
     if (impl == 2) return lat[mode](D, ct_bytes, a, npairs, stream);
     if (impl == 1) return wide[mode](D, ct_bytes, a, npairs, stream);
```

Measured after the change: 7106, median of 6. +1.6%, better.
